# ps-auxw/CLI-P

Measured on AMD Instinct MI355X. Metric: images/sec ViT-B/32 encode, higher is better.
Workload: dtype bf16

## Files before the change

### cli-p_amd/_lib.py

```python
import ctypes as C
import os

HERE = os.path.dirname(os.path.abspath(__file__))
DEV_LIB = os.environ.get("CLIPMI_DEV_LIB", "") not in ("", "0")
LIB_PATH = os.path.join(HERE, "libclipmi_dev.so" if DEV_LIB else "libclipmi.so")

ABI_VERSION = 8
F32, BF16, U8 = 0, 1, 2

SYMBOLS = [
    "clipmi_encode_image_workspace_bytes", "clipmi_encode_image",
    "clipmi_encode_text_workspace_bytes", "clipmi_encode_text",
    "clipmi_topk_ip_workspace_bytes", "clipmi_topk_ip",
    "clipmi_topk_ip_coarse_workspace_bytes", "clipmi_topk_ip_coarse", "clipmi_dbg_topk_coarse_scan_ms",
    "clipmi_rows_stats", "clipmi_rows_absmax", "clipmi_rows_order_workspace_bytes", "clipmi_rows_order_by_absmax", "clipmi_rows_to_bf16", "clipmi_i8_copy_bytes", "clipmi_i8_meta_bytes", "clipmi_quantize_rows_i8", "clipmi_topk_ip_coarse_i8", "clipmi_dbg_topk_coarse_i8_scan_ms",
    "clipmi_topk_ip_wide_workspace_bytes", "clipmi_topk_ip_wide_i8", "clipmi_dbg_topk_wide_i8_scan_ms",
    "clipmi_dbg_quantize_rows_fp8", "clipmi_dbg_gemm_fp8",
    "clipmi_merge_topk_workspace_bytes", "clipmi_merge_topk", "clipmi_merge_topk_packed",
    "clipmi_l2_normalize_rows", "clipmi_resize_crop_rgb8", "clipmi_jpeg_workspace_bytes", "clipmi_jpeg_decode_rgb8", "clipmi_jpeg_progressive_workspace_bytes", "clipmi_jpeg_decode_progressive_rgb8", "clipmi_last_error", "clipmi_abi_version",
    "clipmi_dbg_gemm_bf16", "clipmi_dbg_layernorm", "clipmi_dbg_attention", "clipmi_dbg_topk_scan_ms",
    "clipmi_dbg_encode_image_probe_ms", "clipmi_dbg_encode_image_probe3_ms",
    "clipmi_dbg_split_stats", "clipmi_dbg_gemm_ln", "clipmi_dbg_gemm_resid_ln", "clipmi_dbg_gemm_resid_ln_leaf", "clipmi_dbg_gemm_ln_leaf", "clipmi_dbg_quantize_rows_fp8mx", "clipmi_dbg_gemm_fp8_bsa",
]


class Tower(C.Structure):
    _fields_ = [(n, C.c_int32) for n in (
        "abi_version", "kind", "width", "layers", "heads", "mlp", "embed", "tokens",
        "patch", "res", "patch_k", "vocab")] + [(n, C.c_uint64) for n in (
        "blob_bytes",
        "off_patch_w", "off_cls", "off_pos", "off_ln_pre_w", "off_ln_pre_b",
        "off_tok_emb",
        "off_layers", "layer_stride",
        "lo_ln1_w", "lo_ln1_b", "lo_qkv_w", "lo_qkv_b", "lo_out_w", "lo_out_b",
        "lo_ln2_w", "lo_ln2_b", "lo_fc_w", "lo_fc_b", "lo_proj_w", "lo_proj_b",
        "off_ln_post_w", "off_ln_post_b", "off_out_proj")] + [
        ("weight_format", C.c_int32), ("ln_fold", C.c_int32)] + [(n, C.c_uint64) for n in (
        "lo_qkv_s", "lo_out_s", "lo_fc_s", "lo_proj_s", "lo_qkv_colsum", "lo_qkv_cb", "lo_fc_colsum", "lo_fc_cb")]


class ClipmiError(RuntimeError):
    pass


_lib = None


def lib():
    global _lib
    if _lib is not None:
        return _lib
    if not os.path.exists(LIB_PATH):
        raise ClipmiError(
            f"{LIB_PATH} is missing: build the HIP library first "
            "(python -c 'import __graft_entry__ as g; g.build()'). There is no CPU fallback.")
    from . import build as _build
    if os.path.isdir(_build.CSRC) and not _build.is_current(_build.DEV if DEV_LIB else _build.PRODUCT):
        raise ClipmiError(
            f"{LIB_PATH} does not match the sources under csrc/ (content stamp mismatch): rebuild "
            "(python cli-p_amd/build.py). A stale HIP library is never loaded silently.")
    L = C.CDLL(LIB_PATH)
    vp, i32, i64, sz = C.c_void_p, C.c_int, C.c_int64, C.c_size_t
    TP = C.POINTER(Tower)
    L.clipmi_last_error.restype = C.c_char_p
    L.clipmi_abi_version.restype = i32
    L.clipmi_encode_image_workspace_bytes.restype = sz
    L.clipmi_encode_image_workspace_bytes.argtypes = [TP, i32]
    L.clipmi_encode_image.restype = i32
    L.clipmi_encode_image.argtypes = [TP, vp, vp, i32, i32, vp, i32, vp, sz, vp]
    L.clipmi_encode_text_workspace_bytes.restype = sz
    L.clipmi_encode_text_workspace_bytes.argtypes = [TP, i32]
    L.clipmi_encode_text.restype = i32
    L.clipmi_encode_text.argtypes = [TP, vp, vp, i32, vp, i32, vp, sz, vp]
    L.clipmi_topk_ip_workspace_bytes.restype = sz
    L.clipmi_topk_ip_workspace_bytes.argtypes = [i64, i32, i32, i32]
    L.clipmi_topk_ip.restype = i32
    L.clipmi_topk_ip.argtypes = [vp, i32, i64, i32, vp, i32, i32, i64, vp, vp, vp, sz, vp]
    L.clipmi_topk_ip_coarse_workspace_bytes.restype = sz
    L.clipmi_topk_ip_coarse_workspace_bytes.argtypes = [i64, i32, i32, i32]
    L.clipmi_topk_ip_coarse.restype = i32
    L.clipmi_topk_ip_coarse.argtypes = [vp, vp, i64, i32, C.c_float, vp, i32, i32, i64, vp, vp, vp, sz, vp]
    L.clipmi_dbg_quantize_rows_fp8.restype = i32
    L.clipmi_dbg_quantize_rows_fp8.argtypes = [vp, vp, vp, i32, i32, vp]
    L.clipmi_dbg_gemm_fp8.restype = i32
    L.clipmi_dbg_gemm_fp8.argtypes = [vp, vp, vp, vp, vp, vp, i32, i32, i32, i32, vp]
    L.clipmi_rows_stats.restype = i32
    L.clipmi_rows_stats.argtypes = [vp, i64, i32, vp, vp, vp]
    L.clipmi_rows_to_bf16.restype = i32
    L.clipmi_rows_to_bf16.argtypes = [vp, i64, i32, vp, vp]
    L.clipmi_i8_copy_bytes.restype = sz
    L.clipmi_i8_copy_bytes.argtypes = [i64, i32]
    L.clipmi_i8_meta_bytes.restype = sz
    L.clipmi_i8_meta_bytes.argtypes = [i64]
    L.clipmi_quantize_rows_i8.restype = i32
    L.clipmi_quantize_rows_i8.argtypes = [vp, i64, i32, vp, vp, sz, vp, sz, vp]
    L.clipmi_rows_absmax.restype = i32
    L.clipmi_rows_absmax.argtypes = [vp, i64, i32, vp, vp]
    L.clipmi_rows_order_workspace_bytes.restype = sz
    L.clipmi_rows_order_workspace_bytes.argtypes = [i64]
    L.clipmi_rows_order_by_absmax.restype = i32
    L.clipmi_rows_order_by_absmax.argtypes = [vp, i64, i32, vp, vp, sz, vp]
    L.clipmi_topk_ip_coarse_i8.restype = i32
    L.clipmi_topk_ip_coarse_i8.argtypes = [vp, vp, vp, C.c_float, i64, i32, C.c_float, vp, i32, i32, i64, vp, vp, vp, sz, vp]
    L.clipmi_dbg_topk_coarse_i8_scan_ms.restype = i32
    L.clipmi_dbg_topk_coarse_i8_scan_ms.argtypes = [vp, vp, vp, C.c_float, i64, i32, C.c_float, vp, i32, i32, vp, vp, vp, sz, vp,
                                                    i32, C.POINTER(C.c_float), C.POINTER(C.c_longlong)]
    L.clipmi_topk_ip_wide_workspace_bytes.restype = sz
    L.clipmi_topk_ip_wide_workspace_bytes.argtypes = [i64, i32, i32, i32]
    L.clipmi_topk_ip_wide_i8.restype = i32
    L.clipmi_topk_ip_wide_i8.argtypes = [vp, vp, vp, C.c_float, i64, i32, C.c_float, vp, i32, i32, i64, vp, vp, vp, sz, vp]
    L.clipmi_dbg_topk_wide_i8_scan_ms.restype = i32
    L.clipmi_dbg_topk_wide_i8_scan_ms.argtypes = [vp, vp, vp, C.c_float, i64, i32, C.c_float, vp, i32, i32, vp, vp, vp, sz, vp,
                                                  i32, C.POINTER(C.c_float), C.POINTER(C.c_longlong), C.POINTER(C.c_int),
                                                  C.POINTER(C.c_int)]
    L.clipmi_dbg_topk_coarse_scan_ms.restype = i32
    L.clipmi_dbg_topk_coarse_scan_ms.argtypes = [vp, vp, i64, i32, C.c_float, vp, i32, i32, vp, vp, vp, sz, vp, i32,
                                                 C.POINTER(C.c_float), C.POINTER(C.c_longlong)]
    L.clipmi_merge_topk_workspace_bytes.restype = sz
    L.clipmi_merge_topk_workspace_bytes.argtypes = [i32, i32, i32]
    L.clipmi_merge_topk.restype = i32
    L.clipmi_merge_topk.argtypes = [vp, vp, i32, i32, i32, vp, vp, vp, sz, vp]
    L.clipmi_merge_topk_packed.restype = i32
    L.clipmi_merge_topk_packed.argtypes = [vp, sz, i32, i32, i32, vp, vp, vp]
    L.clipmi_l2_normalize_rows.restype = i32
    L.clipmi_l2_normalize_rows.argtypes = [vp, i64, i32, vp]
    L.clipmi_resize_crop_rgb8.restype = i32
    L.clipmi_resize_crop_rgb8.argtypes = [vp, vp, i32, i32, vp, i32, vp, vp, vp]
    L.clipmi_jpeg_workspace_bytes.restype = i64
    L.clipmi_jpeg_workspace_bytes.argtypes = [i64, i32]
    L.clipmi_jpeg_decode_rgb8.restype = i32
    L.clipmi_jpeg_decode_rgb8.argtypes = [vp, vp, i32, vp, i32, i64, i64, i64, vp, vp, vp, i64, vp]
    L.clipmi_jpeg_progressive_workspace_bytes.restype = i64
    L.clipmi_jpeg_progressive_workspace_bytes.argtypes = [i32, i64, i32]
    L.clipmi_jpeg_decode_progressive_rgb8.restype = i32
    L.clipmi_jpeg_decode_progressive_rgb8.argtypes = [vp, vp, i32, vp, i32, vp, i32, i64, i64, i64, vp, vp, vp, i64, vp]
    L.clipmi_dbg_gemm_bf16.restype = i32
    L.clipmi_dbg_gemm_bf16.argtypes = [vp, vp, vp, vp, i32, i32, i32, i32, vp]
    L.clipmi_dbg_split_stats.restype = i32
    L.clipmi_dbg_split_stats.argtypes = [vp, i32, vp, vp, i32, i32, vp]
    L.clipmi_dbg_gemm_ln.restype = i32
    L.clipmi_dbg_gemm_ln.argtypes = [vp, vp, vp, vp, vp, vp, i32, i32, i32, i32, vp]
    L.clipmi_dbg_quantize_rows_fp8mx.restype = i32
    L.clipmi_dbg_quantize_rows_fp8mx.argtypes = [vp, vp, vp, i32, i32, vp]
    L.clipmi_dbg_gemm_fp8_bsa.restype = i32
    L.clipmi_dbg_gemm_fp8_bsa.argtypes = [vp, vp, vp, vp, vp, vp, i32, i32, i32, i32, vp]
    L.clipmi_dbg_gemm_resid_ln_leaf.restype = i32
    L.clipmi_dbg_gemm_resid_ln_leaf.argtypes = [vp, vp, vp, vp, vp, i32, i32, i32, vp]
    L.clipmi_dbg_gemm_ln_leaf.restype = i32
    L.clipmi_dbg_gemm_ln_leaf.argtypes = [vp, vp, vp, vp, vp, vp, i32, i32, i32, i32, vp]
    L.clipmi_dbg_gemm_resid_ln.restype = i32
    L.clipmi_dbg_gemm_resid_ln.argtypes = [vp, vp, vp, vp, vp, vp, i32, i32, i32, i32, vp]
    L.clipmi_dbg_layernorm.restype = i32
    L.clipmi_dbg_layernorm.argtypes = [vp, vp, vp, vp, i32, i32, i32, vp]
    L.clipmi_dbg_attention.restype = i32
    L.clipmi_dbg_attention.argtypes = [vp, vp, i32, i32, i32, i32, vp]
    L.clipmi_dbg_topk_scan_ms.restype = i32
    L.clipmi_dbg_topk_scan_ms.argtypes = [vp, i64, i32, vp, i32, i32, vp, vp, vp, sz, vp, i32, C.POINTER(C.c_float)]
    L.clipmi_dbg_encode_image_probe_ms.restype = i32
    L.clipmi_dbg_encode_image_probe_ms.argtypes = [TP, vp, vp, i32, i32, vp, vp, sz, vp, i32, i32,
                                                   C.POINTER(C.c_float), C.POINTER(C.c_int)]
    L.clipmi_dbg_encode_image_probe3_ms.restype = i32
    L.clipmi_dbg_encode_image_probe3_ms.argtypes = [TP, vp, vp, i32, i32, vp, vp, sz, vp, i32, i32,
                                                    C.POINTER(C.c_float), C.POINTER(C.c_int), C.POINTER(C.c_int),
                                                    C.POINTER(C.c_int)]
    if L.clipmi_abi_version() != ABI_VERSION:
        raise ClipmiError(f"libclipmi.so ABI {L.clipmi_abi_version()} != binding {ABI_VERSION}: rebuild")
    _lib = L
    return L


def check(rc, what):
    if rc != 0:
        msg = lib().clipmi_last_error().decode("utf-8", "replace")
        raise ClipmiError(f"{what} failed (code {rc}): {msg}")


def last_error():
    return lib().clipmi_last_error().decode("utf-8", "replace")


def stream_ptr(device=None):
    import torch
    return C.c_void_p(torch.cuda.current_stream(device).cuda_stream)


_SIDE_STREAMS = {}


_COPY_STREAMS = {}


def copy_stream(device):
    import torch
    key = torch.device(device).index
    s = _COPY_STREAMS.get(key)
    if s is None:
        s = _COPY_STREAMS[key] = torch.cuda.Stream(device=device)
    return s


def side_stream(device):
    import torch
    cur = torch.cuda.current_stream(device)
    key = (torch.device(device).index, cur.cuda_stream)
    s = _SIDE_STREAMS.get(key)
    if s is None:
        s = _SIDE_STREAMS[key] = torch.cuda.Stream(device=device)
    return cur, s
```

### cli-p_amd/csrc/encode.hip

```cpp
#include "vit_kernels.hpp"

namespace clipmi {
namespace {

struct Ws {
    unsigned short* patches;
    float* x;
    unsigned short* h;
    unsigned short* big;
    unsigned short* pooled;
    int* rowidx;
    unsigned char* a8;
    float* a_scale;
    unsigned char* a_bs;
    unsigned char* x8;
    unsigned char* x8_bs;
    void* x3;
    float* ln_part;
    float* ln_leaf;
    void* x3c;
    float* partc;
    float* leafc;
    float* xc;
};

size_t carve(const clipmi_tower* t, int B, void* base, size_t cap, Ws* out) {
    Arena ar(base ? base : reinterpret_cast<void*>(256), cap);
    const size_t rows = (size_t)B * t->tokens;
    const int W = t->width;
    Ws w{};
    if (t->kind == 0) w.patches = ar.take<unsigned short>((size_t)B * (t->tokens - 1) * t->patch_k);
    w.x = ar.take<float>(rows * W);
    w.h = ar.take<unsigned short>(rows * W);
    w.big = ar.take<unsigned short>(rows * 4 * W);
    w.pooled = ar.take<unsigned short>((size_t)B * W);
    w.rowidx = ar.take<int>((size_t)B);
    if (t->weight_format == 1) {
        w.a8 = ar.take<unsigned char>(rows * 4 * W);
        w.a_scale = ar.take<float>(rows);
        w.a_bs = ar.take<unsigned char>((rows + 255) / 256 * 256 * (size_t)(4 * W / 32));
    }
    if (t->ln_fold && t->weight_format == 1) {
        w.x8 = ar.take<unsigned char>(rows * W);
        w.x8_bs = ar.take<unsigned char>((rows + 255) / 256 * 256 * (size_t)(W / 32));
        w.ln_part = ar.take<float>(rows * 2 * (W / 256));
    } else if (t->ln_fold) {
        w.x3 = ar.take<unsigned char>(rows * resid_row_bytes(W));
        w.ln_part = ar.take<float>(rows * 2 * (W / 256));
        if (rows <= (size_t)SKINNY_MAX_M) w.ln_leaf = ar.take<float>(rows * 2 * (W / 4));
    }
    if (t->kind == 0 && t->weight_format == 0) {
        if (t->ln_fold) {
            w.x3c = ar.take<unsigned char>((size_t)B * resid_row_bytes(W));
            w.partc = ar.take<float>((size_t)B * 2 * (W / 256));
            if (B <= SKINNY_MAX_M) w.leafc = ar.take<float>((size_t)B * 2 * (W / 4));
        } else {
            w.xc = ar.take<float>((size_t)B * W);
        }
    }
    if (out) *out = w;
    return ar.off + 256;
}

int check_tower(const clipmi_tower* t, int kind, const char* who) {
    if (!t) return set_err(CLIPMI_EINVAL, "%s: NULL tower", who);
    if (t->abi_version != CLIPMI_ABI_VERSION)
        return set_err(CLIPMI_EINVAL, "%s: tower ABI %d != %d", who, t->abi_version, CLIPMI_ABI_VERSION);
    if (t->kind != kind) return set_err(CLIPMI_EINVAL, "%s: tower kind %d", who, t->kind);
    if (t->width % 128 != 0 || t->heads * 64 != t->width || t->mlp != 4 * t->width || t->embed % 128 != 0 ||
        t->width > 1024 || t->layers < 1)
        return set_err(CLIPMI_EUNSUPPORTED,
                       "%s: width=%d heads=%d mlp=%d embed=%d (need width %% 128 == 0 <= 1024, head dim 64, embed %% 128 == 0)",
                       who, t->width, t->heads, t->mlp, t->embed);
    if (t->weight_format != 0 && t->weight_format != 1)
        return set_err(CLIPMI_EINVAL, "%s: weight_format %d", who, t->weight_format);
    if (t->weight_format == 1 && t->width % 256 != 0)
        return set_err(CLIPMI_EUNSUPPORTED, "%s: fp8 weights need width %% 256 == 0 (width %d)", who, t->width);
    if (t->ln_fold != 0 && (t->ln_fold != 1 || t->width % 256 != 0))
        return set_err(CLIPMI_EINVAL, "%s: ln_fold %d needs width %% 256 == 0 (width %d)", who, t->ln_fold, t->width);
#ifndef CLIPMI_DEV
    if (t->ln_fold != 0 && t->weight_format != 0)
        return set_err(CLIPMI_EUNSUPPORTED, "%s: folded LayerNorms on FP8 weights exist in the development library only", who);
#endif
    if (t->tokens > 80 && kind == 1)
        return set_err(CLIPMI_EUNSUPPORTED, "%s: %d tokens (causal attention covers <= 80)", who, t->tokens);
    return 0;
}

template <typename T>
const T* at(const void* blob, uint64_t off) {
    return reinterpret_cast<const T*>(static_cast<const char*>(blob) + off);
}

bool encode_tail() {
    static const int mode = (int)dev_knob("CLIPMI_ENCODE_TAIL", 1);
    return mode != 0;
}

int launch_gather_rows(const void* src, void* dst, int B, int L, size_t row_bytes, hipStream_t st) {
    if (row_bytes % 16 != 0) return set_err(CLIPMI_EINVAL, "gather_rows: %zu bytes per row", row_bytes);
    const int row16 = (int)(row_bytes / 16);
    hipLaunchKernelGGL(gather_rows_kernel, dim3((unsigned)(((long long)B * row16 + 255) / 256)), dim3(256), 0, st,
                       static_cast<const uint4*>(src), static_cast<uint4*>(dst), B, L, row16);
    CLIPMI_CHECK_LAUNCH("gather_rows_kernel");
    return 0;
}

int run_layers(const clipmi_tower* t, const void* blob, const Ws& w, int B, int causal, hipStream_t st, GemmProbe* probe,
               bool* pruned = nullptr) {
    const int W = t->width, L = t->tokens, M = B * L;
    const bool fp8 = t->weight_format == 1;
    const bool tail = pruned && !causal && !fp8 && (t->ln_fold ? w.x3c != nullptr : w.xc != nullptr) && encode_tail();
    if (pruned) *pruned = tail;
    auto linear = [&](const unsigned short* A, int K, uint64_t w_off, uint64_t b_off, void* out, int N, int epi) -> int {
        GemmArgs g{};
        g.bias = at<float>(blob, b_off); g.out = out; g.M = M; g.N = N; g.K = K;
        g.A = A; g.W = at<unsigned short>(blob, w_off);
        return launch_gemm_algo(g, epi, 0, st, probe);
    };
#ifdef CLIPMI_DEV
    if (t->ln_fold && fp8) {
        auto lnfold8 = [&](uint64_t w_off, uint64_t s_off, uint64_t cb_off, uint64_t cs_off, void* out, unsigned char* out_bs, int N,
                           int epi) -> int {
            GemmArgs g{};
            g.A = reinterpret_cast<const unsigned short*>(w.x8); g.a_bscale = w.x8_bs;
            g.W = at<unsigned short>(blob, w_off); g.w_scale = at<float>(blob, s_off);
            g.bias = at<float>(blob, cb_off); g.colsum = at<float>(blob, cs_off); g.ln_part_in = w.ln_part;
            g.out = out; g.out_bscale = out_bs; g.M = M; g.N = N; g.K = W;
            return launch_gemm_fp8(g, epi, st);
        };
        auto resid8 = [&](const unsigned char* A8, int K, uint64_t w_off, uint64_t s_off, uint64_t b_off) -> int {
            GemmArgs g{};
            g.A = reinterpret_cast<const unsigned short*>(A8); g.a_bscale = w.a_bs;
            g.W = at<unsigned short>(blob, w_off); g.w_scale = at<float>(blob, s_off); g.bias = at<float>(blob, b_off);
            g.out = w.x; g.x8 = w.x8; g.x8_bs = w.x8_bs; g.ln_part = w.ln_part; g.M = M; g.N = W; g.K = K;
            return launch_gemm_fp8(g, EPI_BIAS_RESID_LN8, st);
        };
        unsigned char* const big8 = reinterpret_cast<unsigned char*>(w.big);
        static const bool fuse_off = dev_knob("CLIPMI_FP8_FUSE", 1) == 0;
        for (int l = 0; l < t->layers; ++l) {
            const uint64_t lb = t->off_layers + (uint64_t)l * t->layer_stride;
            if (int rc = lnfold8(lb + t->lo_qkv_w, lb + t->lo_qkv_s, lb + t->lo_qkv_cb, lb + t->lo_qkv_colsum, w.big, nullptr, 3 * W, EPI_LN_BIAS_BF16)) return rc;
            bool fused = false;
            if (int rc = launch_attention(w.big, w.h, B, L, t->heads, causal, 1, st, fuse_off ? nullptr : w.a8, w.a_bs, &fused)) return rc;
            if (!fused)
                if (int rc = launch_quantize_rows_fp8mx(w.h, w.a8, w.a_bs, M, W, st)) return rc;
            if (int rc = resid8(w.a8, W, lb + t->lo_out_w, lb + t->lo_out_s, lb + t->lo_out_b)) return rc;
            if (!fuse_off) {
                if (int rc = lnfold8(lb + t->lo_fc_w, lb + t->lo_fc_s, lb + t->lo_fc_cb, lb + t->lo_fc_colsum, big8, w.a_bs, 4 * W, EPI_LN_BIAS_QGELU_BF16)) return rc;
                if (int rc = resid8(big8, 4 * W, lb + t->lo_proj_w, lb + t->lo_proj_s, lb + t->lo_proj_b)) return rc;
            } else {
                if (int rc = lnfold8(lb + t->lo_fc_w, lb + t->lo_fc_s, lb + t->lo_fc_cb, lb + t->lo_fc_colsum, w.big, nullptr, 4 * W, EPI_LN_BIAS_QGELU_BF16)) return rc;
                if (int rc = launch_quantize_rows_fp8mx(w.big, w.a8, w.a_bs, M, 4 * W, st)) return rc;
                if (int rc = resid8(w.a8, 4 * W, lb + t->lo_proj_w, lb + t->lo_proj_s, lb + t->lo_proj_b)) return rc;
            }
        }
        return 0;
    }
#endif
    if (t->ln_fold) {
        auto lb_of = [&](int l) { return t->off_layers + (uint64_t)l * t->layer_stride; };
        const bool leaf_mode = w.ln_leaf != nullptr && gemm_resid_writes_leaves(M, W, W) && gemm_resid_writes_leaves(M, W, 4 * W);
        bool leaves = false;
        auto ln_linear = [&](uint64_t w_off, uint64_t cb_off, uint64_t cs_off, int N, int epi) -> int {
            GemmArgs g{};
            g.A = static_cast<const unsigned short*>(w.x3); g.lda_bytes = (unsigned)resid_row_bytes(W);
            g.W = at<unsigned short>(blob, w_off); g.bias = at<float>(blob, cb_off);
            g.colsum = at<float>(blob, cs_off); g.ln_part_in = w.ln_part;
            if (leaves) g.ln_leaf_in = w.ln_leaf;
            g.out = w.big; g.M = M; g.N = N; g.K = W;
            return launch_gemm_algo(g, epi, 0, st, probe);
        };
        auto resid_linear = [&](const unsigned short* A, int K, uint64_t w_off, uint64_t b_off) -> int {
            GemmArgs g{};
            g.A = A; g.W = at<unsigned short>(blob, w_off); g.bias = at<float>(blob, b_off);
            g.M = M; g.N = W; g.K = K;
            g.x3 = w.x3; g.ln_part = w.ln_part; g.tmp_f32 = w.x;
            if (leaf_mode) { g.ln_leaf = w.ln_leaf; leaves = true; }
            return launch_gemm_algo(g, EPI_BIAS_RESID_LN_F32, 0, st, probe);
        };
        for (int l = 0; l < t->layers; ++l) {
            const uint64_t lb = lb_of(l);
            if (int rc = ln_linear(lb + t->lo_qkv_w, lb + t->lo_qkv_cb, lb + t->lo_qkv_colsum, 3 * W, EPI_LN_BIAS_BF16)) return rc;
            if (tail && l == t->layers - 1) {
                const bool tleaf = w.leafc != nullptr && gemm_resid_writes_leaves(B, W, W) && gemm_resid_writes_leaves(B, W, 4 * W);
                if (int rc = launch_attention(w.big, w.h, B, L, t->heads, causal, 1, st)) return rc;
                if (int rc = launch_gather_rows(w.x3, w.x3c, B, L, resid_row_bytes(W), st)) return rc;
                auto tail_resid = [&](const unsigned short* A, unsigned lda_bytes, int K, uint64_t w_off, uint64_t b_off) -> int {
                    GemmArgs g{};
                    g.A = A; g.lda_bytes = lda_bytes; g.W = at<unsigned short>(blob, w_off); g.bias = at<float>(blob, b_off);
                    g.M = B; g.N = W; g.K = K;
                    g.x3 = w.x3c; g.ln_part = w.partc; g.tmp_f32 = w.x;
                    if (tleaf) g.ln_leaf = w.leafc;
                    return launch_gemm_algo(g, EPI_BIAS_RESID_LN_F32, 0, st, nullptr);
                };
                if (int rc = tail_resid(w.h, (unsigned)((size_t)L * W * 2), W, lb + t->lo_out_w, lb + t->lo_out_b)) return rc;
                GemmArgs g{};
                g.A = static_cast<const unsigned short*>(w.x3c); g.lda_bytes = (unsigned)resid_row_bytes(W);
                g.W = at<unsigned short>(blob, lb + t->lo_fc_w); g.bias = at<float>(blob, lb + t->lo_fc_cb);
                g.colsum = at<float>(blob, lb + t->lo_fc_colsum); g.ln_part_in = w.partc;
                if (tleaf) g.ln_leaf_in = w.leafc;
                g.out = w.big; g.M = B; g.N = 4 * W; g.K = W;
                if (int rc = launch_gemm_algo(g, EPI_LN_BIAS_QGELU_BF16, 0, st, nullptr)) return rc;
                return tail_resid(w.big, 0u, 4 * W, lb + t->lo_proj_w, lb + t->lo_proj_b);
            }
            hipEvent_t* aev = nullptr;
            if (probe && probe->mode == 2 && probe->n < GemmProbe::MAX) {
                const int pi = probe->begin(GemmProbe::EPI_ATTENTION, 2, st, 0);
                aev = &probe->ev[2 * pi];
            }
            if (int rc = launch_attention(w.big, w.h, B, L, t->heads, causal, 1, st, nullptr, nullptr, nullptr, aev)) return rc;
            if (int rc = resid_linear(w.h, W, lb + t->lo_out_w, lb + t->lo_out_b)) return rc;
            if (int rc = ln_linear(lb + t->lo_fc_w, lb + t->lo_fc_cb, lb + t->lo_fc_colsum, 4 * W, EPI_LN_BIAS_QGELU_BF16)) return rc;
            if (int rc = resid_linear(w.big, 4 * W, lb + t->lo_proj_w, lb + t->lo_proj_b)) return rc;
        }
        return 0;
    }
    if (fp8) {
        auto gemm8 = [&](const unsigned char* A8, const float* a_scale, const unsigned char* a_bs, int K, uint64_t w_off,
                         uint64_t s_off, uint64_t b_off, void* out, unsigned char* out_bs, int N, int epi) -> int {
            GemmArgs g{};
            g.bias = at<float>(blob, b_off); g.out = out; g.M = M; g.N = N; g.K = K;
            g.A = reinterpret_cast<const unsigned short*>(A8);
            g.W = at<unsigned short>(blob, w_off);
            g.a_scale = a_scale; g.a_bscale = a_bs; g.out_bscale = out_bs;
            g.w_scale = at<float>(blob, s_off);
            return launch_gemm_fp8(g, epi, st);
        };
        static const bool fuse_off = dev_knob("CLIPMI_FP8_FUSE", 1) == 0;
        const bool fc_mx = !fuse_off && gemm_fp8_emits_mx(M, 4 * W, W);
        unsigned char* const big8 = reinterpret_cast<unsigned char*>(w.big);
        for (int l = 0; l < t->layers; ++l) {
            const uint64_t lb = t->off_layers + (uint64_t)l * t->layer_stride;
            LnArgs ln{w.x, at<float>(blob, lb + t->lo_ln1_w), at<float>(blob, lb + t->lo_ln1_b), w.h, nullptr, 1, M, W, 1};
            ln.out8 = w.a8; ln.scale8 = w.a_scale;
            if (int rc = launch_layernorm(ln, st)) return rc;
            if (int rc = gemm8(w.a8, w.a_scale, nullptr, W, lb + t->lo_qkv_w, lb + t->lo_qkv_s, lb + t->lo_qkv_b, w.big, nullptr, 3 * W, EPI_BIAS_BF16)) return rc;
            bool fused = false;
            if (int rc = launch_attention(w.big, w.h, B, L, t->heads, causal, 1, st, fuse_off ? nullptr : w.a8, w.a_bs, &fused)) return rc;
            if (!fused)
                if (int rc = launch_quantize_rows_fp8mx(w.h, w.a8, w.a_bs, M, W, st)) return rc;
            if (int rc = gemm8(w.a8, nullptr, w.a_bs, W, lb + t->lo_out_w, lb + t->lo_out_s, lb + t->lo_out_b, w.x, nullptr, W, EPI_BIAS_RESID_F32)) return rc;
            ln.w = at<float>(blob, lb + t->lo_ln2_w); ln.b = at<float>(blob, lb + t->lo_ln2_b);
            if (int rc = launch_layernorm(ln, st)) return rc;
            const unsigned char* h8 = w.a8;
            if (fc_mx) {
                if (int rc = gemm8(w.a8, w.a_scale, nullptr, W, lb + t->lo_fc_w, lb + t->lo_fc_s, lb + t->lo_fc_b, big8, w.a_bs, 4 * W, EPI_BIAS_QGELU_BF16)) return rc;
                h8 = big8;
            } else {
                if (int rc = gemm8(w.a8, w.a_scale, nullptr, W, lb + t->lo_fc_w, lb + t->lo_fc_s, lb + t->lo_fc_b, w.big, nullptr, 4 * W, EPI_BIAS_QGELU_BF16)) return rc;
                if (int rc = launch_quantize_rows_fp8mx(w.big, w.a8, w.a_bs, M, 4 * W, st)) return rc;
            }
            if (int rc = gemm8(h8, nullptr, w.a_bs, 4 * W, lb + t->lo_proj_w, lb + t->lo_proj_s, lb + t->lo_proj_b, w.x, nullptr, W, EPI_BIAS_RESID_F32)) return rc;
        }
        return 0;
    }
    for (int l = 0; l < t->layers; ++l) {
        const uint64_t lb = t->off_layers + (uint64_t)l * t->layer_stride;
        LnArgs ln{w.x, at<float>(blob, lb + t->lo_ln1_w), at<float>(blob, lb + t->lo_ln1_b), w.h, nullptr, 1, M, W, 1};
        if (int rc = launch_layernorm(ln, st)) return rc;
        if (int rc = linear(w.h, W, lb + t->lo_qkv_w, lb + t->lo_qkv_b, w.big, 3 * W, EPI_BIAS_BF16)) return rc;
        if (int rc = launch_attention(w.big, w.h, B, L, t->heads, causal, 1, st)) return rc;
        if (tail && l == t->layers - 1) {
            if (int rc = launch_gather_rows(w.x, w.xc, B, L, (size_t)W * 4, st)) return rc;
            auto tail_linear = [&](const unsigned short* A, unsigned lda_bytes, int K, uint64_t w_off, uint64_t b_off, void* out, int N,
                                   int epi) -> int {
                GemmArgs g{};
                g.A = A; g.lda_bytes = lda_bytes; g.W = at<unsigned short>(blob, w_off); g.bias = at<float>(blob, b_off);
                g.out = out; g.M = B; g.N = N; g.K = K;
                return launch_gemm_algo(g, epi, 0, st, nullptr);
            };
            if (int rc = tail_linear(w.h, (unsigned)((size_t)L * W * 2), W, lb + t->lo_out_w, lb + t->lo_out_b, w.xc, W, EPI_BIAS_RESID_F32)) return rc;
            LnArgs ln2{w.xc, at<float>(blob, lb + t->lo_ln2_w), at<float>(blob, lb + t->lo_ln2_b), w.h, nullptr, 1, B, W, 1};
            if (int rc = launch_layernorm(ln2, st)) return rc;
            if (int rc = tail_linear(w.h, 0u, W, lb + t->lo_fc_w, lb + t->lo_fc_b, w.big, 4 * W, EPI_BIAS_QGELU_BF16)) return rc;
            return tail_linear(w.big, 0u, 4 * W, lb + t->lo_proj_w, lb + t->lo_proj_b, w.xc, W, EPI_BIAS_RESID_F32);
        }
        if (int rc = linear(w.h, W, lb + t->lo_out_w, lb + t->lo_out_b, w.x, W, EPI_BIAS_RESID_F32)) return rc;
        ln.w = at<float>(blob, lb + t->lo_ln2_w); ln.b = at<float>(blob, lb + t->lo_ln2_b);
        if (int rc = launch_layernorm(ln, st)) return rc;
        if (int rc = linear(w.h, W, lb + t->lo_fc_w, lb + t->lo_fc_b, w.big, 4 * W, EPI_BIAS_QGELU_BF16)) return rc;
        if (int rc = linear(w.big, 4 * W, lb + t->lo_proj_w, lb + t->lo_proj_b, w.x, W, EPI_BIAS_RESID_F32)) return rc;
    }
    return 0;
}

int run_head(const clipmi_tower* t, const void* blob, const Ws& w, int B, const int* rowidx, long long row_step,
             float* out, int normalize, hipStream_t st) {
    const bool split = t->ln_fold && t->weight_format == 0;
    LnArgs ln{split ? nullptr : w.x, at<float>(blob, t->off_ln_post_w), at<float>(blob, t->off_ln_post_b), w.pooled, rowidx,
              row_step, B, t->width, 1};
    ln.x3 = w.x3;
    if (int rc = launch_layernorm(ln, st)) return rc;
    GemmArgs g{};
    g.A = w.pooled; g.W = at<unsigned short>(blob, t->off_out_proj); g.bias = nullptr; g.out = out;
    g.M = B; g.N = t->embed; g.K = t->width;
    if (int rc = launch_gemm_algo(g, EPI_F32, 0, st)) return rc;
    if (normalize) return clipmi_l2_normalize_rows(out, B, t->embed, st);
    return 0;
}

}
}

using namespace clipmi;

extern "C" size_t clipmi_encode_image_workspace_bytes(const clipmi_tower* t, int B) {
    if (check_tower(t, 0, "encode_image")) return 0;
    if (B < 1) { set_err(CLIPMI_EINVAL, "encode_image: B=%d", B); return 0; }
    return carve(t, B, nullptr, ~(size_t)0, nullptr);
}

static int encode_image_impl(const clipmi_tower* t, const void* blob_dev, const void* pixels_dev, int pix_dtype,
                             int B, float* out_dev, int normalize, void* ws_dev, size_t ws_bytes, void* stream, GemmProbe* probe) {
    if (int rc = check_tower(t, 0, "encode_image")) return rc;
    if (!blob_dev || !pixels_dev || !out_dev || !ws_dev) return set_err(CLIPMI_EINVAL, "encode_image: NULL pointer");
    if (B < 1) return set_err(CLIPMI_EINVAL, "encode_image: B=%d", B);
    if (pix_dtype != CLIPMI_F32 && pix_dtype != CLIPMI_BF16 && pix_dtype != CLIPMI_U8)
        return set_err(CLIPMI_EINVAL, "encode_image: pix_dtype %d", pix_dtype);
    const int grid = t->res / t->patch, np = grid * grid;
    if (np + 1 != t->tokens || t->patch_k % 64 != 0 || t->patch_k < 3 * t->patch * t->patch)
        return set_err(CLIPMI_EINVAL, "encode_image: inconsistent tower (res %d patch %d tokens %d patch_k %d)", t->res,
                       t->patch, t->tokens, t->patch_k);
    const size_t need = clipmi_encode_image_workspace_bytes(t, B);
    if (ws_bytes < need) return set_err(CLIPMI_EWORKSPACE, "encode_image: workspace %zu < %zu", ws_bytes, need);
    Ws w;
    carve(t, B, ws_dev, ws_bytes, &w);
    hipStream_t st = as_stream(stream);
    const int W = t->width, L = t->tokens;

    PatchArgs pa{pixels_dev, w.patches, pix_dtype, B, t->res, t->patch, grid, np, t->patch_k};
    if (int rc = launch_patchify(pa, st)) return rc;
    GemmArgs g{};
    g.A = w.patches; g.W = at<unsigned short>(blob_dev, t->off_patch_w); g.bias = nullptr; g.out = w.x;
    g.M = B * np; g.N = W; g.K = t->patch_k; g.pos = at<float>(blob_dev, t->off_pos); g.np = np; g.L = L;
    if (int rc = launch_gemm_algo(g, EPI_PATCH_F32, 0, st)) return rc;
    hipLaunchKernelGGL(cls_rows_kernel, dim3((unsigned)(((long long)B * W + 255) / 256)), dim3(256), 0, st, w.x,
                       at<float>(blob_dev, t->off_cls), at<float>(blob_dev, t->off_pos), B, L, W);
    CLIPMI_CHECK_LAUNCH("cls_rows_kernel");
    LnArgs ln{w.x, at<float>(blob_dev, t->off_ln_pre_w), at<float>(blob_dev, t->off_ln_pre_b), w.x, nullptr, 1, B * L, W, 0};
    const bool fold8 = t->ln_fold && t->weight_format == 1;
    if (t->ln_fold && !fold8) { ln.out_x3 = w.x3; ln.out_part = w.ln_part; }
    if (int rc = launch_layernorm(ln, st)) return rc;
#ifdef CLIPMI_DEV
    if (fold8)
        if (int rc = launch_rows_mx_stats(w.x, w.x8, w.x8_bs, w.ln_part, B * L, W, st)) return rc;
#endif
    bool pruned = false;
    if (int rc = run_layers(t, blob_dev, w, B, 0, st, probe, &pruned)) return rc;
    if (pruned) {
        Ws wc = w;
        wc.x = w.xc; wc.x3 = w.x3c;
        return run_head(t, blob_dev, wc, B, nullptr, 1, out_dev, normalize, st);
    }
    return run_head(t, blob_dev, w, B, nullptr, L, out_dev, normalize, st);
}

extern "C" int clipmi_encode_image(const clipmi_tower* t, const void* blob_dev, const void* pixels_dev, int pix_dtype,
                                   int B, float* out_dev, int normalize, void* ws_dev, size_t ws_bytes, void* stream) {
    return encode_image_impl(t, blob_dev, pixels_dev, pix_dtype, B, out_dev, normalize, ws_dev, ws_bytes, stream, nullptr);
}

extern "C" size_t clipmi_encode_text_workspace_bytes(const clipmi_tower* t, int Q) {
    if (check_tower(t, 1, "encode_text")) return 0;
    if (Q < 1) { set_err(CLIPMI_EINVAL, "encode_text: Q=%d", Q); return 0; }
    return carve(t, Q, nullptr, ~(size_t)0, nullptr);
}

extern "C" int clipmi_encode_text(const clipmi_tower* t, const void* blob_dev, const int32_t* ids_dev, int Q,
                                  float* out_dev, int normalize, void* ws_dev, size_t ws_bytes, void* stream) {
    if (int rc = check_tower(t, 1, "encode_text")) return rc;
    if (!blob_dev || !ids_dev || !out_dev || !ws_dev) return set_err(CLIPMI_EINVAL, "encode_text: NULL pointer");
    if (Q < 1) return set_err(CLIPMI_EINVAL, "encode_text: Q=%d", Q);
    const size_t need = clipmi_encode_text_workspace_bytes(t, Q);
    if (ws_bytes < need) return set_err(CLIPMI_EWORKSPACE, "encode_text: workspace %zu < %zu", ws_bytes, need);
    Ws w;
    carve(t, Q, ws_dev, ws_bytes, &w);
    hipStream_t st = as_stream(stream);
    const int W = t->width, L = t->tokens;
    const long long n4 = (long long)Q * L * (W / 4);
    const bool fold8_ = t->ln_fold && t->weight_format == 1;
    if (t->ln_fold && !fold8_ && W % 256 == 0 && W <= 1024) {
        hipLaunchKernelGGL(text_embed_split_kernel, dim3((unsigned)((Q * L + 3) / 4 + 1)), dim3(256), 0, st, ids_dev,
                           at<float>(blob_dev, t->off_tok_emb), at<float>(blob_dev, t->off_pos), w.x3, w.ln_part, w.rowidx, Q, L, W,
                           t->vocab);
        CLIPMI_CHECK_LAUNCH("text_embed_split_kernel");
        if (int rc = run_layers(t, blob_dev, w, Q, 1, st, nullptr)) return rc;
        return run_head(t, blob_dev, w, Q, w.rowidx, 1, out_dev, normalize, st);
    }
    hipLaunchKernelGGL(text_embed_kernel, dim3((unsigned)((n4 + 255) / 256)), dim3(256), 0, st, w.x, ids_dev,
                       at<float>(blob_dev, t->off_tok_emb), at<float>(blob_dev, t->off_pos), Q, L, W, t->vocab);
    CLIPMI_CHECK_LAUNCH("text_embed_kernel");
    hipLaunchKernelGGL(eot_rows_kernel, dim3((Q + 63) / 64), dim3(64), 0, st, ids_dev, w.rowidx, Q, L);
    CLIPMI_CHECK_LAUNCH("eot_rows_kernel");
#ifdef CLIPMI_DEV
    if (t->ln_fold && t->weight_format == 1) {
        if (int rc = launch_rows_mx_stats(w.x, w.x8, w.x8_bs, w.ln_part, Q * L, W, st)) return rc;
    } else
#endif
    if (t->ln_fold) {
        if (int rc = launch_split_stats(w.x, false, w.x3, w.ln_part, Q * L, W, st)) return rc;
    }
    if (int rc = run_layers(t, blob_dev, w, Q, 1, st, nullptr)) return rc;
    return run_head(t, blob_dev, w, Q, w.rowidx, 1, out_dev, normalize, st);
}

static int encode_probe(const clipmi_tower* t, const void* blob_dev, const void* pixels_dev, int pix_dtype, int B, float* out_dev,
                        void* ws_dev, size_t ws_bytes, void* stream, int probe_epi, int reps, int nmodes, float* ms, int* launches,
                        int* kernel_kind, int* epi_ran) {
    if (!ms || reps < 1) return set_err(CLIPMI_EINVAL, "dbg_encode_image_probe_ms: bad arguments");
    const int k_filter = probe_epi >> 8;
    probe_epi &= 0xff;
    GemmProbe p;
    for (int i = 0; i < 2 * GemmProbe::MAX; ++i)
        if (hipEventCreate(&p.ev[i]) != hipSuccess) return set_err(CLIPMI_EHIP, "hipEventCreate");
    for (int i = 0; i < GemmProbe::MAX; ++i)
        if (hipEventCreate(&p.pre[i]) != hipSuccess) return set_err(CLIPMI_EHIP, "hipEventCreate");
    int rc = 0;
    for (int mode = 0; mode < nmodes && rc == 0; ++mode) {
        double total = 0.0;
        int count = 0;
        for (int r = 0; r < reps && rc == 0; ++r) {
            p.epi = probe_epi; p.n = 0; p.mode = mode;
            rc = encode_image_impl(t, blob_dev, pixels_dev, pix_dtype, B, out_dev, 1, ws_dev, ws_bytes, stream, &p);
            if (rc) break;
            if (hipStreamSynchronize(as_stream(stream)) != hipSuccess) { rc = set_err(CLIPMI_EHIP, "hipStreamSynchronize"); break; }
            for (int i = 0; i < p.n; ++i) {
                if (GemmProbe::base_of(p.epi_of[i]) != probe_epi || (k_filter && p.k_of[i] != k_filter)) continue;
                float v = 0.f;
                if (mode == 0) (void)hipEventElapsedTime(&v, p.ev[2 * i], p.ev[2 * i + 1]);
                else if (mode == 1) (void)hipEventElapsedTime(&v, p.pre[i], p.ev[2 * i + 1]);
                else {
                    if (i == 0 || p.kernel_of[i - 1] != 2 ||
                        (p.epi_of[i - 1] != EPI_BIAS_RESID_LN_F32 && p.epi_of[i - 1] != EPI_LN_BIAS_QGELU_BF16 &&
                         p.epi_of[i - 1] != GemmProbe::EPI_ATTENTION)) continue;
                    (void)hipEventElapsedTime(&v, p.ev[2 * (i - 1) + 1], p.ev[2 * i + 1]);
                }
                total += v;
                ++count;
                if (kernel_kind) *kernel_kind = p.kernel_of[i];
                if (epi_ran) *epi_ran = p.epi_of[i];
            }
        }
        if (rc == 0 && count == 0 && mode == 0) rc = set_err(CLIPMI_EINVAL, "dbg_encode_image_probe_ms: no launch matched epi %d", probe_epi);
        if (rc == 0) { ms[mode] = count ? (float)(total / count) : 0.f; if (launches && mode == 0) *launches = count; }
    }
    for (int i = 0; i < 2 * GemmProbe::MAX; ++i) (void)hipEventDestroy(p.ev[i]);
    for (int i = 0; i < GemmProbe::MAX; ++i) (void)hipEventDestroy(p.pre[i]);
    return rc;
}

extern "C" int clipmi_dbg_encode_image_probe_ms(const clipmi_tower* t, const void* blob_dev, const void* pixels_dev,
                                                int pix_dtype, int B, float* out_dev, void* ws_dev, size_t ws_bytes,
                                                void* stream, int probe_epi, int reps, float* kernel_ms, int* launches) {
    return encode_probe(t, blob_dev, pixels_dev, pix_dtype, B, out_dev, ws_dev, ws_bytes, stream, probe_epi, reps, 1, kernel_ms,
                        launches, nullptr, nullptr);
}

extern "C" int clipmi_dbg_encode_image_probe3_ms(const clipmi_tower* t, const void* blob_dev, const void* pixels_dev,
                                                 int pix_dtype, int B, float* out_dev, void* ws_dev, size_t ws_bytes,
                                                 void* stream, int probe_epi, int reps, float* ms3, int* launches,
                                                 int* kernel_kind, int* epi_ran) {
    return encode_probe(t, blob_dev, pixels_dev, pix_dtype, B, out_dev, ws_dev, ws_bytes, stream, probe_epi, reps, 3, ms3,
                        launches, kernel_kind, epi_ran);
}
```

### cli-p_amd/csrc/gemm.hip

```cpp
#include "gemm256p.hpp"
#include "gemm_skinny.hpp"
#ifdef CLIPMI_DEV
#endif
#include "gemm256f8.hpp"
#include <hip/hip_ext.h>
#include <cstdlib>

namespace clipmi {

static bool lds_opted(int* slots) {
    int dev = 0;
    (void)hipGetDevice(&dev);
    if (dev < 0 || dev >= 64) return false;
    if (slots[dev]) return true;
    slots[dev] = 1;
    return false;
}

template <int EPI>
static int launch_epi(const GemmArgs& g, hipStream_t st, GemmProbe* probe) {
    const int grid = (g.N / GEMM_BN) * ((g.M + GEMM_BM - 1) / GEMM_BM);
    if (probe && probe->wants(EPI)) {
        GemmProbe& p = *probe;
        const int i = p.begin(EPI, 0, st, g.K);
        hipExtLaunchKernelGGL(gemm_bf16_nt_kernel<EPI>, dim3(grid), dim3(256), GEMM_LDS_BYTES, st, p.ev[2 * i],
                              p.ev[2 * i + 1], 0, g);
    } else {
        hipLaunchKernelGGL(gemm_bf16_nt_kernel<EPI>, dim3(grid), dim3(256), GEMM_LDS_BYTES, st, g);
    }
    CLIPMI_CHECK_LAUNCH("gemm_bf16_nt_kernel");
    return 0;
}

template <int EPI>
static int launch_epi256(const GemmArgs& g, hipStream_t st, GemmProbe* probe) {
    const int grid = (g.N / 256) * ((g.M + 255) / 256);
    static thread_local int opted[64];
    if (!lds_opted(opted)) {
        if (hipFuncSetAttribute((const void*)gemm256_bf16_nt_kernel<EPI>, hipFuncAttributeMaxDynamicSharedMemorySize,
                                G256_LDS) != hipSuccess)
            return set_err(CLIPMI_EHIP, "hipFuncSetAttribute(gemm256, %d B LDS)", G256_LDS);
    }
    if (probe && probe->wants(EPI)) {
        GemmProbe& p = *probe;
        const int i = p.begin(EPI, 1, st, g.K);
        hipExtLaunchKernelGGL(gemm256_bf16_nt_kernel<EPI>, dim3(grid), dim3(512), G256_LDS, st, p.ev[2 * i],
                              p.ev[2 * i + 1], 0, g);
    } else {
        hipLaunchKernelGGL(gemm256_bf16_nt_kernel<EPI>, dim3(grid), dim3(512), G256_LDS, st, g);
    }
    CLIPMI_CHECK_LAUNCH("gemm256_bf16_nt_kernel");
    return 0;
}

#ifdef CLIPMI_DEV
template <int EPI, int WD = 1>
static int launch_epi256wd(const GemmArgs& g, hipStream_t st) {
    const int grid = (g.N / 256) * ((g.M + 255) / 256);
    static thread_local int opted[64];
    if (!lds_opted(opted)) {
        if (hipFuncSetAttribute((const void*)gemm256_bf16_nt_kernel<EPI, WD>, hipFuncAttributeMaxDynamicSharedMemorySize,
                                G256_LDS) != hipSuccess)
            return set_err(CLIPMI_EHIP, "hipFuncSetAttribute(gemm256 WD, %d B LDS)", G256_LDS);
    }
    hipLaunchKernelGGL((gemm256_bf16_nt_kernel<EPI, WD>), dim3(grid), dim3(512), G256_LDS, st, g);
    CLIPMI_CHECK_LAUNCH("gemm256_bf16_nt_kernel<WD>");
    return 0;
}
#endif

static int persist_mode() {
    static const int mode = (int)dev_knob("CLIPMI_GEMM_PERSIST", 1);
    return mode;
}

constexpr int g256p_lds(int epi, bool fp8, int N, int K, int dbg) {
    const int nseg = K >> 8;
    return G256_LDS + N * 4 * (fp8 ? 2 : 1) + (fp8 ? 1024 : epi_is_ln(epi) ? 1024 + 256 * nseg * 8 + (nseg < 4 ? 8 : 0) : 0) +
           ((dbg & 12) ? 8192 + 2048 : 0);
}

template <int EPI, bool FP8 = false>
static int launch_epi256p(const GemmArgs& g, hipStream_t st, GemmProbe* probe) {
    const int tiles = (g.N / 256) * ((g.M + 255) / 256);
    static const int grid_max = (int)dev_knob("CLIPMI_GEMM_GRID", NUM_CU);
    const int grid = tiles < grid_max ? tiles : grid_max;
    const int lds = g256p_lds(EPI, FP8, g.N, g.K, g.dbg);
    if (lds > LDS_BYTES) return set_err(CLIPMI_EUNSUPPORTED, "gemm256p: %d B of LDS for N=%d", lds, g.N);
    static thread_local int opted[64];
    if (!lds_opted(opted)) {
        if (hipFuncSetAttribute((const void*)gemm256p_bf16_nt_kernel<EPI, FP8>, hipFuncAttributeMaxDynamicSharedMemorySize,
                                LDS_BYTES) != hipSuccess)
            return set_err(CLIPMI_EHIP, "hipFuncSetAttribute(gemm256p, %d B LDS)", LDS_BYTES);
    }
    if (probe && probe->wants(EPI)) {
        GemmProbe& p = *probe;
        const int i = p.begin(EPI, 2, st, g.K);
        hipExtLaunchKernelGGL((gemm256p_bf16_nt_kernel<EPI, FP8>), dim3(grid), dim3(512), lds, st, p.ev[2 * i],
                              p.ev[2 * i + 1], 0, g);
    } else {
        hipLaunchKernelGGL((gemm256p_bf16_nt_kernel<EPI, FP8>), dim3(grid), dim3(512), lds, st, g);
    }
    CLIPMI_CHECK_LAUNCH("gemm256p_bf16_nt_kernel");
    return 0;
}


static int split_pct() {
    static const int pct = (int)dev_knob("CLIPMI_GEMM_SPLIT", 40);
    return pct;
}

static bool skinny_ok(const GemmArgs& g) {
    static const bool off = dev_knob("CLIPMI_GEMM_SKINNY", 1) == 0;
    return !off && g.M >= 1 && g.M <= SKINNY_MAX_M && g.N % 16 == 0 && g.K % 32 == 0 && g.K >= 32;
}

template <int EPI>
static int launch_skinny_t(const GemmArgs& g, hipStream_t st) {
    const int nstrips = g.N / 16, mtiles = (g.M + 15) / 16;
    const int waves = nstrips * mtiles <= 4 * NUM_CU ? 1 : 4;
    const dim3 grid((nstrips + waves - 1) / waves, mtiles);
    if (g.K > 512) hipLaunchKernelGGL((gemm_skinny_kernel<EPI, 32>), grid, dim3(waves * 64), 0, st, g);
    else hipLaunchKernelGGL((gemm_skinny_kernel<EPI, 16>), grid, dim3(waves * 64), 0, st, g);
    CLIPMI_CHECK_LAUNCH("gemm_skinny_kernel");
    return 0;
}

bool gemm_resid_writes_leaves(int M, int N, int K) {
    GemmArgs g{};
    g.M = M; g.N = N; g.K = K;
    return skinny_ok(g) && N % 256 == 0 && N <= 1024;
}

static int launch_skinny(const GemmArgs& g, int epi, hipStream_t st) {
    if (!g.A || !g.W || (!g.out && epi != EPI_BIAS_RESID_LN_F32)) return set_err(CLIPMI_EINVAL, "gemm: NULL pointer");
    switch (epi) {
        case EPI_BIAS_BF16: return launch_skinny_t<EPI_BIAS_BF16>(g, st);
        case EPI_BIAS_QGELU_BF16: return launch_skinny_t<EPI_BIAS_QGELU_BF16>(g, st);
        case EPI_BIAS_RESID_F32: return launch_skinny_t<EPI_BIAS_RESID_F32>(g, st);
        case EPI_F32: return launch_skinny_t<EPI_F32>(g, st);
        case EPI_PATCH_F32: return launch_skinny_t<EPI_PATCH_F32>(g, st);
        case EPI_LN_BIAS_BF16: return launch_skinny_t<EPI_LN_BIAS_BF16>(g, st);
        case EPI_LN_BIAS_QGELU_BF16: return launch_skinny_t<EPI_LN_BIAS_QGELU_BF16>(g, st);
        case EPI_BIAS_RESID_LN_F32: return launch_skinny_t<EPI_BIAS_RESID_LN_F32>(g, st);
    }
    return set_err(CLIPMI_EINVAL, "gemm_skinny: epilogue %d", epi);
}

int launch_gemm_algo(const GemmArgs& g, int epi, int algo, hipStream_t st, GemmProbe* probe) {
    if (epi_is_ln(epi) && ((!g.ln_part_in && !g.ln_leaf_in) || !g.colsum || !g.bias || g.K % 256 != 0 || g.K > 1024))
        return set_err(CLIPMI_EINVAL, "gemm: LN-folded epilogue %d needs ln_part_in, colsum, bias and K %% 256 == 0, K <= 1024", epi);
    if (epi == EPI_BIAS_RESID_LN_F32 &&
        (!g.x3 || !g.ln_part || !g.tmp_f32 || g.N % 256 != 0 || g.N > 1024 || ((size_t)g.x3 & 15) != 0))
        return set_err(CLIPMI_EINVAL, "gemm: EPI_BIAS_RESID_LN_F32 needs x3 (16-byte aligned), ln_part, tmp_f32 and N %% 256 == 0, N <= 1024");
    if (g.lda_bytes && (g.lda_bytes % 16 != 0 || g.lda_bytes < 2u * (unsigned)g.K))
        return set_err(CLIPMI_EINVAL, "gemm: lda_bytes %u (need a multiple of 16, >= 2 K)", g.lda_bytes);
#ifndef CLIPMI_DEV
    if (algo == 4 || algo == 5) return set_err(CLIPMI_EUNSUPPORTED, "algo %d exists in the development build only (libclipmi_dev.so)", algo);
#else
    if (algo == 5) {
        if (g.N % 256 != 0 || g.K % 64 != 0 || g.K < 128 || g.M < 1 || !g.A || !g.W || !g.out)
            return set_err(CLIPMI_EINVAL, "gemm256 WD: N %% 256 == 0, K %% 64 == 0, K >= 128");
        if (epi == EPI_BIAS_BF16) return launch_epi256wd<EPI_BIAS_BF16>(g, st);
        if (epi == EPI_BIAS_QGELU_BF16) return launch_epi256wd<EPI_BIAS_QGELU_BF16>(g, st);
        if (epi == EPI_F32) return launch_epi256wd<EPI_F32>(g, st);
        return set_err(CLIPMI_EINVAL, "gemm256 WD: epilogue %d", epi);
    }
    if (algo == 4) return set_err(CLIPMI_EUNSUPPORTED, "algo 4 (gemm2w, DESIGN 4.4g) was removed in round 5: measured slower in round 3, its sources are in the history");
#endif
    const bool ok256 = g.N % 256 == 0 && g.K % 64 == 0 && g.K >= 128;
    if (algo == 2 && !ok256) return set_err(CLIPMI_EINVAL, "gemm256: N=%d K=%d (need N %% 256 == 0, K %% 64 == 0, K >= 128)", g.N, g.K);
    const bool store_only = epi == EPI_BIAS_BF16 || epi == EPI_BIAS_QGELU_BF16 || epi == EPI_BIAS_RESID_F32 || epi_is_ln(epi) ||
                            epi == EPI_BIAS_RESID_LN_F32;
    const bool ok256p = ok256 && g.K % 128 == 0 && g.N <= G256P_MAX_N && store_only && g.K <= (1 << 20) &&
                        g256p_lds(epi, false, g.N, g.K, g.dbg) <= LDS_BYTES && (!epi_is_ln(epi) || (g.K % 256 == 0 && g.K <= 1024));
    if (algo == 3 && !ok256p)
        return set_err(CLIPMI_EINVAL, "gemm256p: M=%d N=%d K=%d epi=%d (need N %% 256 == 0, K %% 128 == 0, a store-only epilogue "
                       "and bias/colsum rows that fit LDS)", g.M, g.N, g.K, epi);
    bool use256 = algo == 2 || algo == 3;
    bool use256p = algo == 3;
    if (algo == 0 && ok256 && g.M >= 1024) {
        const long long tiles = (long long)(g.N / 256) * ((g.M + 255) / 256);
        const long long rounds = (tiles + NUM_CU - 1) / NUM_CU;
        const long long pct = g.K >= 2048 ? 72 : 78;
        use256 = tiles * 100 >= rounds * NUM_CU * pct;
        use256p = use256 && ok256p && persist_mode() != 0 &&
                  (tiles > NUM_CU || (epi == EPI_BIAS_RESID_LN_F32 && persist_mode() != 2));
        if (ok256p && persist_mode() != 0 && tiles > NUM_CU && epi != EPI_PATCH_F32 && (tiles % NUM_CU) != 0 &&
            (tiles % NUM_CU) * 100 < (long long)NUM_CU * split_pct()) {
            const int ntn = g.N / 256;
            const long long main_tiles = (tiles / NUM_CU) * NUM_CU;
            const int rows_main = (int)(main_tiles / ntn) * 256;
            if (rows_main >= 256 && rows_main < g.M) {
                GemmArgs a = g, b = g;
                a.M = rows_main;
                b.M = g.M - rows_main;
                b.A = g.A + (size_t)rows_main * gemm_lda(g);
                const size_t oe = (size_t)rows_main * g.N;
                if (epi == EPI_BIAS_RESID_LN_F32) {
                    b.x3 = static_cast<char*>(g.x3) + (size_t)rows_main * resid_row_bytes(g.N); b.tmp_f32 = g.tmp_f32 + oe;
                    b.ln_part = g.ln_part + (size_t)rows_main * (g.N / 256) * 2;
                } else if (epi_is_bf16_out(epi)) {
                    b.out = static_cast<unsigned short*>(g.out) + oe;
                } else {
                    b.out = static_cast<float*>(g.out) + oe;
                }
                if (b.ln_part_in) b.ln_part_in = g.ln_part_in + (size_t)rows_main * (g.K / 256) * 2;
                if (int rc = launch_gemm_algo(a, epi, 3, st, probe)) return rc;
                return launch_gemm_algo(b, epi, 0, st, probe);
            }
        }
    }
    if (g.M < 1 || !g.A || !g.W || (!g.out && epi != EPI_BIAS_RESID_LN_F32)) return set_err(CLIPMI_EINVAL, "gemm: bad arguments");
    const bool skinny = algo == 0 && skinny_ok(g);
    if (skinny && epi != EPI_BIAS_RESID_LN_F32) return launch_skinny(g, epi, st);
    if (epi == EPI_BIAS_RESID_LN_F32 && skinny && g.ln_leaf) return launch_skinny(g, epi, st);
    if (g.ln_leaf_in && !(skinny && epi_is_ln(epi)))
        return set_err(CLIPMI_EINVAL, "gemm: ln_leaf_in is read by the skinny LN-folded consumers only (M <= %d)", SKINNY_MAX_M);
    if (epi == EPI_BIAS_RESID_LN_F32 && !use256p) {
        GemmArgs t = g;
        t.out = g.tmp_f32;
        GemmProbe* pr = (probe && probe->wants(EPI_BIAS_RESID_LN_F32)) ? probe : nullptr;
        const int saved_epi = pr ? pr->epi : -1;
        if (pr) pr->epi = EPI_F32;
        const int rc = skinny ? launch_skinny(t, EPI_F32, st) : use256 ? launch_epi256<EPI_F32>(t, st, pr) : launch_gemm(t, EPI_F32, st, pr);
        if (pr) pr->epi = saved_epi;
        if (rc) return rc;
        return launch_split_stats(g.tmp_f32, true, g.x3, g.ln_part, g.M, g.N, st);
    }
    if (!use256) return launch_gemm(g, epi, st, probe);
    if (use256p) {
        switch (epi) {
            case EPI_BIAS_BF16: return launch_epi256p<EPI_BIAS_BF16>(g, st, probe);
            case EPI_BIAS_QGELU_BF16: return launch_epi256p<EPI_BIAS_QGELU_BF16>(g, st, probe);
            case EPI_BIAS_RESID_F32: return launch_epi256p<EPI_BIAS_RESID_F32>(g, st, probe);
            case EPI_LN_BIAS_BF16: return launch_epi256p<EPI_LN_BIAS_BF16>(g, st, probe);
            case EPI_LN_BIAS_QGELU_BF16: return launch_epi256p<EPI_LN_BIAS_QGELU_BF16>(g, st, probe);
            case EPI_BIAS_RESID_LN_F32: return launch_epi256p<EPI_BIAS_RESID_LN_F32>(g, st, probe);
        }
        return set_err(CLIPMI_EINVAL, "gemm256p: epilogue %d", epi);
    }
    switch (epi) {
        case EPI_BIAS_BF16: return launch_epi256<EPI_BIAS_BF16>(g, st, probe);
        case EPI_BIAS_QGELU_BF16: return launch_epi256<EPI_BIAS_QGELU_BF16>(g, st, probe);
        case EPI_BIAS_RESID_F32: return launch_epi256<EPI_BIAS_RESID_F32>(g, st, probe);
        case EPI_F32: return launch_epi256<EPI_F32>(g, st, probe);
        case EPI_PATCH_F32: return launch_epi256<EPI_PATCH_F32>(g, st, probe);
        case EPI_LN_BIAS_BF16: return launch_epi256<EPI_LN_BIAS_BF16>(g, st, probe);
        case EPI_LN_BIAS_QGELU_BF16: return launch_epi256<EPI_LN_BIAS_QGELU_BF16>(g, st, probe);
    }
    return set_err(CLIPMI_EINVAL, "gemm: unknown epilogue %d", epi);
}

template <int EPI, bool MX>
static int launch_epi256f8(const GemmArgs& g, hipStream_t st) {
    const int grid = (g.N / 256) * ((g.M + 255) / 256);
    static thread_local int opted[64];
    if (!lds_opted(opted)) {
        if (hipFuncSetAttribute((const void*)gemm256f8_nt_kernel<EPI, MX>, hipFuncAttributeMaxDynamicSharedMemorySize,
                                G256_LDS) != hipSuccess)
            return set_err(CLIPMI_EHIP, "hipFuncSetAttribute(gemm256f8, %d B LDS)", G256_LDS);
    }
    hipLaunchKernelGGL((gemm256f8_nt_kernel<EPI, MX>), dim3(grid), dim3(512), G256_LDS, st, g);
    CLIPMI_CHECK_LAUNCH("gemm256f8_nt_kernel");
    return 0;
}

constexpr int G256F8_BSA_MAX_K = 4096;
template <int EPI>
static int launch_epi256f8_bsa(const GemmArgs& g, hipStream_t st) {
    const int grid = (g.N / 256) * ((g.M + 255) / 256);
    const int lds = G256_LDS + 256 * (g.K / 32);
    static thread_local int opted[64];
    if (!lds_opted(opted)) {
        if (hipFuncSetAttribute((const void*)gemm256f8_nt_kernel<EPI, true, true>, hipFuncAttributeMaxDynamicSharedMemorySize,
                                G256_LDS + 256 * (G256F8_BSA_MAX_K / 32)) != hipSuccess)
            return set_err(CLIPMI_EHIP, "hipFuncSetAttribute(gemm256f8 block-scaled)");
    }
    hipLaunchKernelGGL((gemm256f8_nt_kernel<EPI, true, true>), dim3(grid), dim3(512), lds, st, g);
    CLIPMI_CHECK_LAUNCH("gemm256f8_nt_kernel(block-scaled A)");
    return 0;
}

bool gemm_fp8_emits_mx(int M, int N, int K) {
    const long long tiles = (long long)(N / 256) * ((M + 255) / 256);
    return M >= 1 && N % 256 == 0 && K % 256 == 0 && K >= 256 && tiles > NUM_CU && N <= 3840 && persist_mode() != 0;
}

int launch_gemm_fp8(const GemmArgs& g, int epi, hipStream_t st, int mx) {
    if (g.M < 1 || g.N % 256 != 0 || g.K % 128 != 0 || g.K < 256)
        return set_err(CLIPMI_EINVAL, "gemm_fp8: M=%d N=%d K=%d (need N %% 256 == 0, K %% 128 == 0, K >= 256)", g.M, g.N, g.K);
    if (!g.A || !g.W || !g.out || (!g.a_scale && !g.a_bscale) || !g.w_scale) return set_err(CLIPMI_EINVAL, "gemm_fp8: NULL pointer");
    if (g.a_bscale) {
        if (g.K > G256F8_BSA_MAX_K) return set_err(CLIPMI_EINVAL, "gemm_fp8: block-scaled A needs K <= %d", G256F8_BSA_MAX_K);
        if (epi == EPI_BIAS_RESID_F32) return launch_epi256f8_bsa<EPI_BIAS_RESID_F32>(g, st);
        if (epi == EPI_F32) return launch_epi256f8_bsa<EPI_F32>(g, st);
#ifdef CLIPMI_DEV
        if (epi == EPI_BIAS_RESID_LN8) {
            if (!g.x8 || !g.x8_bs || !g.ln_part || g.N > 1024)
                return set_err(CLIPMI_EINVAL, "gemm_fp8: EPI_BIAS_RESID_LN8 needs x8, x8_bs, ln_part and N <= 1024");
            return launch_epi256f8_bsa<EPI_BIAS_RESID_LN8>(g, st);
        }
        if (epi_is_ln(epi)) {
            if (!g.ln_part_in || !g.colsum || !g.bias || g.K % 256 != 0 || g.K > 1024)
                return set_err(CLIPMI_EINVAL, "gemm_fp8: LN-folded epilogue %d needs ln_part_in, colsum, bias, K %% 256 == 0, K <= 1024", epi);
            if (g.out_bscale && epi != EPI_LN_BIAS_QGELU_BF16)
                return set_err(CLIPMI_EINVAL, "gemm_fp8: e4m3 + block-scale output exists for the QuickGELU forms only");
            return epi == EPI_LN_BIAS_BF16 ? launch_epi256f8_bsa<EPI_LN_BIAS_BF16>(g, st) : launch_epi256f8_bsa<EPI_LN_BIAS_QGELU_BF16>(g, st);
        }
#endif
        return set_err(CLIPMI_EINVAL, "gemm_fp8: block-scaled A with epilogue %d", epi);
    }
    const long long tiles = (long long)(g.N / 256) * ((g.M + 255) / 256);
    if (g.out_bscale && !(mx == 1 && epi == EPI_BIAS_QGELU_BF16 && gemm_fp8_emits_mx(g.M, g.N, g.K)))
        return set_err(CLIPMI_EINVAL, "gemm_fp8: e4m3 + block-scale output exists for the persistent QuickGELU form only");
    if (mx == 1 && tiles > NUM_CU && g.K % 256 == 0 && g.N <= 3840 && persist_mode() != 0) {
        if (epi == EPI_BIAS_BF16) return launch_epi256p<EPI_BIAS_BF16, true>(g, st, nullptr);
        if (epi == EPI_BIAS_QGELU_BF16) return launch_epi256p<EPI_BIAS_QGELU_BF16, true>(g, st, nullptr);
    }
    switch (epi) {
        case EPI_BIAS_BF16: return mx ? launch_epi256f8<EPI_BIAS_BF16, true>(g, st) : launch_epi256f8<EPI_BIAS_BF16, false>(g, st);
        case EPI_BIAS_QGELU_BF16:
            return mx ? launch_epi256f8<EPI_BIAS_QGELU_BF16, true>(g, st) : launch_epi256f8<EPI_BIAS_QGELU_BF16, false>(g, st);
        case EPI_BIAS_RESID_F32:
            return mx ? launch_epi256f8<EPI_BIAS_RESID_F32, true>(g, st) : launch_epi256f8<EPI_BIAS_RESID_F32, false>(g, st);
        case EPI_F32: return mx ? launch_epi256f8<EPI_F32, true>(g, st) : launch_epi256f8<EPI_F32, false>(g, st);
    }
    return set_err(CLIPMI_EINVAL, "gemm_fp8: epilogue %d", epi);
}

int launch_gemm(const GemmArgs& g, int epi, hipStream_t st, GemmProbe* probe) {
    if (g.M < 1 || g.N < 1 || g.K < 1 || g.N % GEMM_BN != 0 || g.K % GEMM_BK != 0)
        return set_err(CLIPMI_EINVAL, "gemm: M=%d N=%d K=%d (need N %% 128 == 0, K %% 64 == 0)", g.M, g.N, g.K);
    if (!g.A || !g.W || !g.out) return set_err(CLIPMI_EINVAL, "gemm: NULL pointer");
    switch (epi) {
        case EPI_BIAS_BF16: return launch_epi<EPI_BIAS_BF16>(g, st, probe);
        case EPI_BIAS_QGELU_BF16: return launch_epi<EPI_BIAS_QGELU_BF16>(g, st, probe);
        case EPI_BIAS_RESID_F32: return launch_epi<EPI_BIAS_RESID_F32>(g, st, probe);
        case EPI_F32: return launch_epi<EPI_F32>(g, st, probe);
        case EPI_PATCH_F32: return launch_epi<EPI_PATCH_F32>(g, st, probe);
        case EPI_LN_BIAS_BF16: return launch_epi<EPI_LN_BIAS_BF16>(g, st, probe);
        case EPI_LN_BIAS_QGELU_BF16: return launch_epi<EPI_LN_BIAS_QGELU_BF16>(g, st, probe);
    }
    return set_err(CLIPMI_EINVAL, "gemm: unknown epilogue %d", epi);
}

}

using namespace clipmi;

extern "C" int clipmi_dbg_gemm_bf16(const void* a_dev, const void* w_dev, const float* bias_dev, void* out_dev, int M,
                                    int N, int K, int epi, void* stream) {
    const int algo = (epi >> 8) & 7;
    epi &= 0xff;
    if (epi < 0 || epi > 3) return set_err(CLIPMI_EINVAL, "dbg_gemm: epi %d", epi);
    GemmArgs g{};
    g.A = static_cast<const unsigned short*>(a_dev);
    g.W = static_cast<const unsigned short*>(w_dev);
    g.bias = bias_dev;
    g.out = out_dev;
    g.M = M; g.N = N; g.K = K;
    static const int dbg_env = (int)dev_knob("CLIPMI_GEMM_DBG", 0);
    g.dbg = dbg_env;
    if (g.dbg & 12) { g.pos = bias_dev; g.bias = nullptr; }
    return launch_gemm_algo(g, epi, algo, as_stream(stream));
}

extern "C" int clipmi_dbg_gemm_ln(const void* x3_dev, const void* wg_dev, const float* cb_dev, const float* colsum_dev,
                                  const float* part_dev, void* out_dev, int M, int N, int K, int epi, void* stream) {
    const int algo = (epi >> 8) & 3;
    epi &= 0xff;
    if (!epi_is_ln(epi)) return set_err(CLIPMI_EINVAL, "dbg_gemm_ln: epi %d", epi);
    GemmArgs g{};
    g.A = static_cast<const unsigned short*>(x3_dev);
    g.lda_bytes = (unsigned)resid_row_bytes(K);
    g.W = static_cast<const unsigned short*>(wg_dev);
    g.bias = cb_dev; g.colsum = colsum_dev; g.ln_part_in = part_dev;
    g.out = out_dev;
    g.M = M; g.N = N; g.K = K;
    return launch_gemm_algo(g, epi, algo, as_stream(stream));
}

extern "C" int clipmi_dbg_gemm_resid_ln_leaf(const void* a_dev, const void* w_dev, const float* bias_dev, void* x3_dev, float* leaf_dev,
                                             int M, int N, int K, void* stream) {
    if (!leaf_dev || !gemm_resid_writes_leaves(M, N, K))
        return set_err(CLIPMI_EINVAL, "dbg_gemm_resid_ln_leaf: M <= %d, N %% 256 == 0, N <= 1024, K %% 32 == 0", SKINNY_MAX_M);
    GemmArgs g{};
    g.A = static_cast<const unsigned short*>(a_dev);
    g.W = static_cast<const unsigned short*>(w_dev);
    g.bias = bias_dev;
    g.x3 = x3_dev; g.ln_leaf = leaf_dev;
    g.ln_part = leaf_dev; g.tmp_f32 = leaf_dev;
    g.M = M; g.N = N; g.K = K;
    return launch_gemm_algo(g, EPI_BIAS_RESID_LN_F32, 0, as_stream(stream));
}

extern "C" int clipmi_dbg_gemm_ln_leaf(const void* x3_dev, const void* wg_dev, const float* cb_dev, const float* colsum_dev,
                                       const float* leaf_dev, void* out_dev, int M, int N, int K, int epi, void* stream) {
    if (!epi_is_ln(epi)) return set_err(CLIPMI_EINVAL, "dbg_gemm_ln_leaf: epi %d", epi);
    GemmArgs g{};
    g.A = static_cast<const unsigned short*>(x3_dev);
    g.lda_bytes = (unsigned)resid_row_bytes(K);
    g.W = static_cast<const unsigned short*>(wg_dev);
    g.bias = cb_dev; g.colsum = colsum_dev; g.ln_leaf_in = leaf_dev;
    g.out = out_dev;
    g.M = M; g.N = N; g.K = K;
    return launch_gemm_algo(g, epi, 0, as_stream(stream));
}

extern "C" int clipmi_dbg_gemm_resid_ln(const void* a_dev, const void* w_dev, const float* bias_dev, void* x3_dev,
                                        float* part_dev, float* tmp_dev, int M, int N, int K, int algo, void* stream) {
    GemmArgs g{};
    g.A = static_cast<const unsigned short*>(a_dev);
    g.W = static_cast<const unsigned short*>(w_dev);
    g.bias = bias_dev;
    g.x3 = x3_dev;
    g.ln_part = part_dev; g.tmp_f32 = tmp_dev;
    g.M = M; g.N = N; g.K = K;
    static const int dbg_env = (int)dev_knob("CLIPMI_GEMM_DBG", 0);
    g.dbg = dbg_env;
    return launch_gemm_algo(g, EPI_BIAS_RESID_LN_F32, algo & 7, as_stream(stream));
}

extern "C" int clipmi_dbg_gemm_fp8_bsa(const void* a8_dev, const void* w8_dev, const void* a_bscale_dev, const float* w_scale_dev,
                                       const float* bias_dev, void* out_dev, int M, int N, int K, int epi, void* stream) {
    GemmArgs g{};
    g.A = static_cast<const unsigned short*>(a8_dev);
    g.W = static_cast<const unsigned short*>(w8_dev);
    g.a_bscale = static_cast<const unsigned char*>(a_bscale_dev); g.w_scale = w_scale_dev;
    g.bias = bias_dev;
    g.out = out_dev;
    g.M = M; g.N = N; g.K = K;
    return launch_gemm_fp8(g, epi, as_stream(stream), 1);
}

extern "C" int clipmi_dbg_gemm_fp8(const void* a8_dev, const void* w8_dev, const float* a_scale_dev, const float* w_scale_dev,
                                   const float* bias_dev, void* out_dev, int M, int N, int K, int epi, void* stream) {
    const int mx = (epi >> 8) & 1 ? 0 : ((epi >> 9) & 1 ? 2 : 1);
    epi &= 0xff;
    if (epi < 0 || epi > 3) return set_err(CLIPMI_EINVAL, "dbg_gemm_fp8: epi %d", epi);
    GemmArgs g{};
    g.A = static_cast<const unsigned short*>(a8_dev);
    g.W = static_cast<const unsigned short*>(w8_dev);
    g.a_scale = a_scale_dev; g.w_scale = w_scale_dev;
    g.bias = bias_dev;
    g.out = out_dev;
    g.M = M; g.N = N; g.K = K;
    return launch_gemm_fp8(g, epi, as_stream(stream), mx);
}
```

### cli-p_amd/csrc/gemm.hpp

```cpp
#pragma once
#include "common.hpp"

namespace clipmi {

typedef __bf16 bf16x8 __attribute__((ext_vector_type(8)));
typedef __bf16 bf16x2 __attribute__((ext_vector_type(2)));
typedef float f32x4 __attribute__((ext_vector_type(4)));
typedef float f32x2 __attribute__((ext_vector_type(2)));

__device__ __forceinline__ unsigned pack_bf16x2(float a, float b) {
    f32x2 v = {a, b};
    bf16x2 r = __builtin_convertvector(v, bf16x2);
    return __builtin_bit_cast(unsigned, r);
}

__device__ __forceinline__ float bf16_to_f32(unsigned short h) { return __uint_as_float((unsigned)h << 16); }

constexpr float QGELU_C = -2.4554669595930157f;
__device__ __forceinline__ float quick_gelu(float x) {
    return x * __builtin_amdgcn_rcpf(1.0f + __builtin_amdgcn_exp2f(x * QGELU_C));
}
__device__ __forceinline__ f32x4 quick_gelu4(f32x4 x) {
    const f32x4 t = x * QGELU_C;
    f32x4 e;
    e.x = __builtin_amdgcn_exp2f(t.x); e.y = __builtin_amdgcn_exp2f(t.y);
    e.z = __builtin_amdgcn_exp2f(t.z); e.w = __builtin_amdgcn_exp2f(t.w);
    const f32x4 d = e + 1.0f;
    f32x4 r;
    r.x = __builtin_amdgcn_rcpf(d.x); r.y = __builtin_amdgcn_rcpf(d.y);
    r.z = __builtin_amdgcn_rcpf(d.z); r.w = __builtin_amdgcn_rcpf(d.w);
    return x * r;
}

enum Epilogue {
    EPI_BIAS_BF16 = 0,
    EPI_BIAS_QGELU_BF16 = 1,
    EPI_BIAS_RESID_F32 = 2,
    EPI_F32 = 3,
    EPI_PATCH_F32 = 4,
    EPI_LN_BIAS_BF16 = 5,
    EPI_LN_BIAS_QGELU_BF16 = 6,
    EPI_BIAS_RESID_LN_F32 = 7,
    EPI_BIAS_RESID_LN8 = 8
};

constexpr float LN_EPS = 1e-5f;

__device__ __forceinline__ float ln_lane_sum(f32x4 v) { return (v.x + v.y) + (v.z + v.w); }
__device__ __forceinline__ float ln_lane_sumsq(f32x4 v) {
    float q = v.x * v.x;
    q = __builtin_fmaf(v.y, v.y, q);
    q = __builtin_fmaf(v.z, v.z, q);
    return __builtin_fmaf(v.w, v.w, q);
}
template <int CTRL>
__device__ __forceinline__ float lane_dpp(float v) {
    return __int_as_float(__builtin_amdgcn_update_dpp(0, __float_as_int(v), CTRL, 0xf, 0xf, false));
}
__device__ __forceinline__ float lane_xor8(float v) { return lane_dpp<0x128>(v); }
__device__ __forceinline__ float lane_xor4(float v, bool bit2) {
    const float up = lane_dpp<0x104>(v), dn = lane_dpp<0x114>(v);
    return bit2 ? dn : up;
}
__device__ __forceinline__ float lane_xor2(float v) { return lane_dpp<0x4E>(v); }
__device__ __forceinline__ float lane_xor1(float v) { return lane_dpp<0xB1>(v); }
__device__ __forceinline__ float lane_fold32(float a, float b) {
    const auto r = __builtin_amdgcn_permlane32_swap(__float_as_uint(a), __float_as_uint(b), false, false);
    return __uint_as_float(r[0]) + __uint_as_float(r[1]);
}
__device__ __forceinline__ float lane_fold16(float a, float b) {
    const auto r = __builtin_amdgcn_permlane16_swap(__float_as_uint(a), __float_as_uint(b), false, false);
    return __uint_as_float(r[0]) + __uint_as_float(r[1]);
}
__device__ __forceinline__ float ln_wave_sum(float v) {
    const bool bit2 = (__builtin_amdgcn_mbcnt_lo(~0u, 0u) & 4u) != 0;
    v = lane_fold32(v, v);
    v = lane_fold16(v, v);
    v += lane_xor8(v);
    v += lane_xor4(v, bit2);
    v += lane_xor2(v);
    v += lane_xor1(v);
    return v;
}
__device__ __forceinline__ f32x2 ln_row_stats(const float* part, int nseg, int W) {
    float s = part[0], q = part[1];
    if (nseg > 1) { s += part[2]; q += part[3]; }
    if (nseg > 2) { s += part[4]; q += part[5]; }
    if (nseg > 3) { s += part[6]; q += part[7]; }
    const float inv = 1.0f / (float)W;
    const float mean = s * inv;
    float var = __builtin_fmaf(-mean, mean, q * inv);
    var = var > 0.f ? var : 0.f;
    return f32x2{mean, __builtin_amdgcn_rsqf(var + LN_EPS)};
}
__device__ __forceinline__ f32x4 ln_apply(f32x4 acc, float mean, float rstd, f32x4 colsum, f32x4 cb) {
    f32x4 r;
    r.x = __builtin_fmaf(__builtin_fmaf(-mean, colsum.x, acc.x), rstd, cb.x);
    r.y = __builtin_fmaf(__builtin_fmaf(-mean, colsum.y, acc.y), rstd, cb.y);
    r.z = __builtin_fmaf(__builtin_fmaf(-mean, colsum.z, acc.z), rstd, cb.z);
    r.w = __builtin_fmaf(__builtin_fmaf(-mean, colsum.w, acc.w), rstd, cb.w);
    return r;
}
__device__ __forceinline__ f32x4 split_join(uint2 hi, unsigned lo) {
    return f32x4{__uint_as_float(__builtin_amdgcn_perm(hi.x, lo, 0x0504000cu) - 0x8000u),
                 __uint_as_float(__builtin_amdgcn_perm(hi.x, lo, 0x0706010cu) - 0x8000u),
                 __uint_as_float(__builtin_amdgcn_perm(hi.y, lo, 0x0504020cu) - 0x8000u),
                 __uint_as_float(__builtin_amdgcn_perm(hi.y, lo, 0x0706030cu) - 0x8000u)};
}
__device__ __forceinline__ void split_make(f32x4 o, uint2& hi, unsigned& lo) {
    hi = make_uint2(pack_bf16x2(o.x, o.y), pack_bf16x2(o.z, o.w));
    auto rem = [](float v, unsigned hb) -> unsigned {
        const unsigned t = (__float_as_uint(v) + 0x8080u) - hb;
        return t < 0xffffu ? t : 0xffffu;
    };
    const unsigned t0 = rem(o.x, hi.x << 16), t1 = rem(o.y, hi.x & 0xffff0000u), t2 = rem(o.z, hi.y << 16),
                   t3 = rem(o.w, hi.y & 0xffff0000u);
    lo = __builtin_amdgcn_perm(t1, t0, 0x0c0c0501u) | __builtin_amdgcn_perm(t3, t2, 0x05010c0cu);
}
__host__ __device__ constexpr size_t resid_row_bytes(int W) { return (size_t)W * 3; }
__device__ __forceinline__ const unsigned short* resid_hi(const void* x3, size_t row, int W) {
    return reinterpret_cast<const unsigned short*>(static_cast<const char*>(x3) + row * resid_row_bytes(W));
}
__device__ __forceinline__ unsigned short* resid_hi(void* x3, size_t row, int W) {
    return reinterpret_cast<unsigned short*>(static_cast<char*>(x3) + row * resid_row_bytes(W));
}
__device__ __forceinline__ const unsigned char* resid_lo(const void* x3, size_t row, int W) {
    return reinterpret_cast<const unsigned char*>(static_cast<const char*>(x3) + row * resid_row_bytes(W) + (size_t)W * 2);
}
__device__ __forceinline__ unsigned char* resid_lo(void* x3, size_t row, int W) {
    return reinterpret_cast<unsigned char*>(static_cast<char*>(x3) + row * resid_row_bytes(W) + (size_t)W * 2);
}
__device__ __forceinline__ unsigned fp8mx_scale_byte(float amax) {
    const int e = (int)((__float_as_uint(amax) >> 23) & 0xffu);
    if (amax == 0.f) return 127u;
    return (unsigned)(e > 7 ? e - 7 : 0);
}
__device__ __forceinline__ float fp8mx_inv(unsigned sb) { return __uint_as_float((254u - sb) << 23); }
__device__ __forceinline__ uint2 fp8_pack8(const float* f) {
    int lo = 0, hi = 0;
    lo = __builtin_amdgcn_cvt_pk_fp8_f32(f[0], f[1], lo, false);
    lo = __builtin_amdgcn_cvt_pk_fp8_f32(f[2], f[3], lo, true);
    hi = __builtin_amdgcn_cvt_pk_fp8_f32(f[4], f[5], hi, false);
    hi = __builtin_amdgcn_cvt_pk_fp8_f32(f[6], f[7], hi, true);
    return make_uint2((unsigned)lo, (unsigned)hi);
}

__device__ __forceinline__ void ln8_row_segment(f32x4 v, unsigned& packed4, unsigned& scale_byte, float& sum, float& sumsq) {
    sum = ln_wave_sum(ln_lane_sum(v));
    sumsq = ln_wave_sum(ln_lane_sumsq(v));
    float mx = fmaxf(fmaxf(fabsf(v.x), fabsf(v.y)), fmaxf(fabsf(v.z), fabsf(v.w)));
    mx = fmaxf(mx, __shfl_xor(mx, 1));
    mx = fmaxf(mx, __shfl_xor(mx, 2));
    mx = fmaxf(mx, __shfl_xor(mx, 4));
    scale_byte = fp8mx_scale_byte(mx);
    const float inv = fp8mx_inv(scale_byte);
    int pk = 0;
    pk = __builtin_amdgcn_cvt_pk_fp8_f32(v.x * inv, v.y * inv, pk, false);
    pk = __builtin_amdgcn_cvt_pk_fp8_f32(v.z * inv, v.w * inv, pk, true);
    packed4 = (unsigned)pk;
}

__device__ __forceinline__ uint2 mx_pack_bf16x8(uint4 x, unsigned& sb_out) {
    const unsigned w_[4] = {x.x, x.y, x.z, x.w};
    typedef unsigned short u16x2 __attribute__((ext_vector_type(2)));
    u16x2 pm = __builtin_elementwise_max(
        __builtin_elementwise_max(__builtin_bit_cast(u16x2, w_[0] & 0x7fff7fffu), __builtin_bit_cast(u16x2, w_[1] & 0x7fff7fffu)),
        __builtin_elementwise_max(__builtin_bit_cast(u16x2, w_[2] & 0x7fff7fffu), __builtin_bit_cast(u16x2, w_[3] & 0x7fff7fffu)));
    unsigned mm = __builtin_bit_cast(unsigned, pm);
    mm = (mm & 0xffffu) > (mm >> 16) ? (mm & 0xffffu) : (mm >> 16);
    const unsigned m1_ = (unsigned)__builtin_amdgcn_update_dpp(0, (int)mm, 0xB1, 0xf, 0xf, false);
    mm = mm > m1_ ? mm : m1_;
    const unsigned m2_ = (unsigned)__builtin_amdgcn_update_dpp(0, (int)mm, 0x4E, 0xf, 0xf, false);
    mm = mm > m2_ ? mm : m2_;
    const unsigned e_ = mm >> 7;
    const unsigned sb_ = mm == 0u ? 127u : (e_ > 7u ? e_ - 7u : 0u);
    const float inv_ = fp8mx_inv(sb_);
    float f[8];
#pragma unroll
    for (int j = 0; j < 4; ++j) {
        const f32x2 p_ = f32x2{__uint_as_float(w_[j] << 16), __uint_as_float(w_[j] & 0xffff0000u)} * inv_;
        f[2 * j] = p_.x;
        f[2 * j + 1] = p_.y;
    }
    sb_out = sb_;
    return fp8_pack8(f);
}

constexpr bool epi_is_ln(int e) { return e == EPI_LN_BIAS_BF16 || e == EPI_LN_BIAS_QGELU_BF16; }
constexpr bool epi_is_qgelu(int e) { return e == EPI_BIAS_QGELU_BF16 || e == EPI_LN_BIAS_QGELU_BF16; }
constexpr bool epi_is_bf16_out(int e) { return e == EPI_BIAS_BF16 || e == EPI_BIAS_QGELU_BF16 || epi_is_ln(e); }

struct GemmArgs {
    const unsigned short* A;
    const unsigned short* W;
    const float* bias;
    void* out;
    int M, N, K;
    const float* pos;
    int np, L;
    unsigned char* x8;
    unsigned char* x8_bs;
    int dbg;
    const float* a_scale;
    const float* w_scale;
    const unsigned char* a_bscale;
    unsigned char* out_bscale;
    const float* ln_part_in;
    const float* colsum;
    void* x3;
    float* ln_part;
    float* tmp_f32;
    unsigned lda_bytes;
    float* ln_leaf;
    const float* ln_leaf_in;
};
constexpr int SKINNY_MAX_M = 128;
__host__ __device__ inline size_t gemm_lda(const GemmArgs& g) { return g.lda_bytes ? (size_t)g.lda_bytes / 2 : (size_t)g.K; }

__device__ __forceinline__ void gemm_tile_coords(int bid, int nwg, int mtiles, int ntn, int GM, int GN, int& bm, int& bn) {
    const int xcd = bid & 7, qq = nwg >> 3, rr = nwg & 7;
    const int tile = (xcd < rr ? xcd * (qq + 1) : rr * (qq + 1) + (xcd - rr) * qq) + (bid >> 3);
    const int per_super = GM * ntn;
    const int sr = tile / per_super;
    const int r = tile - sr * per_super;
    const int left = mtiles - sr * GM;
    const int gm = left < GM ? left : GM;
    const int full = ntn / GN;
    int ng = r / (gm * GN);
    ng = ng < full ? ng : full;
    const int r2 = r - ng * gm * GN;
    const int gn = (ntn - ng * GN) < GN ? (ntn - ng * GN) : GN;
    const int mi = r2 / gn;
    bm = sr * GM + mi;
    bn = ng * GN + (r2 - mi * gn);
}

constexpr int GEMM_BM = 128, GEMM_BN = 128, GEMM_BK = 64;
constexpr int GEMM_TILE_BYTES = GEMM_BM * GEMM_BK * 2;
constexpr int GEMM_LDS_BYTES = 4 * GEMM_TILE_BYTES;

template <int EPI>
__global__ void __launch_bounds__(256) gemm_bf16_nt_kernel(GemmArgs g) {
    extern __shared__ __attribute__((aligned(16))) char smem[];
    const int tid = threadIdx.x;
    const int lane = tid & 63;
    const int wave = __builtin_amdgcn_readfirstlane(tid >> 6);
    const int wm = wave >> 1, wn = wave & 1;
    const int fr = lane & 15, fg = lane >> 4;

    const int ntn = g.N / GEMM_BN;
    int bm, bn;
    gemm_tile_coords(blockIdx.x, gridDim.x, (g.M + GEMM_BM - 1) / GEMM_BM, ntn, 8, 8, bm, bn);
    const int m0 = bm * GEMM_BM, n0 = bn * GEMM_BN;
    const int K = g.K;

    const int srow = lane >> 3;
    const int spos = lane & 7;
    const unsigned short* a_src[4];
    const unsigned short* w_src[4];
#pragma unroll
    for (int i = 0; i < 4; ++i) {
        const int row = wave * 32 + i * 8 + srow;
        const int chunk = spos ^ (row & 7);
        int am = m0 + row;
        am = am < g.M ? am : g.M - 1;
        a_src[i] = g.A + (size_t)am * gemm_lda(g) + chunk * 8;
        w_src[i] = g.W + (size_t)(n0 + row) * K + chunk * 8;
    }
    auto stage = [&](int kt, int buf) {
        char* abase = smem + buf * (2 * GEMM_TILE_BYTES) + wave * 32 * 128;
        char* bbase = abase + GEMM_TILE_BYTES;
#pragma unroll
        for (int i = 0; i < 4; ++i) {
            __builtin_amdgcn_global_load_lds((const __attribute__((address_space(1))) void*)(a_src[i] + kt * GEMM_BK),
                                             (__attribute__((address_space(3))) void*)(abase + i * 1024), 16, 0, 0);
            __builtin_amdgcn_global_load_lds((const __attribute__((address_space(1))) void*)(w_src[i] + kt * GEMM_BK),
                                             (__attribute__((address_space(3))) void*)(bbase + i * 1024), 16, 0, 0);
        }
    };

    f32x4 acc[4][4];
#pragma unroll
    for (int i = 0; i < 4; ++i)
#pragma unroll
        for (int j = 0; j < 4; ++j) acc[i][j] = f32x4{0.f, 0.f, 0.f, 0.f};

    const int sw = fr & 7;
    const int a_off = (wm * 64 + fr) * 128;
    const int b_off = GEMM_TILE_BYTES + (wn * 64 + fr) * 128;
    const int c0 = ((0 + fg) ^ sw) * 16, c1 = ((4 + fg) ^ sw) * 16;

    const int nk = K / GEMM_BK;
    stage(0, 0);
    for (int kt = 0; kt < nk; ++kt) {
        asm volatile("s_waitcnt vmcnt(0)" ::: "memory");
        __syncthreads();
        if (kt + 1 < nk) stage(kt + 1, (kt + 1) & 1);
        const char* base = smem + (kt & 1) * (2 * GEMM_TILE_BYTES);
        bf16x8 af[4][2], wf[4][2];
#pragma unroll
        for (int t = 0; t < 4; ++t) {
            af[t][0] = *reinterpret_cast<const bf16x8*>(base + a_off + t * 2048 + c0);
            af[t][1] = *reinterpret_cast<const bf16x8*>(base + a_off + t * 2048 + c1);
            wf[t][0] = *reinterpret_cast<const bf16x8*>(base + b_off + t * 2048 + c0);
            wf[t][1] = *reinterpret_cast<const bf16x8*>(base + b_off + t * 2048 + c1);
        }
#pragma unroll
        for (int ks = 0; ks < 2; ++ks)
#pragma unroll
            for (int mt = 0; mt < 4; ++mt)
#pragma unroll
                for (int nt = 0; nt < 4; ++nt)
                    acc[mt][nt] = __builtin_amdgcn_mfma_f32_16x16x32_bf16(wf[nt][ks], af[mt][ks], acc[mt][nt], 0, 0, 0);
    }

    f32x4 bz[4], cs[4];
#pragma unroll
    for (int nt = 0; nt < 4; ++nt) {
        const int n = n0 + wn * 64 + nt * 16 + 4 * fg;
        bz[nt] = g.bias ? *reinterpret_cast<const f32x4*>(g.bias + n) : f32x4{0.f, 0.f, 0.f, 0.f};
        if (epi_is_ln(EPI)) cs[nt] = *reinterpret_cast<const f32x4*>(g.colsum + n);
    }
    constexpr bool RMW = (EPI == EPI_BIAS_RESID_F32) || (EPI == EPI_PATCH_F32);
    auto row_of = [&](int mt, size_t& orow, const float*& addrow, bool& valid) {
        const int m = m0 + wm * 64 + mt * 16 + fr;
        valid = m < g.M;
        const int mc = valid ? m : g.M - 1;
        orow = (size_t)mc;
        addrow = nullptr;
        if (EPI == EPI_PATCH_F32) {
            const int b_ = mc / g.np, p_ = mc - b_ * g.np;
            orow = (size_t)b_ * g.L + 1 + p_;
            addrow = g.pos + (size_t)(1 + p_) * g.N;
        } else if (EPI == EPI_BIAS_RESID_F32) {
            addrow = static_cast<const float*>(g.out) + orow * g.N;
        }
    };
    f32x4 cur[4], nxt[4];
    if (RMW) {
        size_t orow; const float* addrow; bool valid;
        row_of(0, orow, addrow, valid);
#pragma unroll
        for (int nt = 0; nt < 4; ++nt) cur[nt] = *reinterpret_cast<const f32x4*>(addrow + n0 + wn * 64 + nt * 16 + 4 * fg);
    }
#pragma unroll
    for (int mt = 0; mt < 4; ++mt) {
        size_t orow; const float* addrow; bool valid;
        row_of(mt, orow, addrow, valid);
        if (RMW && mt + 1 < 4) {
            size_t orow2; const float* addrow2; bool valid2;
            row_of(mt + 1, orow2, addrow2, valid2);
#pragma unroll
            for (int nt = 0; nt < 4; ++nt) nxt[nt] = *reinterpret_cast<const f32x4*>(addrow2 + n0 + wn * 64 + nt * 16 + 4 * fg);
        }
#pragma unroll
        for (int nt = 0; nt < 4; ++nt) {
            const int n = n0 + wn * 64 + nt * 16 + 4 * fg;
            f32x4 v;
            if (epi_is_ln(EPI)) {
                const int nseg = g.K >> 8;
                const f32x2 st = ln_row_stats(g.ln_part_in + orow * 2 * nseg, nseg, g.K);
                v = ln_apply(acc[mt][nt], st.x, st.y, cs[nt], bz[nt]);
            } else {
                v = acc[mt][nt] + bz[nt];
            }
            if (epi_is_bf16_out(EPI)) {
                if (epi_is_qgelu(EPI)) {
                    v = quick_gelu4(v);
                }
                if (valid)
                    *reinterpret_cast<uint2*>(static_cast<unsigned short*>(g.out) + orow * g.N + n) =
                        make_uint2(pack_bf16x2(v.x, v.y), pack_bf16x2(v.z, v.w));
            } else {
                if (RMW) v += cur[nt];
                if (valid) *reinterpret_cast<f32x4*>(static_cast<float*>(g.out) + orow * g.N + n) = v;
            }
        }
        if (RMW) {
#pragma unroll
            for (int nt = 0; nt < 4; ++nt) cur[nt] = nxt[nt];
        }
    }
}

struct GemmProbe {
    static constexpr int MAX = 96;
    static constexpr int EPI_ATTENTION = 100;
    int epi = -1, n = 0;
    int mode = 0;
    hipEvent_t ev[2 * MAX];
    hipEvent_t pre[MAX];
    int epi_of[MAX];
    int kernel_of[MAX];
    int k_of[MAX];
    static int base_of(int e) {
        return e == EPI_LN_BIAS_BF16 ? EPI_BIAS_BF16 : e == EPI_LN_BIAS_QGELU_BF16 ? EPI_BIAS_QGELU_BF16 :
               e == EPI_BIAS_RESID_LN_F32 ? EPI_BIAS_RESID_F32 : e;
    }
    bool wants(int e) const { return n < MAX && (mode == 2 || base_of(e) == epi); }
    int begin(int e, int kernel, hipStream_t st, int K = 0) {
        epi_of[n] = e;
        kernel_of[n] = kernel;
        k_of[n] = K;
        if (mode == 1) (void)hipEventRecord(pre[n], st);
        return n++;
    }
};

int launch_gemm(const GemmArgs& g, int epi, hipStream_t st, GemmProbe* probe = nullptr);
int launch_gemm_algo(const GemmArgs& g, int epi, int algo, hipStream_t st, GemmProbe* probe = nullptr);
int launch_gemm_fp8(const GemmArgs& g, int epi, hipStream_t st, int mx = 1);
bool gemm_resid_writes_leaves(int M, int N, int K);
bool gemm_fp8_emits_mx(int M, int N, int K);
int launch_split_stats(const float* x_or_add, bool add, void* x3, float* part, int M, int W, hipStream_t st);

}
```

### cli-p_amd/csrc/gemm_skinny.hpp

```cpp
#pragma once
#include "gemm.hpp"

namespace clipmi {

template <int EPI, int DEPTH>
__global__ void __launch_bounds__(256) gemm_skinny_kernel(GemmArgs g) {
    constexpr int SKINNY_DEPTH = DEPTH;
    const int lane = threadIdx.x & 63;
    const int wave = __builtin_amdgcn_readfirstlane(threadIdx.x >> 6);
    const int fr = lane & 15, fg = lane >> 4;
    const int nstrips = g.N >> 4;
    const int strip = blockIdx.x * (blockDim.x >> 6) + wave;
    if (strip >= nstrips) return;
    const int n0 = strip << 4, m0 = blockIdx.y << 4;
    const int K = g.K;
    int am = m0 + fr;
    const bool valid = am < g.M;
    am = valid ? am : g.M - 1;
    const bf16x8* wp = reinterpret_cast<const bf16x8*>(g.W + (size_t)(n0 + fr) * K + 8 * fg);
    const bf16x8* ap = reinterpret_cast<const bf16x8*>(g.A + (size_t)am * gemm_lda(g) + 8 * fg);
    const int nk = K >> 5;

    const int n = n0 + 4 * fg;
    const f32x4 bz = g.bias ? *reinterpret_cast<const f32x4*>(g.bias + n) : f32x4{0.f, 0.f, 0.f, 0.f};
    f32x4 cs = {0.f, 0.f, 0.f, 0.f};
    float part[8] = {0.f, 0.f, 0.f, 0.f, 0.f, 0.f, 0.f, 0.f};
    f32x4 add = {0.f, 0.f, 0.f, 0.f};
    size_t orow = (size_t)am;
    if (epi_is_ln(EPI)) {
        cs = *reinterpret_cast<const f32x4*>(g.colsum + n);
        const int nseg = K >> 8;
        if (!g.ln_leaf_in) {
            const float* pp = g.ln_part_in + orow * 2 * nseg;
#pragma unroll
            for (int i = 0; i < 4; ++i)
                if (i < nseg) { part[2 * i] = pp[2 * i]; part[2 * i + 1] = pp[2 * i + 1]; }
        }
    } else if (EPI == EPI_PATCH_F32) {
        const int b_ = am / g.np, p_ = am - b_ * g.np;
        orow = (size_t)b_ * g.L + 1 + p_;
        add = *reinterpret_cast<const f32x4*>(g.pos + (size_t)(1 + p_) * g.N + n);
    } else if (EPI == EPI_BIAS_RESID_F32) {
        add = *reinterpret_cast<const f32x4*>(static_cast<const float*>(g.out) + orow * g.N + n);
    }
    uint2 xh = make_uint2(0u, 0u);
    unsigned xl = 0u;
    if (EPI == EPI_BIAS_RESID_LN_F32) {
        xh = *reinterpret_cast<const uint2*>(resid_hi(g.x3, orow, g.N) + n);
        xl = *reinterpret_cast<const unsigned*>(resid_lo(g.x3, orow, g.N) + n);
    }
    if (epi_is_ln(EPI) && g.ln_leaf_in) {
        const int nseg = K >> 8;
        const f32x2* lf = reinterpret_cast<const f32x2*>(g.ln_leaf_in) + orow * (size_t)(K >> 2) + fg;
#pragma unroll
        for (int j = 0; j < 4; ++j) {
            if (j < nseg) {
                f32x2 v[16];
#pragma unroll
                for (int t = 0; t < 16; ++t) v[t] = lf[64 * j + 4 * t];
                float sm[2];
#pragma unroll
                for (int c = 0; c < 2; ++c) {
                    float a[8], b[4];
#pragma unroll
                    for (int t = 0; t < 8; ++t) a[t] = v[t][c] + v[t + 8][c];
#pragma unroll
                    for (int t = 0; t < 4; ++t) b[t] = a[t] + a[t + 4];
                    const float c0 = b[0] + b[2], c1 = b[1] + b[3];
                    float d = c0 + c1;
                    d = lane_fold32(d, d);
                    sm[c] = lane_fold16(d, d);
                }
                part[2 * j] = sm[0];
                part[2 * j + 1] = sm[1];
            }
        }
    }

    f32x4 acc = {0.f, 0.f, 0.f, 0.f};
    bf16x8 wf[SKINNY_DEPTH], af[SKINNY_DEPTH];
#pragma unroll
    for (int d = 0; d < SKINNY_DEPTH; ++d) {
        const int s = d < nk ? d : nk - 1;
        wf[d] = wp[4 * s];
        af[d] = ap[4 * s];
    }
    for (int s0 = 0; s0 < nk; s0 += SKINNY_DEPTH) {
#pragma unroll
        for (int d = 0; d < SKINNY_DEPTH; ++d) {
            if (s0 + d < nk) acc = __builtin_amdgcn_mfma_f32_16x16x32_bf16(wf[d], af[d], acc, 0, 0, 0);
            int s = s0 + d + SKINNY_DEPTH;
            s = s < nk ? s : nk - 1;
            wf[d] = wp[4 * s];
            af[d] = ap[4 * s];
        }
    }

    f32x4 v;
    if (epi_is_ln(EPI)) {
        const f32x2 st = ln_row_stats(part, K >> 8, K);
        v = ln_apply(acc, st.x, st.y, cs, bz);
    } else {
        v = acc + bz;
    }
    if (epi_is_bf16_out(EPI)) {
        if (epi_is_qgelu(EPI)) v = quick_gelu4(v);
        if (valid)
            *reinterpret_cast<uint2*>(static_cast<unsigned short*>(g.out) + orow * g.N + n) =
                make_uint2(pack_bf16x2(v.x, v.y), pack_bf16x2(v.z, v.w));
        return;
    }
    if (EPI == EPI_BIAS_RESID_LN_F32) {
        const f32x4 o = v + split_join(xh, xl);
        uint2 nh;
        unsigned nl;
        split_make(o, nh, nl);
        if (valid) {
            *reinterpret_cast<uint2*>(resid_hi(g.x3, orow, g.N) + n) = nh;
            *reinterpret_cast<unsigned*>(resid_lo(g.x3, orow, g.N) + n) = nl;
            *reinterpret_cast<f32x2*>(g.ln_leaf + (orow * (size_t)(g.N >> 2) + (size_t)(n >> 2)) * 2) = f32x2{ln_lane_sum(o), ln_lane_sumsq(o)};
        }
        return;
    }
    if (EPI == EPI_PATCH_F32 || EPI == EPI_BIAS_RESID_F32) v += add;
    if (valid) *reinterpret_cast<f32x4*>(static_cast<float*>(g.out) + orow * g.N + n) = v;
}

}
```

### cli-p_amd/csrc/vit_kernels.hip

```cpp
#include "vit_kernels.hpp"
#include <hip/hip_ext.h>
#include <cstdlib>

namespace clipmi {

int launch_layernorm(const LnArgs& a, hipStream_t st) {
    if (a.M < 1) return 0;
    if (a.W % 4 != 0 || a.W > 1024) return set_err(CLIPMI_EINVAL, "layernorm: W=%d (need W %% 4 == 0, W <= 1024)", a.W);
    if (a.out_x3 && (a.W % 256 != 0 || !a.out_part)) return set_err(CLIPMI_EINVAL, "layernorm: split output needs W %% 256 == 0");
    hipLaunchKernelGGL(layernorm_kernel, dim3((a.M + 3) / 4), dim3(256), 0, st, a);
    CLIPMI_CHECK_LAUNCH("layernorm_kernel");
    return 0;
}

int launch_split_stats(const float* x_or_add, bool add, void* x3, float* part, int M, int W, hipStream_t st) {
    if (M < 1) return 0;
    if (!x_or_add || !x3 || !part || W % 256 != 0 || W < 256 || W > 1024)
        return set_err(CLIPMI_EINVAL, "split_stats: W=%d (need W %% 256 == 0, 256 <= W <= 1024)", W);
    if (add) hipLaunchKernelGGL(split_stats_kernel<true>, dim3((M + 3) / 4), dim3(256), 0, st, x_or_add, x3, part, M, W);
    else hipLaunchKernelGGL(split_stats_kernel<false>, dim3((M + 3) / 4), dim3(256), 0, st, x_or_add, x3, part, M, W);
    CLIPMI_CHECK_LAUNCH("split_stats_kernel");
    return 0;
}

template <int NT, bool CAUSAL, bool TR>
static int launch_attn_t(const unsigned short* qkv, unsigned short* out, int B, int L, int heads, hipStream_t st) {
    constexpr int KS = (NT + 1) / 2;
    const size_t lds = 4 * KS * 32 * 128;
    const long long items = (long long)B * heads;
    hipLaunchKernelGGL((attention_kernel<NT, CAUSAL, TR>), dim3((unsigned)((items + 3) / 4)), dim3(256), lds, st, qkv, out,
                       B, L, heads);
    CLIPMI_CHECK_LAUNCH("attention_kernel");
    return 0;
}

int launch_attention(const unsigned short* qkv, unsigned short* out, int B, int L, int heads, int causal, int tr,
                     hipStream_t st, unsigned char* out8, unsigned char* out_bs, bool* fused, hipEvent_t* probe_ev) {
    if (fused) *fused = false;
    if (B < 1) return 0;
    if (L < 1) return set_err(CLIPMI_EINVAL, "attention: L=%d", L);
    if (L > 80) {
        if (causal) return set_err(CLIPMI_EUNSUPPORTED, "attention: causal mask with L=%d > 80", L);
        const int qblocks = (L + 31) / 32;
        const int g4 = (qblocks + 3) / 4;
        const long long groups = (long long)B * heads * g4;
        hipLaunchKernelGGL((attention_flash_kernel<4, 2>), dim3((unsigned)groups), dim3(256), 2 * 16384, st, qkv, out, B, L, heads, g4);
        CLIPMI_CHECK_LAUNCH("attention_flash_kernel");
        return 0;
    }
    const int nt = (L + 15) / 16;
    static const int use52 = (int)dev_knob("CLIPMI_ATTN52", 2);
    if (L >= 49 && L <= 52 && !causal && tr == 1 && use52 == 2) {
        const long long items = (long long)B * heads;
        const long long resident = (long long)NUM_CU * 5;
        if (out8 && out_bs && fused) {
            hipLaunchKernelGGL(attention52x4_kernel<true>, dim3((unsigned)(items < resident ? items : resident)), dim3(256),
                               64 * 128 + 52 * 128, st, qkv, out, B, L, heads, out8, out_bs);
            *fused = true;
        } else if (probe_ev) {
            hipExtLaunchKernelGGL(attention52x4_kernel<false>, dim3((unsigned)(items < resident ? items : resident)), dim3(256),
                                  64 * 128 + 52 * 128, st, probe_ev[0], probe_ev[1], 0, qkv, out, B, L, heads, (unsigned char*)nullptr,
                                  (unsigned char*)nullptr);
        } else {
            hipLaunchKernelGGL(attention52x4_kernel<false>, dim3((unsigned)(items < resident ? items : resident)), dim3(256),
                               64 * 128 + 52 * 128, st, qkv, out, B, L, heads, (unsigned char*)nullptr, (unsigned char*)nullptr);
        }
        CLIPMI_CHECK_LAUNCH("attention52x4_kernel");
        return 0;
    }
    if (L >= 49 && L <= 52 && !causal && tr && use52) {
        const long long items = (long long)B * heads;
        const size_t lds = 4 * 52 * 128;
        hipLaunchKernelGGL(attention52_kernel, dim3((unsigned)((items + 3) / 4)), dim3(256), lds, st, qkv, out, B, L, heads);
        CLIPMI_CHECK_LAUNCH("attention52_kernel");
        return 0;
    }
#define ATT(NT_)                                                                                         \
    if (nt <= NT_) {                                                                                     \
        if (causal) return tr ? launch_attn_t<NT_, true, true>(qkv, out, B, L, heads, st)                \
                              : launch_attn_t<NT_, true, false>(qkv, out, B, L, heads, st);              \
        return tr ? launch_attn_t<NT_, false, true>(qkv, out, B, L, heads, st)                           \
                  : launch_attn_t<NT_, false, false>(qkv, out, B, L, heads, st);                         \
    }
    ATT(1) ATT(2) ATT(4) ATT(5)
#undef ATT
    return set_err(CLIPMI_EUNSUPPORTED, "attention: L=%d", L);
}

int launch_quantize_rows_fp8(const unsigned short* in, unsigned char* out, float* scale, int M, int K, hipStream_t st) {
    if (M < 1) return 0;
    if (K < 8 || K % 8 != 0 || !in || !out || !scale) return set_err(CLIPMI_EINVAL, "quantize_rows_fp8: K=%d", K);
    hipLaunchKernelGGL(quantize_rows_fp8_kernel, dim3((unsigned)((M + 3) / 4)), dim3(256), 0, st, in, out, scale, M, K);
    CLIPMI_CHECK_LAUNCH("quantize_rows_fp8_kernel");
    return 0;
}

int launch_quantize_rows_fp8mx(const unsigned short* in, unsigned char* out, unsigned char* bscale, int M, int K, hipStream_t st) {
    if (M < 1) return 0;
    if (K < 32 || K % 32 != 0 || !in || !out || !bscale) return set_err(CLIPMI_EINVAL, "quantize_rows_fp8mx: K=%d", K);
    hipLaunchKernelGGL(quantize_rows_fp8mx_kernel, dim3((unsigned)((M + 3) / 4)), dim3(256), 0, st, in, out, bscale, M, K);
    CLIPMI_CHECK_LAUNCH("quantize_rows_fp8mx_kernel");
    return 0;
}

#ifdef CLIPMI_DEV
int launch_rows_mx_stats(const float* x, unsigned char* x8, unsigned char* bs, float* part, int M, int W, hipStream_t st) {
    if (M < 1) return 0;
    if (W < 256 || W % 256 != 0 || !x || !x8 || !bs || !part) return set_err(CLIPMI_EINVAL, "rows_mx_stats: W=%d", W);
    hipLaunchKernelGGL(rows_mx_stats_kernel, dim3((unsigned)((M + 3) / 4)), dim3(256), 0, st, x, x8, bs, part, M, W);
    CLIPMI_CHECK_LAUNCH("rows_mx_stats_kernel");
    return 0;
}
#endif

int launch_patchify(const PatchArgs& a, hipStream_t st) {
    if (a.dtype == CLIPMI_U8 && a.P % 16 == 0 && a.R % 16 == 0 && a.patch_k == 3 * a.P * a.P && a.P * a.R <= 48 * 1024) {
        hipLaunchKernelGGL(patchify_strip_u8_kernel, dim3((unsigned)((long long)a.B * 3 * a.grid)), dim3(256), (size_t)a.P * a.R + 512, st, a);
        CLIPMI_CHECK_LAUNCH("patchify_strip_u8_kernel");
        return 0;
    }
    const long long total = (long long)a.B * a.np * (a.patch_k / 8);
    hipLaunchKernelGGL(patchify_kernel, dim3((unsigned)((total + 255) / 256)), dim3(256), 0, st, a);
    CLIPMI_CHECK_LAUNCH("patchify_kernel");
    return 0;
}

}

using namespace clipmi;

extern "C" int clipmi_dbg_layernorm(const float* x_dev, const float* w_dev, const float* b_dev, void* out_dev, int M,
                                    int W, int out_bf16, void* stream) {
    if (!x_dev || !w_dev || !b_dev || !out_dev) return set_err(CLIPMI_EINVAL, "dbg_layernorm: NULL pointer");
    LnArgs a{x_dev, w_dev, b_dev, out_dev, nullptr, 1, M, W, out_bf16};
    return launch_layernorm(a, as_stream(stream));
}

extern "C" int clipmi_dbg_attention(const void* qkv_dev, void* out_dev, int B, int L, int heads, int causal,
                                    void* stream) {
    if (!qkv_dev || !out_dev) return set_err(CLIPMI_EINVAL, "dbg_attention: NULL pointer");
    return launch_attention(static_cast<const unsigned short*>(qkv_dev), static_cast<unsigned short*>(out_dev), B, L,
                            heads, causal & 1, (causal & 2) ? 0 : ((causal & 4) ? 2 : 1), as_stream(stream));
}

extern "C" int clipmi_dbg_quantize_rows_fp8(const void* in_bf16_dev, void* out_fp8_dev, float* scale_dev, int M, int K,
                                            void* stream) {
    return launch_quantize_rows_fp8(static_cast<const unsigned short*>(in_bf16_dev), static_cast<unsigned char*>(out_fp8_dev),
                                    scale_dev, M, K, as_stream(stream));
}

extern "C" int clipmi_dbg_quantize_rows_fp8mx(const void* in_bf16_dev, void* out_fp8_dev, void* bscale_dev, int M, int K, void* stream) {
    return launch_quantize_rows_fp8mx(static_cast<const unsigned short*>(in_bf16_dev), static_cast<unsigned char*>(out_fp8_dev),
                                      static_cast<unsigned char*>(bscale_dev), M, K, as_stream(stream));
}

extern "C" int clipmi_dbg_split_stats(const float* x_dev, int add, void* x3_dev, float* part_dev, int M, int W, void* stream) {
    return launch_split_stats(x_dev, add != 0, x3_dev, part_dev, M, W, as_stream(stream));
}
```

### cli-p_amd/csrc/vit_kernels.hpp

```cpp
#pragma once
#include "gemm.hpp"

namespace clipmi {

struct PatchArgs {
    const void* pix;
    unsigned short* out;
    int dtype, B, R, P, grid, np, patch_k;
};

static __global__ void __launch_bounds__(256) patchify_kernel(PatchArgs a) {
    const long long total = (long long)a.B * a.np * (a.patch_k / 8);
    const long long i = (long long)blockIdx.x * 256 + threadIdx.x;
    if (i >= total) return;
    const int kc = a.patch_k / 8;
    const int k8 = (int)(i % kc);
    const long long bp = i / kc;
    const int p = (int)(bp % a.np);
    const int b = (int)(bp / a.np);
    const int PP = a.P * a.P;
    const float mean[3] = {0.48145466f, 0.4578275f, 0.40821073f};
    const float stdv[3] = {0.26862954f, 0.26130258f, 0.27577711f};
    float v[8];
    if ((a.P & 7) == 0 && (a.R & 7) == 0) {
        const int k = k8 * 8;
        if (k < 3 * PP) {
            const int c = k / PP, rem = k - c * PP;
            const int py = rem / a.P, px = rem - py * a.P;
            const int y = (p / a.grid) * a.P + py, xx = (p % a.grid) * a.P + px;
            const size_t src = (((size_t)b * 3 + c) * a.R + y) * a.R + xx;
            if (a.dtype == CLIPMI_F32) {
                const f32x4 lo = *reinterpret_cast<const f32x4*>(static_cast<const float*>(a.pix) + src);
                const f32x4 hi = *reinterpret_cast<const f32x4*>(static_cast<const float*>(a.pix) + src + 4);
                v[0] = lo.x; v[1] = lo.y; v[2] = lo.z; v[3] = lo.w; v[4] = hi.x; v[5] = hi.y; v[6] = hi.z; v[7] = hi.w;
            } else if (a.dtype == CLIPMI_BF16) {
                const uint4 raw = *reinterpret_cast<const uint4*>(static_cast<const unsigned short*>(a.pix) + src);
                const unsigned w[4] = {raw.x, raw.y, raw.z, raw.w};
#pragma unroll
                for (int j = 0; j < 4; ++j) {
                    v[2 * j] = __uint_as_float(w[j] << 16);
                    v[2 * j + 1] = __uint_as_float(w[j] & 0xffff0000u);
                }
            } else {
                const uint2 raw = *reinterpret_cast<const uint2*>(static_cast<const unsigned char*>(a.pix) + src);
                const float m = mean[c], s = stdv[c];
#pragma unroll
                for (int j = 0; j < 8; ++j) {
                    const unsigned byte = ((j < 4 ? raw.x : raw.y) >> (8 * (j & 3))) & 0xffu;
                    v[j] = ((float)byte / 255.0f - m) / s;
                }
            }
        } else {
#pragma unroll
            for (int j = 0; j < 8; ++j) v[j] = 0.f;
        }
    } else {
#pragma unroll
    for (int j = 0; j < 8; ++j) {
        const int k = k8 * 8 + j;
        float x = 0.f;
        if (k < 3 * PP) {
            const int c = k / PP, rem = k - c * PP;
            const int py = rem / a.P, px = rem - py * a.P;
            const int y = (p / a.grid) * a.P + py, xx = (p % a.grid) * a.P + px;
            const size_t src = (((size_t)b * 3 + c) * a.R + y) * a.R + xx;
            if (a.dtype == CLIPMI_F32) x = static_cast<const float*>(a.pix)[src];
            else if (a.dtype == CLIPMI_BF16) x = bf16_to_f32(static_cast<const unsigned short*>(a.pix)[src]);
            else x = ((float)static_cast<const unsigned char*>(a.pix)[src] / 255.0f - mean[c]) / stdv[c];
        }
        v[j] = x;
    }
    }
    uint4 o = make_uint4(pack_bf16x2(v[0], v[1]), pack_bf16x2(v[2], v[3]), pack_bf16x2(v[4], v[5]), pack_bf16x2(v[6], v[7]));
    *reinterpret_cast<uint4*>(a.out + ((size_t)bp * a.patch_k + k8 * 8)) = o;
}

static __global__ void __launch_bounds__(256) patchify_strip_u8_kernel(PatchArgs a) {
    extern __shared__ __attribute__((aligned(16))) char smem[];
    const int gy = blockIdx.x % a.grid;
    const int c = (blockIdx.x / a.grid) % 3;
    const int b = blockIdx.x / (3 * a.grid);
    const float mean[3] = {0.48145466f, 0.4578275f, 0.40821073f};
    const float stdv[3] = {0.26862954f, 0.26130258f, 0.27577711f};
    const float m = mean[c], sd = stdv[c];
    const unsigned char* src = static_cast<const unsigned char*>(a.pix) + (((size_t)b * 3 + c) * a.R + (size_t)gy * a.P) * a.R;
    unsigned short* lut = reinterpret_cast<unsigned short*>(smem + a.P * a.R);
    lut[threadIdx.x] = (unsigned short)(pack_bf16x2(((float)threadIdx.x / 255.0f - m) / sd, 0.f) & 0xffffu);
    const int nchunk = (a.P * a.R) >> 4;
    for (int j = threadIdx.x; j < nchunk; j += 256)
        *reinterpret_cast<uint4*>(smem + j * 16) = *reinterpret_cast<const uint4*>(src + (size_t)j * 16);
    __syncthreads();
    const int per_patch = (a.P * a.P) >> 3, per_row = a.P >> 3;
    for (int o = threadIdx.x; o < a.grid * per_patch; o += 256) {
        const int gx = o / per_patch, rem = o - gx * per_patch;
        const int y = rem / per_row, px = (rem - y * per_row) << 3;
        const uint2 raw = *reinterpret_cast<const uint2*>(smem + y * a.R + gx * a.P + px);
        unsigned w4[4];
#pragma unroll
        for (int k = 0; k < 4; ++k) {
            const unsigned word = k < 2 ? raw.x : raw.y;
            const unsigned b0 = (word >> (16 * (k & 1))) & 0xffu, b1 = (word >> (16 * (k & 1) + 8)) & 0xffu;
            w4[k] = (unsigned)lut[b0] | ((unsigned)lut[b1] << 16);
        }
        unsigned short* dst = a.out + ((size_t)b * a.np + gy * a.grid + gx) * a.patch_k + c * a.P * a.P + y * a.P + px;
        *reinterpret_cast<uint4*>(dst) = make_uint4(w4[0], w4[1], w4[2], w4[3]);
    }
}

static __global__ void __launch_bounds__(256) cls_rows_kernel(float* x, const float* cls, const float* pos, int B, int L, int W) {
    const long long i = (long long)blockIdx.x * 256 + threadIdx.x;
    if (i >= (long long)B * W) return;
    const int b = (int)(i / W), c = (int)(i - (long long)b * W);
    x[(size_t)b * L * W + c] = cls[c] + pos[c];
}

static __global__ void __launch_bounds__(256) gather_rows_kernel(const uint4* __restrict__ src, uint4* __restrict__ dst, int B,
                                                                 int row_step, int row16) {
    const long long i = (long long)blockIdx.x * 256 + threadIdx.x;
    if (i >= (long long)B * row16) return;
    const int b = (int)(i / row16), c = (int)(i - (long long)b * row16);
    dst[(size_t)b * row16 + c] = src[(size_t)b * row_step * row16 + c];
}

static __global__ void __launch_bounds__(256) text_embed_kernel(float* x, const int* ids, const float* tok, const float* pos,
                                                         int Q, int L, int W, int vocab) {
    const long long i = (long long)blockIdx.x * 256 + threadIdx.x;
    const int wc = W / 4;
    if (i >= (long long)Q * L * wc) return;
    const int c4 = (int)(i % wc);
    const long long row = i / wc;
    const int t = (int)(row % L);
    int id = ids[row];
    id = id < 0 ? 0 : (id >= vocab ? vocab - 1 : id);
    const f32x4 e = *reinterpret_cast<const f32x4*>(tok + (size_t)id * W + c4 * 4);
    const f32x4 p = *reinterpret_cast<const f32x4*>(pos + (size_t)t * W + c4 * 4);
    *reinterpret_cast<f32x4*>(x + (size_t)row * W + c4 * 4) = e + p;
}

static __global__ void eot_rows_kernel(const int* ids, int* rowidx, int Q, int L) {
    const int q = blockIdx.x * blockDim.x + threadIdx.x;
    if (q >= Q) return;
    int best = ids[(size_t)q * L], bi = 0;
    for (int t = 1; t < L; ++t) {
        const int v = ids[(size_t)q * L + t];
        if (v > best) { best = v; bi = t; }
    }
    rowidx[q] = q * L + bi;
}

struct LnArgs {
    const float* x;
    const float* w;
    const float* b;
    void* out;
    const int* rowidx;
    long long row_step;
    int M, W, out_bf16;
    unsigned char* out8;
    float* scale8;
    const void* x3;
    void* out_x3;
    float* out_part;
};

static __global__ void __launch_bounds__(256) layernorm_kernel(LnArgs a) {
    const int lane = threadIdx.x & 63;
    const int r = blockIdx.x * 4 + (threadIdx.x >> 6);
    if (r >= a.M) return;
    const long long src_row = a.rowidx ? (long long)a.rowidx[r] : (long long)r * a.row_step;
    const float* p = a.x + src_row * a.W;
    f32x4 v[4];
    float s = 0.f;
#pragma unroll
    for (int i = 0; i < 4; ++i) {
        const int c = i * 256 + lane * 4;
        v[i] = f32x4{0.f, 0.f, 0.f, 0.f};
        if (c < a.W) {
            if (a.x) v[i] = *reinterpret_cast<const f32x4*>(p + c);
            else v[i] = split_join(*reinterpret_cast<const uint2*>(resid_hi(a.x3, (size_t)src_row, a.W) + c),
                                   *reinterpret_cast<const unsigned*>(resid_lo(a.x3, (size_t)src_row, a.W) + c));
        }
        s += v[i].x + v[i].y + v[i].z + v[i].w;
    }
#pragma unroll
    for (int o = 32; o >= 1; o >>= 1) s += __shfl_xor(s, o);
    const float mean = s / (float)a.W;
    float q = 0.f;
#pragma unroll
    for (int i = 0; i < 4; ++i) {
        const int c = i * 256 + lane * 4;
        if (c < a.W) {
            const f32x4 d = v[i] - mean;
            q += d.x * d.x + d.y * d.y + d.z * d.z + d.w * d.w;
        }
    }
#pragma unroll
    for (int o = 32; o >= 1; o >>= 1) q += __shfl_xor(q, o);
    const float rstd = rsqrtf(q / (float)a.W + 1e-5f);
    if (a.out8) {
        float mx = 0.f;
#pragma unroll
        for (int i = 0; i < 4; ++i) {
            const int c = i * 256 + lane * 4;
            if (c < a.W) {
                const f32x4 g = *reinterpret_cast<const f32x4*>(a.w + c);
                const f32x4 bb = *reinterpret_cast<const f32x4*>(a.b + c);
                const f32x4 y = (v[i] - mean) * rstd * g + bb;
                const unsigned lo = pack_bf16x2(y.x, y.y), hi = pack_bf16x2(y.z, y.w);
                v[i] = f32x4{__uint_as_float(lo << 16), __uint_as_float(lo & 0xffff0000u), __uint_as_float(hi << 16),
                             __uint_as_float(hi & 0xffff0000u)};
                mx = fmaxf(fmaxf(mx, fabsf(v[i].x)), fmaxf(fabsf(v[i].y), fmaxf(fabsf(v[i].z), fabsf(v[i].w))));
            }
        }
#pragma unroll
        for (int o = 32; o >= 1; o >>= 1) mx = fmaxf(mx, __shfl_xor(mx, o));
        const float sc = mx > 0.f ? mx / 448.0f : 1.0f;
        const float inv = 1.0f / sc;
#pragma unroll
        for (int i = 0; i < 4; ++i) {
            const int c = i * 256 + lane * 4;
            if (c < a.W) {
                int pk = 0;
                pk = __builtin_amdgcn_cvt_pk_fp8_f32(v[i].x * inv, v[i].y * inv, pk, false);
                pk = __builtin_amdgcn_cvt_pk_fp8_f32(v[i].z * inv, v[i].w * inv, pk, true);
                *reinterpret_cast<unsigned*>(a.out8 + (size_t)r * a.W + c) = (unsigned)pk;
            }
        }
        if (lane == 0) a.scale8[r] = sc;
        return;
    }
    if (a.out_x3) {
        const int nseg = a.W >> 8;
#pragma unroll
        for (int i = 0; i < 4; ++i) {
            if (i < nseg) {
                const int c = i * 256 + lane * 4;
                const f32x4 g = *reinterpret_cast<const f32x4*>(a.w + c);
                const f32x4 bb = *reinterpret_cast<const f32x4*>(a.b + c);
                const f32x4 y = (v[i] - mean) * rstd * g + bb;
                uint2 nh;
                unsigned nl;
                split_make(y, nh, nl);
                *reinterpret_cast<uint2*>(resid_hi(a.out_x3, (size_t)r, a.W) + c) = nh;
                *reinterpret_cast<unsigned*>(resid_lo(a.out_x3, (size_t)r, a.W) + c) = nl;
                const float sa = ln_wave_sum(ln_lane_sum(y));
                const float sq = ln_wave_sum(ln_lane_sumsq(y));
                if (lane == 0) *reinterpret_cast<f32x2*>(a.out_part + ((size_t)r * nseg + i) * 2) = f32x2{sa, sq};
            }
        }
        return;
    }
#pragma unroll
    for (int i = 0; i < 4; ++i) {
        const int c = i * 256 + lane * 4;
        if (c < a.W) {
            const f32x4 g = *reinterpret_cast<const f32x4*>(a.w + c);
            const f32x4 bb = *reinterpret_cast<const f32x4*>(a.b + c);
            const f32x4 y = (v[i] - mean) * rstd * g + bb;
            if (a.out_bf16)
                *reinterpret_cast<uint2*>(static_cast<unsigned short*>(a.out) + (size_t)r * a.W + c) =
                    make_uint2(pack_bf16x2(y.x, y.y), pack_bf16x2(y.z, y.w));
            else
                *reinterpret_cast<f32x4*>(static_cast<float*>(a.out) + (size_t)r * a.W + c) = y;
        }
    }
}

template <bool ADD>
static __global__ void __launch_bounds__(256) split_stats_kernel(const float* __restrict__ x, void* x3, float* __restrict__ part,
                                                                 int M, int W) {
    const int lane = threadIdx.x & 63;
    const int r = blockIdx.x * 4 + (threadIdx.x >> 6);
    if (r >= M) return;
    const int nseg = W >> 8;
    const float* p = x + (size_t)r * W;
    unsigned short* const hrow = resid_hi(x3, (size_t)r, W);
    unsigned char* const lrow = resid_lo(x3, (size_t)r, W);
#pragma unroll
    for (int j = 0; j < 4; ++j) {
        if (j < nseg) {
            const int c = j * 256 + lane * 4;
            f32x4 v = *reinterpret_cast<const f32x4*>(p + c);
            if (ADD) v = v + split_join(*reinterpret_cast<const uint2*>(hrow + c), *reinterpret_cast<const unsigned*>(lrow + c));
            uint2 nh;
            unsigned nl;
            split_make(v, nh, nl);
            *reinterpret_cast<uint2*>(hrow + c) = nh;
            *reinterpret_cast<unsigned*>(lrow + c) = nl;
            const float sa = ln_wave_sum(ln_lane_sum(v));
            const float sq = ln_wave_sum(ln_lane_sumsq(v));
            if (lane == 0) *reinterpret_cast<f32x2*>(part + ((size_t)r * nseg + j) * 2) = f32x2{sa, sq};
        }
    }
}

static __global__ void __launch_bounds__(256) text_embed_split_kernel(const int* __restrict__ ids, const float* __restrict__ tok,
                                                                      const float* __restrict__ pos, void* x3, float* __restrict__ part,
                                                                      int* __restrict__ rowidx, int Q, int L, int W, int vocab) {
    const int M = Q * L, nrb = (M + 3) / 4;
    if ((int)blockIdx.x >= nrb) {
        for (int q = threadIdx.x; q < Q; q += 256) {
            int best = ids[(size_t)q * L], bi = 0;
            for (int t = 1; t < L; ++t) {
                const int v = ids[(size_t)q * L + t];
                if (v > best) { best = v; bi = t; }
            }
            rowidx[q] = q * L + bi;
        }
        return;
    }
    const int lane = threadIdx.x & 63;
    const int r = blockIdx.x * 4 + (threadIdx.x >> 6);
    if (r >= M) return;
    const int nseg = W >> 8, t = r % L;
    int id = ids[r];
    id = id < 0 ? 0 : (id >= vocab ? vocab - 1 : id);
    unsigned short* const hrow = resid_hi(x3, (size_t)r, W);
    unsigned char* const lrow = resid_lo(x3, (size_t)r, W);
#pragma unroll
    for (int j = 0; j < 4; ++j) {
        if (j < nseg) {
            const int c = j * 256 + lane * 4;
            const f32x4 v = *reinterpret_cast<const f32x4*>(tok + (size_t)id * W + c) + *reinterpret_cast<const f32x4*>(pos + (size_t)t * W + c);
            uint2 nh;
            unsigned nl;
            split_make(v, nh, nl);
            *reinterpret_cast<uint2*>(hrow + c) = nh;
            *reinterpret_cast<unsigned*>(lrow + c) = nl;
            const float sa = ln_wave_sum(ln_lane_sum(v));
            const float sq = ln_wave_sum(ln_lane_sumsq(v));
            if (lane == 0) *reinterpret_cast<f32x2*>(part + ((size_t)r * nseg + j) * 2) = f32x2{sa, sq};
        }
    }
}

typedef short s16x4 __attribute__((ext_vector_type(4)));

template <int NT, bool CAUSAL, bool TR>
__global__ void __launch_bounds__(256) attention_kernel(const unsigned short* __restrict__ qkv,
                                                        unsigned short* __restrict__ out, int B, int L, int heads) {
    extern __shared__ __attribute__((aligned(16))) char smem[];
    constexpr int KS = (NT + 1) / 2;
    constexpr int ROWS = KS * 32;
    const int lane = threadIdx.x & 63;
    const int wave = __builtin_amdgcn_readfirstlane(threadIdx.x >> 6);
    const int fr = lane & 15, fg = lane >> 4;
    const int W = heads * 64;
    const long long item = (long long)blockIdx.x * 4 + wave;
    if (item >= (long long)B * heads) return;
    const int b = (int)(item / heads), h = (int)(item - (long long)b * heads);
    const unsigned short* base = qkv + (size_t)b * L * 3 * W + h * 64;
    const size_t rs = (size_t)3 * W;
    char* vt = smem + wave * (ROWS * 128);

#pragma unroll
    for (int i = 0; i < ROWS / 8; ++i) {
        int row = i * 8 + (lane >> 3);
        const int srcrow = row < L ? row : L - 1;
        const uint4 d = *reinterpret_cast<const uint4*>(base + (size_t)srcrow * rs + 2 * W + (lane & 7) * 8);
        *reinterpret_cast<uint4*>(vt + row * 128 + (lane & 7) * 16) = d;
    }

    bf16x8 kf[NT][2], qf[NT][2];
#pragma unroll
    for (int t = 0; t < NT; ++t) {
        int row = t * 16 + fr;
        row = row < L ? row : L - 1;
        const unsigned short* pr = base + (size_t)row * rs + fg * 8;
        qf[t][0] = *reinterpret_cast<const bf16x8*>(pr);
        qf[t][1] = *reinterpret_cast<const bf16x8*>(pr + 32);
        kf[t][0] = *reinterpret_cast<const bf16x8*>(pr + W);
        kf[t][1] = *reinterpret_cast<const bf16x8*>(pr + W + 32);
    }
    f32x4 s[NT][NT];
#pragma unroll
    for (int kt = 0; kt < NT; ++kt)
#pragma unroll
        for (int qt = 0; qt < NT; ++qt) {
            f32x4 a = {0.f, 0.f, 0.f, 0.f};
            a = __builtin_amdgcn_mfma_f32_16x16x32_bf16(kf[kt][0], qf[qt][0], a, 0, 0, 0);
            a = __builtin_amdgcn_mfma_f32_16x16x32_bf16(kf[kt][1], qf[qt][1], a, 0, 0, 0);
            s[kt][qt] = a;
        }

#pragma unroll
    for (int qt = 0; qt < NT; ++qt) {
        const int qi = qt * 16 + fr;
        float mx = -INFINITY;
#pragma unroll
        for (int kt = 0; kt < NT; ++kt)
#pragma unroll
            for (int r = 0; r < 4; ++r) {
                const int ki = kt * 16 + 4 * fg + r;
                float x = s[kt][qt][r] * 0.125f;
                if (ki >= L || (CAUSAL && ki > qi)) x = -INFINITY;
                s[kt][qt][r] = x;
                mx = fmaxf(mx, x);
            }
        mx = fmaxf(mx, __shfl_xor(mx, 16));
        mx = fmaxf(mx, __shfl_xor(mx, 32));
        float sum = 0.f;
#pragma unroll
        for (int kt = 0; kt < NT; ++kt)
#pragma unroll
            for (int r = 0; r < 4; ++r) {
                const float e = __expf(s[kt][qt][r] - mx);
                s[kt][qt][r] = e;
                sum += e;
            }
        sum += __shfl_xor(sum, 16);
        sum += __shfl_xor(sum, 32);
        const float inv = 1.0f / sum;
#pragma unroll
        for (int kt = 0; kt < NT; ++kt) s[kt][qt] *= inv;
    }

    asm volatile("s_waitcnt lgkmcnt(0)" ::: "memory");
    __builtin_amdgcn_wave_barrier();
    f32x4 o[4][NT];
#pragma unroll
    for (int dt = 0; dt < 4; ++dt)
#pragma unroll
        for (int qt = 0; qt < NT; ++qt) o[dt][qt] = f32x4{0.f, 0.f, 0.f, 0.f};
#pragma unroll
    for (int ks = 0; ks < KS; ++ks) {
        bf16x8 pf[NT];
#pragma unroll
        for (int qt = 0; qt < NT; ++qt) {
            const f32x4 lo = s[2 * ks][qt];
            f32x4 hi = {0.f, 0.f, 0.f, 0.f};
            if (2 * ks + 1 < NT) hi = s[2 * ks + 1 < NT ? 2 * ks + 1 : 0][qt];
            const uint4 u = make_uint4(pack_bf16x2(lo.x, lo.y), pack_bf16x2(lo.z, lo.w), pack_bf16x2(hi.x, hi.y),
                                       pack_bf16x2(hi.z, hi.w));
            pf[qt] = __builtin_bit_cast(bf16x8, u);
        }
#pragma unroll
        for (int dt = 0; dt < 4; ++dt) {
            bf16x8 vf;
            if (TR) {
                const int k0 = 32 * ks + 4 * fg + (fr >> 2);
                const char* ad = vt + k0 * 128 + (dt * 16 + 4 * (fr & 3)) * 2;
                const s16x4 t0 = __builtin_amdgcn_ds_read_tr16_b64_v4i16((__attribute__((address_space(3))) s16x4*)(ad));
                const s16x4 t1 = __builtin_amdgcn_ds_read_tr16_b64_v4i16((__attribute__((address_space(3))) s16x4*)(ad + 16 * 128));
                typedef short s16x8 __attribute__((ext_vector_type(8)));
                const s16x8 t = {t0.x, t0.y, t0.z, t0.w, t1.x, t1.y, t1.z, t1.w};
                vf = __builtin_bit_cast(bf16x8, t);
            } else {
                unsigned short e[8];
#pragma unroll
                for (int j = 0; j < 8; ++j) {
                    const int key = 16 * (2 * ks + (j >> 2)) + 4 * fg + (j & 3);
                    e[j] = *reinterpret_cast<const unsigned short*>(vt + key * 128 + (dt * 16 + fr) * 2);
                }
                const uint4 u = make_uint4(e[0] | ((unsigned)e[1] << 16), e[2] | ((unsigned)e[3] << 16),
                                           e[4] | ((unsigned)e[5] << 16), e[6] | ((unsigned)e[7] << 16));
                vf = __builtin_bit_cast(bf16x8, u);
            }
#pragma unroll
            for (int qt = 0; qt < NT; ++qt)
                o[dt][qt] = __builtin_amdgcn_mfma_f32_16x16x32_bf16(vf, pf[qt], o[dt][qt], 0, 0, 0);
        }
    }

#pragma unroll
    for (int qt = 0; qt < NT; ++qt) {
        const int qi = qt * 16 + fr;
        if (qi >= L) continue;
        unsigned short* dst = out + ((size_t)b * L + qi) * W + h * 64 + 4 * fg;
#pragma unroll
        for (int dt = 0; dt < 4; ++dt) {
            const f32x4 v = o[dt][qt];
            *reinterpret_cast<uint2*>(dst + dt * 16) = make_uint2(pack_bf16x2(v.x, v.y), pack_bf16x2(v.z, v.w));
        }
    }
}

static __global__ void __launch_bounds__(256) quantize_rows_fp8_kernel(const unsigned short* __restrict__ in,
                                                                       unsigned char* __restrict__ out,
                                                                       float* __restrict__ scale, int M, int K) {
    const int lane = threadIdx.x & 63;
    const long long r = (long long)blockIdx.x * 4 + (threadIdx.x >> 6);
    if (r >= M) return;
    const unsigned short* x = in + (size_t)r * K;
    float mx = 0.f;
    for (int k = lane * 8; k < K; k += 512) {
        const uint4 v = *reinterpret_cast<const uint4*>(x + k);
        const unsigned w[4] = {v.x, v.y, v.z, v.w};
#pragma unroll
        for (int j = 0; j < 4; ++j)
            mx = fmaxf(mx, fmaxf(fabsf(__uint_as_float(w[j] << 16)), fabsf(__uint_as_float(w[j] & 0xffff0000u))));
    }
#pragma unroll
    for (int o = 32; o >= 1; o >>= 1) mx = fmaxf(mx, __shfl_xor(mx, o));
    const float s = mx > 0.f ? mx / 448.0f : 1.0f;
    const float inv = 1.0f / s;
    for (int k = lane * 8; k < K; k += 512) {
        const uint4 v = *reinterpret_cast<const uint4*>(x + k);
        const unsigned w[4] = {v.x, v.y, v.z, v.w};
        float f[8];
#pragma unroll
        for (int j = 0; j < 4; ++j) {
            f[2 * j] = __uint_as_float(w[j] << 16) * inv;
            f[2 * j + 1] = __uint_as_float(w[j] & 0xffff0000u) * inv;
        }
        int lo = 0, hi = 0;
        lo = __builtin_amdgcn_cvt_pk_fp8_f32(f[0], f[1], lo, false);
        lo = __builtin_amdgcn_cvt_pk_fp8_f32(f[2], f[3], lo, true);
        hi = __builtin_amdgcn_cvt_pk_fp8_f32(f[4], f[5], hi, false);
        hi = __builtin_amdgcn_cvt_pk_fp8_f32(f[6], f[7], hi, true);
        *reinterpret_cast<uint2*>(out + (size_t)r * K + k) = make_uint2((unsigned)lo, (unsigned)hi);
    }
    if (lane == 0) scale[r] = s;
}

static __global__ void __launch_bounds__(256) quantize_rows_fp8mx_kernel(const unsigned short* __restrict__ in,
                                                                         unsigned char* __restrict__ out,
                                                                         unsigned char* __restrict__ bscale, int M, int K) {
    const int lane = threadIdx.x & 63;
    const long long r = (long long)blockIdx.x * 4 + (threadIdx.x >> 6);
    if (r >= M) return;
    const unsigned short* x = in + (size_t)r * K;
    for (int k0 = 0; k0 < K; k0 += 512) {
        const int k = k0 + lane * 8;
        const bool on = k < K;
        float f[8] = {0.f, 0.f, 0.f, 0.f, 0.f, 0.f, 0.f, 0.f};
        if (on) {
            const uint4 v = *reinterpret_cast<const uint4*>(x + k);
            const unsigned w[4] = {v.x, v.y, v.z, v.w};
#pragma unroll
            for (int j = 0; j < 4; ++j) {
                f[2 * j] = __uint_as_float(w[j] << 16);
                f[2 * j + 1] = __uint_as_float(w[j] & 0xffff0000u);
            }
        }
        float mx = 0.f;
#pragma unroll
        for (int j = 0; j < 8; ++j) mx = fmaxf(mx, fabsf(f[j]));
        mx = fmaxf(mx, __shfl_xor(mx, 1));
        mx = fmaxf(mx, __shfl_xor(mx, 2));
        const unsigned sb = fp8mx_scale_byte(mx);
        const float inv = fp8mx_inv(sb);
#pragma unroll
        for (int j = 0; j < 8; ++j) f[j] *= inv;
        if (on) {
            *reinterpret_cast<uint2*>(out + (size_t)r * K + k) = fp8_pack8(f);
            if ((lane & 3) == 0) bscale[(size_t)r * (K >> 5) + (k >> 5)] = (unsigned char)sb;
        }
    }
}

static __global__ void __launch_bounds__(256) rows_mx_stats_kernel(const float* __restrict__ x, unsigned char* __restrict__ x8,
                                                                   unsigned char* __restrict__ bs, float* __restrict__ part,
                                                                   int M, int W) {
    const int lane = threadIdx.x & 63;
    const long long r = (long long)blockIdx.x * 4 + (threadIdx.x >> 6);
    if (r >= M) return;
    const int nseg = W >> 8;
    for (int sg = 0; sg < nseg; ++sg) {
        const size_t col = (size_t)sg * 256 + lane * 4;
        const f32x4 v = *reinterpret_cast<const f32x4*>(x + (size_t)r * W + col);
        unsigned p4, sb;
        float sm, sq;
        ln8_row_segment(v, p4, sb, sm, sq);
        *reinterpret_cast<unsigned*>(x8 + (size_t)r * W + col) = p4;
        if ((lane & 7) == 0) bs[(size_t)r * (W >> 5) + (col >> 5)] = (unsigned char)sb;
        if (lane == 0) *reinterpret_cast<f32x2*>(part + ((size_t)r * nseg + sg) * 2) = f32x2{sm, sq};
    }
}

static __global__ void __launch_bounds__(256, 6) attention52_kernel(const unsigned short* __restrict__ qkv,
                                                                    unsigned short* __restrict__ out, int B, int L,
                                                                    int heads) {
    extern __shared__ __attribute__((aligned(16))) char smem[];
    constexpr int NT = 4, ROWS = 52;
    const int lane = threadIdx.x & 63;
    const int wave = __builtin_amdgcn_readfirstlane(threadIdx.x >> 6);
    const int fr = lane & 15, fg = lane >> 4;
    const int W = heads * 64;
    const long long item = (long long)blockIdx.x * 4 + wave;
    if (item >= (long long)B * heads) return;
    const int b = (int)(item / heads), h = (int)(item - (long long)b * heads);
    const unsigned short* base = qkv + (size_t)b * L * 3 * W + h * 64;
    const size_t rs = (size_t)3 * W;
    char* vt = smem + wave * (ROWS * 128);

#pragma unroll
    for (int i = 0; i < 7; ++i) {
        const int row = i * 8 + (lane >> 3);
        const int srcrow = row < L ? row : L - 1;
        const uint4 d = *reinterpret_cast<const uint4*>(base + (size_t)srcrow * rs + 2 * W + (lane & 7) * 8);
        if (row < ROWS) *reinterpret_cast<uint4*>(vt + row * 128 + (lane & 7) * 16) = d;
    }
    bf16x8 kf[NT][2];
#pragma unroll
    for (int t = 0; t < NT; ++t) {
        int row = t * 16 + fr;
        row = row < L ? row : L - 1;
        const unsigned short* pr = base + (size_t)row * rs + W + fg * 8;
        kf[t][0] = *reinterpret_cast<const bf16x8*>(pr);
        kf[t][1] = *reinterpret_cast<const bf16x8*>(pr + 32);
    }
    auto q_ptr = [&](int qt) {
        int row = qt * 16 + fr;
        row = row < L ? row : L - 1;
        return base + (size_t)row * rs + fg * 8;
    };
    bf16x8 qn0 = *reinterpret_cast<const bf16x8*>(q_ptr(0));
    bf16x8 qn1 = *reinterpret_cast<const bf16x8*>(q_ptr(0) + 32);
    const int k00 = 4 * fg + (fr >> 2);
    const int krow[4] = {k00, k00 + 16, k00 + 32, (k00 + 48 < ROWS ? k00 + 48 : ROWS - 1)};
    const char* vcol = vt + (4 * (fr & 3)) * 2;
    asm volatile("s_waitcnt lgkmcnt(0)" ::: "memory");
    __builtin_amdgcn_wave_barrier();

#pragma unroll 1
    for (int qt = 0; qt < NT; ++qt) {
        const bf16x8 q0 = qn0, q1 = qn1;
        if (qt + 1 < NT) {
            qn0 = *reinterpret_cast<const bf16x8*>(q_ptr(qt + 1));
            qn1 = *reinterpret_cast<const bf16x8*>(q_ptr(qt + 1) + 32);
        }
        f32x4 s[NT];
#pragma unroll
        for (int kt = 0; kt < NT; ++kt) {
            f32x4 a = {0.f, 0.f, 0.f, 0.f};
            a = __builtin_amdgcn_mfma_f32_16x16x32_bf16(kf[kt][0], q0, a, 0, 0, 0);
            a = __builtin_amdgcn_mfma_f32_16x16x32_bf16(kf[kt][1], q1, a, 0, 0, 0);
            s[kt] = a;
        }
        float mx = -INFINITY;
#pragma unroll
        for (int kt = 0; kt < NT; ++kt)
#pragma unroll
            for (int r = 0; r < 4; ++r) {
                const int ki = kt * 16 + 4 * fg + r;
                float x = s[kt][r] * 0.125f;
                if (ki >= L) x = -INFINITY;
                s[kt][r] = x;
                mx = fmaxf(mx, x);
            }
        mx = fmaxf(mx, __shfl_xor(mx, 16));
        mx = fmaxf(mx, __shfl_xor(mx, 32));
        float sum = 0.f;
#pragma unroll
        for (int kt = 0; kt < NT; ++kt)
#pragma unroll
            for (int r = 0; r < 4; ++r) {
                const float e = __expf(s[kt][r] - mx);
                s[kt][r] = e;
                sum += e;
            }
        sum += __shfl_xor(sum, 16);
        sum += __shfl_xor(sum, 32);
        const float inv = 1.0f / sum;
#pragma unroll
        for (int kt = 0; kt < NT; ++kt) s[kt] *= inv;

        f32x4 o[4];
#pragma unroll
        for (int dt = 0; dt < 4; ++dt) o[dt] = f32x4{0.f, 0.f, 0.f, 0.f};
#pragma unroll
        for (int ks = 0; ks < 2; ++ks) {
            const f32x4 lo = s[2 * ks], hi = s[2 * ks + 1];
            const uint4 u = make_uint4(pack_bf16x2(lo.x, lo.y), pack_bf16x2(lo.z, lo.w), pack_bf16x2(hi.x, hi.y),
                                       pack_bf16x2(hi.z, hi.w));
            const bf16x8 pf = __builtin_bit_cast(bf16x8, u);
#pragma unroll
            for (int dt = 0; dt < 4; ++dt) {
                const s16x4 t0 = __builtin_amdgcn_ds_read_tr16_b64_v4i16(
                    (__attribute__((address_space(3))) s16x4*)(vcol + krow[2 * ks] * 128 + dt * 32));
                const s16x4 t1 = __builtin_amdgcn_ds_read_tr16_b64_v4i16(
                    (__attribute__((address_space(3))) s16x4*)(vcol + krow[2 * ks + 1] * 128 + dt * 32));
                typedef short s16x8 __attribute__((ext_vector_type(8)));
                const s16x8 t = {t0.x, t0.y, t0.z, t0.w, t1.x, t1.y, t1.z, t1.w};
                o[dt] = __builtin_amdgcn_mfma_f32_16x16x32_bf16(__builtin_bit_cast(bf16x8, t), pf, o[dt], 0, 0, 0);
            }
        }
        const int qi = qt * 16 + fr;
        if (qi < L) {
            unsigned short* dst = out + ((size_t)b * L + qi) * W + h * 64 + 4 * fg;
#pragma unroll
            for (int dt = 0; dt < 4; ++dt)
                *reinterpret_cast<uint2*>(dst + dt * 16) = make_uint2(pack_bf16x2(o[dt].x, o[dt].y), pack_bf16x2(o[dt].z, o[dt].w));
        }
    }
}

template <bool OUT8>
static __global__ void __launch_bounds__(256, 5) attention52x4_kernel(const unsigned short* __restrict__ qkv,
                                                                      unsigned short* __restrict__ out, int B, int L,
                                                                      int heads, unsigned char* __restrict__ out8, unsigned char* __restrict__ out_bs) {
    extern __shared__ __attribute__((aligned(16))) char smem[];
    constexpr int NT = 4, ROWS = 52;
    const int lane = threadIdx.x & 63;
    const int wave = __builtin_amdgcn_readfirstlane(threadIdx.x >> 6);
    const int fr = lane & 15, fg = lane >> 4;
    const int W = heads * 64;
    const size_t rs = (size_t)3 * W;
    char* kt_ = smem;
    char* vt = smem + 64 * 128;
    const int srow = lane >> 3, sch = lane & 7;
    const int items = B * heads;

    bf16x8 q0n, q1n;
    uint4 kdn0, kdn1, vdn0, vdn1;
#define ATT52_FETCH(IT)                                                                                  \
    do {                                                                                                 \
        const int b_ = (IT) / heads, h_ = (IT) - b_ * heads;                                             \
        const unsigned short* base_ = qkv + (size_t)b_ * L * 3 * W + h_ * 64;                            \
        int qrow_ = wave * 16 + fr;                                                                      \
        qrow_ = qrow_ < L ? qrow_ : L - 1;                                                               \
        const unsigned short* qp_ = base_ + (size_t)qrow_ * rs + fg * 8;                                 \
        q0n = *reinterpret_cast<const bf16x8*>(qp_);                                                     \
        q1n = *reinterpret_cast<const bf16x8*>(qp_ + 32);                                                \
        int r0_ = (wave * 2) * 8 + srow, r1_ = (wave * 2 + 1) * 8 + srow;    \
        r0_ = r0_ < L ? r0_ : L - 1;                                         \
        r1_ = r1_ < L ? r1_ : L - 1;                                                                     \
        kdn0 = *reinterpret_cast<const uint4*>(base_ + (size_t)r0_ * rs + W + sch * 8);                  \
        vdn0 = *reinterpret_cast<const uint4*>(base_ + (size_t)r0_ * rs + 2 * W + sch * 8);              \
        kdn1 = *reinterpret_cast<const uint4*>(base_ + (size_t)r1_ * rs + W + sch * 8);                  \
        vdn1 = *reinterpret_cast<const uint4*>(base_ + (size_t)r1_ * rs + 2 * W + sch * 8);              \
    } while (0)
    int item = blockIdx.x;
    if (item >= items) return;
    ATT52_FETCH(item);
    for (;;) {
        const int b = item / heads, h = item - b * heads;
        const bf16x8 q0 = q0n, q1 = q1n;
        {
            const int row0 = (wave * 2) * 8 + srow, row1 = row0 + 8;
            *reinterpret_cast<uint4*>(kt_ + row0 * 128 + ((sch ^ (row0 & 7)) << 4)) = kdn0;
            *reinterpret_cast<uint4*>(kt_ + row1 * 128 + ((sch ^ (row1 & 7)) << 4)) = kdn1;
            if (row0 < ROWS) *reinterpret_cast<uint4*>(vt + row0 * 128 + sch * 16) = vdn0;
            if (row1 < ROWS) *reinterpret_cast<uint4*>(vt + row1 * 128 + sch * 16) = vdn1;
        }
        const int nxt = item + gridDim.x;
        const bool has_next = nxt < items;
        if (has_next) ATT52_FETCH(nxt);
        __syncthreads();

    bf16x8 kf[NT][2];
#pragma unroll
    for (int t = 0; t < NT; ++t) {
        const int row = t * 16 + fr;
        kf[t][0] = *reinterpret_cast<const bf16x8*>(kt_ + row * 128 + (((0 + fg) ^ (row & 7)) << 4));
        kf[t][1] = *reinterpret_cast<const bf16x8*>(kt_ + row * 128 + (((4 + fg) ^ (row & 7)) << 4));
    }
    const int k00 = 4 * fg + (fr >> 2);
    const int krow[4] = {k00, k00 + 16, k00 + 32, (k00 + 48 < ROWS ? k00 + 48 : ROWS - 1)};
    const char* vcol = vt + (4 * (fr & 3)) * 2;

    f32x4 s[NT];
#pragma unroll
    for (int kt = 0; kt < NT; ++kt) {
        f32x4 a = {0.f, 0.f, 0.f, 0.f};
        a = __builtin_amdgcn_mfma_f32_16x16x32_bf16(kf[kt][0], q0, a, 0, 0, 0);
        a = __builtin_amdgcn_mfma_f32_16x16x32_bf16(kf[kt][1], q1, a, 0, 0, 0);
        s[kt] = a;
    }
    float mx = -INFINITY;
#pragma unroll
    for (int kt = 0; kt < NT; ++kt)
#pragma unroll
        for (int r = 0; r < 4; ++r) {
            const int ki = kt * 16 + 4 * fg + r;
            float x = s[kt][r] * 0.125f;
            if (ki >= L) x = -INFINITY;
            s[kt][r] = x;
            mx = fmaxf(mx, x);
        }
    mx = fmaxf(mx, __shfl_xor(mx, 16));
    mx = fmaxf(mx, __shfl_xor(mx, 32));
    float sum = 0.f;
#pragma unroll
    for (int kt = 0; kt < NT; ++kt)
#pragma unroll
        for (int r = 0; r < 4; ++r) {
            const float e = __expf(s[kt][r] - mx);
            s[kt][r] = e;
            sum += e;
        }
    sum += __shfl_xor(sum, 16);
    sum += __shfl_xor(sum, 32);
    const float inv = 1.0f / sum;
#pragma unroll
    for (int kt = 0; kt < NT; ++kt) s[kt] *= inv;

    f32x4 o[4];
#pragma unroll
    for (int dt = 0; dt < 4; ++dt) o[dt] = f32x4{0.f, 0.f, 0.f, 0.f};
#pragma unroll
    for (int ks = 0; ks < 2; ++ks) {
        const f32x4 lo = s[2 * ks], hi = s[2 * ks + 1];
        const uint4 u = make_uint4(pack_bf16x2(lo.x, lo.y), pack_bf16x2(lo.z, lo.w), pack_bf16x2(hi.x, hi.y),
                                   pack_bf16x2(hi.z, hi.w));
        const bf16x8 pf = __builtin_bit_cast(bf16x8, u);
#pragma unroll
        for (int dt = 0; dt < 4; ++dt) {
            const s16x4 t0 = __builtin_amdgcn_ds_read_tr16_b64_v4i16(
                (__attribute__((address_space(3))) s16x4*)(vcol + krow[2 * ks] * 128 + dt * 32));
            const s16x4 t1 = __builtin_amdgcn_ds_read_tr16_b64_v4i16(
                (__attribute__((address_space(3))) s16x4*)(vcol + krow[2 * ks + 1] * 128 + dt * 32));
            typedef short s16x8 __attribute__((ext_vector_type(8)));
            const s16x8 t = {t0.x, t0.y, t0.z, t0.w, t1.x, t1.y, t1.z, t1.w};
            o[dt] = __builtin_amdgcn_mfma_f32_16x16x32_bf16(__builtin_bit_cast(bf16x8, t), pf, o[dt], 0, 0, 0);
        }
    }
    const int qi = wave * 16 + fr;
    uint2 pk[4];
#pragma unroll
    for (int dt = 0; dt < 4; ++dt) pk[dt] = make_uint2(pack_bf16x2(o[dt].x, o[dt].y), pack_bf16x2(o[dt].z, o[dt].w));
    const bool odd = fg & 1;
    uint2 mine[2], theirs[2];
#pragma unroll
    for (int j = 0; j < 2; ++j) {
        const uint2 give = odd ? pk[2 * j] : pk[2 * j + 1];
        mine[j] = odd ? pk[2 * j + 1] : pk[2 * j];
        theirs[j] = make_uint2(__shfl_xor(give.x, 16), __shfl_xor(give.y, 16));
    }
    if (OUT8) {
#pragma unroll
        for (int j = 0; j < 2; ++j) {
            const int dt = 2 * j + (odd ? 1 : 0);
            const uint4 v = odd ? make_uint4(theirs[j].x, theirs[j].y, mine[j].x, mine[j].y)
                                : make_uint4(mine[j].x, mine[j].y, theirs[j].x, theirs[j].y);
            const unsigned w_[4] = {v.x, v.y, v.z, v.w};
            float f[8];
            float mxa = 0.f;
#pragma unroll
            for (int i = 0; i < 4; ++i) {
                f[2 * i] = __uint_as_float(w_[i] << 16);
                f[2 * i + 1] = __uint_as_float(w_[i] & 0xffff0000u);
                mxa = fmaxf(mxa, fmaxf(fabsf(f[2 * i]), fabsf(f[2 * i + 1])));
            }
            mxa = fmaxf(mxa, __shfl_xor(mxa, 16));
            mxa = fmaxf(mxa, __shfl_xor(mxa, 32));
            const unsigned sb_ = fp8mx_scale_byte(mxa);
            const float inv_ = fp8mx_inv(sb_);
#pragma unroll
            for (int i = 0; i < 8; ++i) f[i] *= inv_;
            if (qi < L) {
                const size_t row_ = (size_t)b * L + qi;
                *reinterpret_cast<uint2*>(out8 + row_ * W + h * 64 + 4 * (fg & ~1) + dt * 16) = fp8_pack8(f);
                if (fg == 0) out_bs[row_ * (W >> 5) + h * 2 + j] = (unsigned char)sb_;
            }
        }
    } else if (qi < L) {
        unsigned short* dst = out + ((size_t)b * L + qi) * W + h * 64 + 4 * (fg & ~1);
#pragma unroll
        for (int j = 0; j < 2; ++j) {
            const int dt = 2 * j + (odd ? 1 : 0);
            const uint4 v = odd ? make_uint4(theirs[j].x, theirs[j].y, mine[j].x, mine[j].y)
                                : make_uint4(mine[j].x, mine[j].y, theirs[j].x, theirs[j].y);
            *reinterpret_cast<uint4*>(dst + dt * 16) = v;
        }
    }
        if (!has_next) break;
        item = nxt;
        __syncthreads();
    }
#undef ATT52_FETCH
}

template <int WPB, int QT>
__global__ void __launch_bounds__(WPB * 64, QT == 2 ? 4 : 2) attention_flash_kernel(const unsigned short* __restrict__ qkv,
                                                                    unsigned short* __restrict__ out, int B, int L,
                                                                    int heads, int qgroups) {
    extern __shared__ __attribute__((aligned(16))) char smem[];
    constexpr int NT = 4;
    const int tid = threadIdx.x;
    const int lane = tid & 63;
    const int wave = __builtin_amdgcn_readfirstlane(tid >> 6);
    const int fr = lane & 15, fg = lane >> 4;
    const int W = heads * 64;
    const int qgi = blockIdx.x % qgroups;
    const int bh = blockIdx.x / qgroups;
    const int b = bh / heads, h = bh - b * heads;
    const unsigned short* base = qkv + (size_t)b * L * 3 * W + h * 64;
    const size_t rs = (size_t)3 * W;
    const int q0 = (qgi * WPB + wave) * (16 * QT);
    const bool wave_active = q0 < L;

    bf16x8 qf[QT][2];
#pragma unroll
    for (int t = 0; t < QT; ++t) {
        int row = q0 + t * 16 + fr;
        row = row < L ? row : L - 1;
        const unsigned short* pr = base + (size_t)row * rs + fg * 8;
        qf[t][0] = *reinterpret_cast<const bf16x8*>(pr);
        qf[t][1] = *reinterpret_cast<const bf16x8*>(pr + 32);
    }
    f32x4 o[4][QT];
#pragma unroll
    for (int dt = 0; dt < 4; ++dt)
#pragma unroll
        for (int qt = 0; qt < QT; ++qt) o[dt][qt] = f32x4{0.f, 0.f, 0.f, 0.f};
    float m_run[QT], l_run[QT];
#pragma unroll
    for (int qt = 0; qt < QT; ++qt) { m_run[qt] = -INFINITY; l_run[qt] = 0.f; }

    constexpr int PPW = 16 / WPB;
    static_assert(PPW <= 8, "a wave's pieces are all K or all V");
    const int pc0 = wave * PPW, isv0 = pc0 >> 3;
    const int row0 = (pc0 & 7) * 8 + (lane >> 3);
    const unsigned short* const src0 = base + (size_t)row0 * rs + (1 + isv0) * W + (isv0 ? (lane & 7) : ((lane & 7) ^ (row0 & 7))) * 8;
    auto issue_tiles = [&](int k0, int buf) {
        if (k0 + 64 <= L) {
#pragma unroll
            for (int i = 0; i < PPW; ++i) {
                const size_t uoff = (size_t)((unsigned)(k0 + 8 * i) * (unsigned)rs);
                __builtin_amdgcn_global_load_lds((const __attribute__((address_space(1))) void*)(src0 + uoff),
                                                 (__attribute__((address_space(3))) void*)(smem + buf * 16384 + (pc0 + i) * 1024), 16, 0, 0);
            }
        } else {
            asm volatile("" ::: "memory");
#pragma unroll
            for (int i = 0; i < PPW; ++i) {
                int row = k0 + row0 + 8 * i;
                row = row < L ? row : L - 1;
                const unsigned short* src = src0 + (size_t)((unsigned)(row - row0) * (unsigned)rs);
                __builtin_amdgcn_global_load_lds((const __attribute__((address_space(1))) void*)src,
                                                 (__attribute__((address_space(3))) void*)(smem + buf * 16384 + (pc0 + i) * 1024), 16, 0, 0);
            }
        }
    };
    issue_tiles(0, 0);

    const float c = 0.125f * 1.4426950408889634f;
    const int nb = (L + 63) >> 6;
    auto block = [&](auto mask_tag, int j) {
        constexpr bool MASK = decltype(mask_tag)::value;
        const int k0 = j << 6;
        asm volatile("s_waitcnt vmcnt(0)" ::: "memory");
        __syncthreads();
        if (j + 1 < nb) issue_tiles(k0 + 64, (j + 1) & 1);
        const char* kb = smem + (j & 1) * 16384;
        const char* vt = kb + 8192;
        if (wave_active) {
            f32x4 s[NT][QT];
#pragma unroll
            for (int hf = 0; hf < 2; ++hf)
#pragma unroll
                for (int kt = 0; kt < NT; ++kt) {
                    const int row = kt * 16 + fr;
                    const bf16x8 kf = *reinterpret_cast<const bf16x8*>(kb + row * 128 + (((4 * hf + fg) ^ (row & 7)) << 4));
#pragma unroll
                    for (int qt = 0; qt < QT; ++qt)
                        s[kt][qt] = __builtin_amdgcn_mfma_f32_16x16x32_bf16(kf, qf[qt][hf], hf ? s[kt][qt] : f32x4{0.f, 0.f, 0.f, 0.f},
                                                                            0, 0, 0);
                }
            if constexpr (MASK) {
#pragma unroll
                for (int qt = 0; qt < QT; ++qt)
#pragma unroll
                    for (int kt = 0; kt < NT; ++kt)
#pragma unroll
                        for (int r = 0; r < 4; ++r)
                            if (k0 + kt * 16 + 4 * fg + r >= L) s[kt][qt][r] = -INFINITY;
            }
#pragma unroll
            for (int qt = 0; qt < QT; ++qt) {
                float mx = -INFINITY;
#pragma unroll
                for (int kt = 0; kt < NT; ++kt)
#pragma unroll
                    for (int r = 0; r < 4; ++r) mx = fmaxf(mx, s[kt][qt][r]);
                mx = fmaxf(mx, __shfl_xor(mx, 16));
                mx = fmaxf(mx, __shfl_xor(mx, 32));
                mx *= c;
                const float m_new = fmaxf(m_run[qt], mx);
                const float alpha = __builtin_amdgcn_exp2f(m_run[qt] - m_new);
                float sum = 0.f;
#pragma unroll
                for (int kt = 0; kt < NT; ++kt)
#pragma unroll
                    for (int r = 0; r < 4; ++r) {
                        const float e = __builtin_amdgcn_exp2f(fmaf(s[kt][qt][r], c, -m_new));
                        s[kt][qt][r] = e;
                        sum += e;
                    }
                sum += __shfl_xor(sum, 16);
                sum += __shfl_xor(sum, 32);
                l_run[qt] = l_run[qt] * alpha + sum;
                m_run[qt] = m_new;
                if (__ballot(alpha != 1.0f)) {
#pragma unroll
                    for (int dt = 0; dt < 4; ++dt) o[dt][qt] *= alpha;
                }
            }
#pragma unroll
            for (int ks = 0; ks < 2; ++ks) {
                bf16x8 pf[QT];
#pragma unroll
                for (int qt = 0; qt < QT; ++qt) {
                    const f32x4 lo = s[2 * ks][qt], hi = s[2 * ks + 1][qt];
                    const uint4 u = make_uint4(pack_bf16x2(lo.x, lo.y), pack_bf16x2(lo.z, lo.w), pack_bf16x2(hi.x, hi.y),
                                               pack_bf16x2(hi.z, hi.w));
                    pf[qt] = __builtin_bit_cast(bf16x8, u);
                }
#pragma unroll
                for (int dt = 0; dt < 4; ++dt) {
                    const int kk = 32 * ks + 4 * fg + (fr >> 2);
                    const char* ad = vt + kk * 128 + (dt * 16 + 4 * (fr & 3)) * 2;
                    const s16x4 t0 = __builtin_amdgcn_ds_read_tr16_b64_v4i16((__attribute__((address_space(3))) s16x4*)(ad));
                    const s16x4 t1 = __builtin_amdgcn_ds_read_tr16_b64_v4i16((__attribute__((address_space(3))) s16x4*)(ad + 16 * 128));
                    typedef short s16x8 __attribute__((ext_vector_type(8)));
                    const s16x8 t = {t0.x, t0.y, t0.z, t0.w, t1.x, t1.y, t1.z, t1.w};
                    const bf16x8 vf = __builtin_bit_cast(bf16x8, t);
#pragma unroll
                    for (int qt = 0; qt < QT; ++qt)
                        o[dt][qt] = __builtin_amdgcn_mfma_f32_16x16x32_bf16(vf, pf[qt], o[dt][qt], 0, 0, 0);
                }
            }
        }
    };
    for (int j = 0; j + 1 < nb; ++j) block(std::false_type{}, j);
    if ((nb << 6) > L) block(std::true_type{}, nb - 1);
    else block(std::false_type{}, nb - 1);

    if (!wave_active) return;
#pragma unroll
    for (int qt = 0; qt < QT; ++qt) {
        const int qi = q0 + qt * 16 + fr;
        if (qi >= L) continue;
        const float inv = 1.0f / l_run[qt];
        unsigned short* dst = out + ((size_t)b * L + qi) * W + h * 64 + 4 * fg;
#pragma unroll
        for (int dt = 0; dt < 4; ++dt) {
            const f32x4 v = o[dt][qt] * inv;
            *reinterpret_cast<uint2*>(dst + dt * 16) = make_uint2(pack_bf16x2(v.x, v.y), pack_bf16x2(v.z, v.w));
        }
    }
}

int launch_layernorm(const LnArgs& a, hipStream_t st);
int launch_attention(const unsigned short* qkv, unsigned short* out, int B, int L, int heads, int causal, int tr,
                     hipStream_t st, unsigned char* out8 = nullptr, unsigned char* out_bs = nullptr, bool* fused = nullptr,
                     hipEvent_t* probe_ev = nullptr);
int launch_patchify(const PatchArgs& a, hipStream_t st);
int launch_quantize_rows_fp8(const unsigned short* in, unsigned char* out, float* scale, int M, int K, hipStream_t st);
int launch_quantize_rows_fp8mx(const unsigned short* in, unsigned char* out, unsigned char* bscale, int M, int K, hipStream_t st);
int launch_rows_mx_stats(const float* x, unsigned char* x8, unsigned char* bs, float* part, int M, int W, hipStream_t st);

}
```

### include/clipmi.h

```cpp
#ifndef CLIPMI_H
#define CLIPMI_H

#include <stddef.h>
#include <stdint.h>

#ifdef __cplusplus
extern "C" {
#endif

#define CLIPMI_ABI_VERSION 8

enum {
    CLIPMI_OK = 0,
    CLIPMI_EINVAL = 1,
    CLIPMI_EWORKSPACE = 2,
    CLIPMI_EHIP = 3,
    CLIPMI_EUNSUPPORTED = 4
};

enum {
    CLIPMI_F32 = 0,
    CLIPMI_BF16 = 1,
    CLIPMI_U8 = 2
};

typedef struct clipmi_tower {
    int32_t abi_version;
    int32_t kind;
    int32_t width;
    int32_t layers;
    int32_t heads;
    int32_t mlp;
    int32_t embed;
    int32_t tokens;
    int32_t patch;
    int32_t res;
    int32_t patch_k;
    int32_t vocab;

    uint64_t blob_bytes;

    uint64_t off_patch_w, off_cls, off_pos, off_ln_pre_w, off_ln_pre_b;
    uint64_t off_tok_emb;

    uint64_t off_layers, layer_stride;
    uint64_t lo_ln1_w, lo_ln1_b;
    uint64_t lo_qkv_w, lo_qkv_b;
    uint64_t lo_out_w, lo_out_b;
    uint64_t lo_ln2_w, lo_ln2_b;
    uint64_t lo_fc_w, lo_fc_b;
    uint64_t lo_proj_w, lo_proj_b;

    uint64_t off_ln_post_w, off_ln_post_b, off_out_proj;

    int32_t weight_format, ln_fold;
    uint64_t lo_qkv_s, lo_out_s, lo_fc_s, lo_proj_s;

    uint64_t lo_qkv_colsum, lo_qkv_cb, lo_fc_colsum, lo_fc_cb;
} clipmi_tower;

size_t clipmi_encode_image_workspace_bytes(const clipmi_tower* t, int B);
int clipmi_encode_image(const clipmi_tower* t, const void* blob_dev,
                        const void* pixels_dev, int pix_dtype, int B,
                        float* out_dev, int normalize,
                        void* ws_dev, size_t ws_bytes, void* stream);

size_t clipmi_encode_text_workspace_bytes(const clipmi_tower* t, int Q);
int clipmi_encode_text(const clipmi_tower* t, const void* blob_dev,
                       const int32_t* ids_dev, int Q,
                       float* out_dev, int normalize,
                       void* ws_dev, size_t ws_bytes, void* stream);

size_t clipmi_topk_ip_workspace_bytes(int64_t N, int E, int Q, int K);
int clipmi_topk_ip(const void* db_dev, int db_dtype, int64_t N, int E,
                   const float* q_dev, int Q, int K, int64_t id_base,
                   float* out_score_dev, int64_t* out_id_dev,
                   void* ws_dev, size_t ws_bytes, void* stream);

size_t clipmi_topk_ip_coarse_workspace_bytes(int64_t N, int E, int Q, int K);
int clipmi_topk_ip_coarse(const void* db_dev, const void* db_bf16_dev, int64_t N, int E, float rmax,
                          const float* q_dev, int Q, int K, int64_t id_base,
                          float* out_score_dev, int64_t* out_id_dev,
                          void* ws_dev, size_t ws_bytes, void* stream);

int clipmi_rows_stats(const float* db_dev, int64_t N, int E, const float* meta_dev, float* stats2_dev, void* stream);
int clipmi_rows_to_bf16(const float* db_dev, int64_t N, int E, void* out_bf16_dev, void* stream);
size_t clipmi_i8_copy_bytes(int64_t N, int E);
size_t clipmi_i8_meta_bytes(int64_t N);
int clipmi_quantize_rows_i8(const float* db_dev, int64_t N, int E, const uint32_t* perm_dev, void* out_i8_dev, size_t out_i8_bytes,
                            float* meta_dev, size_t meta_bytes, void* stream);
int clipmi_rows_absmax(const float* db_dev, int64_t N, int E, float* out_dev, void* stream);
size_t clipmi_rows_order_workspace_bytes(int64_t N);
int clipmi_rows_order_by_absmax(const float* db_dev, int64_t N, int E, uint32_t* perm_dev, void* ws_dev, size_t ws_bytes, void* stream);
int clipmi_topk_ip_coarse_i8(const void* db_dev, const void* db_i8_dev, const float* meta_dev, float amax,
                             int64_t N, int E, float rmax, const float* q_dev, int Q, int K, int64_t id_base,
                             float* out_score_dev, int64_t* out_id_dev,
                             void* ws_dev, size_t ws_bytes, void* stream);
size_t clipmi_topk_ip_wide_workspace_bytes(int64_t N, int E, int Q, int K);
int clipmi_topk_ip_wide_i8(const void* db_dev, const void* db_i8_dev, const float* meta_dev, float amax,
                           int64_t N, int E, float rmax, const float* q_dev, int Q, int K, int64_t id_base,
                           float* out_score_dev, int64_t* out_id_dev,
                           void* ws_dev, size_t ws_bytes, void* stream);

size_t clipmi_merge_topk_workspace_bytes(int R, int Q, int K);
int clipmi_merge_topk(const float* scores_dev, const int64_t* ids_dev, int R, int Q, int K,
                      float* out_score_dev, int64_t* out_id_dev,
                      void* ws_dev, size_t ws_bytes, void* stream);

int clipmi_merge_topk_packed(const void* gathered_dev, size_t record_bytes, int R, int Q, int K,
                             float* out_score_dev, int64_t* out_id_dev, void* stream);

int clipmi_l2_normalize_rows(float* x_dev, int64_t n, int E, void* stream);

typedef struct clipmi_resize_job {
    int64_t src_off;
    int32_t w, h;
    int32_t r0, nrows;
    int32_t out_index;
    int32_t need_h, need_v;
    int32_t left, top;
    int32_t hk, vk;
    int64_t hcoef_off, vcoef_off;
    int64_t tmp_off;
} clipmi_resize_job;
int clipmi_resize_crop_rgb8(const void* raw_dev, const void* jobs_dev, int njobs, int max_rows, const int32_t* coef_dev,
                            int n_px, void* out_dev, void* scratch_dev, void* stream);

typedef struct clipmi_jpeg_image {
    int64_t stream_off;
    int64_t coef_off;
    int64_t out_off;
    int64_t intervals_off;
    int32_t stream_bytes;
    int32_t width, height;
    int32_t ncomp;
    int32_t hs, vs;
    int32_t dc_tbl[3], ac_tbl[3];
    int32_t restart_interval;
    int32_t n_intervals;
    int32_t stuffed;
    int32_t reserved;
    uint8_t quant[3][64];
} clipmi_jpeg_image;
int64_t clipmi_jpeg_workspace_bytes(int64_t total_blocks, int ntables);
int clipmi_jpeg_decode_rgb8(void* streams_dev, void* images_dev, int n, const void* tables_dev, int ntables,
                            int64_t total_blocks, int64_t max_blocks, int64_t max_pixels, void* out_dev, int32_t* status_dev,
                            void* ws_dev, int64_t ws_bytes, void* stream);

typedef struct clipmi_jpeg_scan {
    int64_t stream_off;
    int32_t stream_bytes;
    int32_t ncomp;
    int32_t comp[3];
    int32_t tbl[3];
    int32_t ss, se, ah, al;
    int32_t reserved[2];
} clipmi_jpeg_scan;
typedef struct clipmi_jpeg_progressive_image {
    int64_t coef_off;
    int64_t out_off;
    int32_t width, height;
    int32_t ncomp;
    int32_t hs, vs;
    int32_t first_scan;
    int32_t n_scans;
    int32_t reserved[5];
    uint8_t quant[3][64];
} clipmi_jpeg_progressive_image;
int64_t clipmi_jpeg_progressive_workspace_bytes(int n, int64_t total_blocks, int ntables);
int clipmi_jpeg_decode_progressive_rgb8(const void* streams_dev, const void* images_dev, int n, const void* scans_dev, int nscans,
                                        const void* tables_dev, int ntables, int64_t total_blocks, int64_t max_blocks,
                                        int64_t max_pixels, void* out_dev, int32_t* status_dev, void* ws_dev, int64_t ws_bytes,
                                        void* stream);

const char* clipmi_last_error(void);
int clipmi_abi_version(void);

int clipmi_dbg_gemm_bf16(const void* a_dev, const void* w_dev, const float* bias_dev,
                         void* out_dev, int M, int N, int K, int epi, void* stream);
int clipmi_dbg_layernorm(const float* x_dev, const float* w_dev, const float* b_dev,
                         void* out_dev, int M, int W, int out_bf16, void* stream);
int clipmi_dbg_attention(const void* qkv_dev, void* out_dev, int B, int L, int heads,
                         int causal, void* stream);

int clipmi_dbg_topk_scan_ms(const void* db_dev, int64_t N, int E, const float* q_dev, int Q, int K,
                            float* out_score_dev, int64_t* out_id_dev, void* ws_dev, size_t ws_bytes,
                            void* stream, int reps, float* scan_ms);

int clipmi_dbg_topk_coarse_scan_ms(const void* db_dev, const void* db_bf16_dev, int64_t N, int E, float rmax,
                                   const float* q_dev, int Q, int K, float* out_score_dev, int64_t* out_id_dev,
                                   void* ws_dev, size_t ws_bytes, void* stream, int reps, float* scan_ms,
                                   long long* survivors );

int clipmi_dbg_topk_coarse_i8_scan_ms(const void* db_dev, const void* db_i8_dev, const float* meta_dev, float amax,
                                      int64_t N, int E, float rmax, const float* q_dev, int Q, int K,
                                      float* out_score_dev, int64_t* out_id_dev, void* ws_dev, size_t ws_bytes,
                                      void* stream, int reps, float* scan_ms, long long* survivors);

int clipmi_dbg_topk_wide_i8_scan_ms(const void* db_dev, const void* db_i8_dev, const float* meta_dev, float amax,
                                    int64_t N, int E, float rmax, const float* q_dev, int Q, int K,
                                    float* out_score_dev, int64_t* out_id_dev, void* ws_dev, size_t ws_bytes,
                                    void* stream, int reps, float* scan_ms, long long* survivors, int* scan_launches,
                                    int* fallback_armed);

int clipmi_dbg_quantize_rows_fp8(const void* in_bf16_dev, void* out_fp8_dev, float* scale_dev, int M, int K, void* stream);
int clipmi_dbg_gemm_fp8(const void* a8_dev, const void* w8_dev, const float* a_scale_dev, const float* w_scale_dev,
                        const float* bias_dev, void* out_dev, int M, int N, int K, int epi, void* stream);

int clipmi_dbg_split_stats(const float* x_dev, int add, void* x3_dev, float* part_dev, int M, int W, void* stream);
int clipmi_dbg_gemm_ln(const void* x3_dev, const void* wg_dev, const float* cb_dev, const float* colsum_dev,
                       const float* part_dev, void* out_dev, int M, int N, int K, int epi, void* stream);
int clipmi_dbg_quantize_rows_fp8mx(const void* in_bf16_dev, void* out_fp8_dev, void* bscale_dev, int M, int K, void* stream);
int clipmi_dbg_gemm_fp8_bsa(const void* a8_dev, const void* w8_dev, const void* a_bscale_dev, const float* w_scale_dev,
                            const float* bias_dev, void* out_dev, int M, int N, int K, int epi, void* stream);
int clipmi_dbg_gemm_resid_ln_leaf(const void* a_dev, const void* w_dev, const float* bias_dev, void* x3_dev, float* leaf_dev,
                                  int M, int N, int K, void* stream);
int clipmi_dbg_gemm_ln_leaf(const void* x3_dev, const void* wg_dev, const float* cb_dev, const float* colsum_dev,
                            const float* leaf_dev, void* out_dev, int M, int N, int K, int epi, void* stream);
int clipmi_dbg_gemm_resid_ln(const void* a_dev, const void* w_dev, const float* bias_dev, void* x3_dev, float* part_dev,
                             float* tmp_dev, int M, int N, int K, int algo, void* stream);

int clipmi_dbg_encode_image_probe_ms(const clipmi_tower* t, const void* blob_dev, const void* pixels_dev,
                                     int pix_dtype, int B, float* out_dev, void* ws_dev, size_t ws_bytes,
                                     void* stream, int probe_epi, int reps, float* kernel_ms, int* launches);

int clipmi_dbg_encode_image_probe3_ms(const clipmi_tower* t, const void* blob_dev, const void* pixels_dev,
                                      int pix_dtype, int B, float* out_dev, void* ws_dev, size_t ws_bytes,
                                      void* stream, int probe_epi, int reps, float* ms3, int* launches,
                                      int* kernel_kind, int* epi_ran);

#ifdef __cplusplus
}
#endif
#endif
```

Baseline: 108,100.

## Compute only CLS-token queries in last-layer attention and add wide skinny GEMM

In the final encoder layer only the CLS token is pooled, so the QKV projection is split: K/V are computed for all tokens while Q is computed only for the gathered CLS rows. A CLS-query variant of the attention kernel then attends one query per image. A new wide skinny GEMM kernel handles tail GEMMs with up to 1024 rows, and the gather kernel also copies LN partial statistics. This cuts the Q projection and attention work in the last layer, at the cost of extra launches, idle waves in the CLS attention kernel, and more code-path complexity.

```diff
diff --git a/cli-p_amd/_lib.py b/cli-p_amd/_lib.py
--- a/cli-p_amd/_lib.py
+++ b/cli-p_amd/_lib.py
@@ -18,7 +18,7 @@
     "clipmi_dbg_quantize_rows_fp8", "clipmi_dbg_gemm_fp8",
     "clipmi_merge_topk_workspace_bytes", "clipmi_merge_topk", "clipmi_merge_topk_packed",
     "clipmi_l2_normalize_rows", "clipmi_resize_crop_rgb8", "clipmi_jpeg_workspace_bytes", "clipmi_jpeg_decode_rgb8", "clipmi_jpeg_progressive_workspace_bytes", "clipmi_jpeg_decode_progressive_rgb8", "clipmi_last_error", "clipmi_abi_version",
-    "clipmi_dbg_gemm_bf16", "clipmi_dbg_layernorm", "clipmi_dbg_attention", "clipmi_dbg_topk_scan_ms",
+    "clipmi_dbg_gemm_bf16", "clipmi_dbg_layernorm", "clipmi_dbg_attention", "clipmi_dbg_attention_cls", "clipmi_dbg_topk_scan_ms",
     "clipmi_dbg_encode_image_probe_ms", "clipmi_dbg_encode_image_probe3_ms",
     "clipmi_dbg_split_stats", "clipmi_dbg_gemm_ln", "clipmi_dbg_gemm_resid_ln", "clipmi_dbg_gemm_resid_ln_leaf", "clipmi_dbg_gemm_ln_leaf", "clipmi_dbg_quantize_rows_fp8mx", "clipmi_dbg_gemm_fp8_bsa",
 ]
@@ -154,6 +154,8 @@
     L.clipmi_dbg_layernorm.argtypes = [vp, vp, vp, vp, i32, i32, i32, vp]
     L.clipmi_dbg_attention.restype = i32
     L.clipmi_dbg_attention.argtypes = [vp, vp, i32, i32, i32, i32, vp]
+    L.clipmi_dbg_attention_cls.restype = i32
+    L.clipmi_dbg_attention_cls.argtypes = [vp, vp, vp, i32, i32, i32, vp]
     L.clipmi_dbg_topk_scan_ms.restype = i32
     L.clipmi_dbg_topk_scan_ms.argtypes = [vp, i64, i32, vp, i32, i32, vp, vp, vp, sz, vp, i32, C.POINTER(C.c_float)]
     L.clipmi_dbg_encode_image_probe_ms.restype = i32
diff --git a/cli-p_amd/csrc/encode.hip b/cli-p_amd/csrc/encode.hip
--- a/cli-p_amd/csrc/encode.hip
+++ b/cli-p_amd/csrc/encode.hip
@@ -53,7 +53,7 @@
         if (t->ln_fold) {
             w.x3c = ar.take<unsigned char>((size_t)B * resid_row_bytes(W));
             w.partc = ar.take<float>((size_t)B * 2 * (W / 256));
-            if (B <= SKINNY_MAX_M) w.leafc = ar.take<float>((size_t)B * 2 * (W / 4));
+            if (B <= TAIL_SKINNY_MAX_M) w.leafc = ar.take<float>((size_t)B * 2 * (W / 4));
         } else {
             w.xc = ar.take<float>((size_t)B * W);
         }
@@ -92,16 +92,30 @@
     return reinterpret_cast<const T*>(static_cast<const char*>(blob) + off);
 }
 
-bool encode_tail() {
+int encode_tail() {
     static const int mode = (int)dev_knob("CLIPMI_ENCODE_TAIL", 1);
-    return mode != 0;
-}
-
-int launch_gather_rows(const void* src, void* dst, int B, int L, size_t row_bytes, hipStream_t st) {
-    if (row_bytes % 16 != 0) return set_err(CLIPMI_EINVAL, "gather_rows: %zu bytes per row", row_bytes);
-    const int row16 = (int)(row_bytes / 16);
-    hipLaunchKernelGGL(gather_rows_kernel, dim3((unsigned)(((long long)B * row16 + 255) / 256)), dim3(256), 0, st,
-                       static_cast<const uint4*>(src), static_cast<uint4*>(dst), B, L, row16);
+    return mode;
+}
+bool tail_cls_query(int M, int W) {
+    static const int mode = (int)dev_knob("CLIPMI_ENCODE_CLSQ", 1);
+    if (mode == 0 || encode_tail() == 3) return false;
+    if (mode == 2) return true;
+    const long long rt = (M + 255) / 256, kv = rt * (2 * W / 256), qkv = rt * (3 * W / 256);
+    return kv > NUM_CU && (kv + NUM_CU - 1) / NUM_CU < (qkv + NUM_CU - 1) / NUM_CU;
+}
+int tail_skinny_rows() {
+    static const long long rows = dev_knob("CLIPMI_TAIL_SKINNY", TAIL_SKINNY_MAX_M);
+    return encode_tail() == 3 || rows < 0 ? 0 : (int)(rows < TAIL_SKINNY_MAX_M ? rows : TAIL_SKINNY_MAX_M);
+}
+
+int launch_gather_rows(const void* src, void* dst, int B, int L, size_t row_bytes, hipStream_t st, const void* ssrc = nullptr,
+                       void* sdst = nullptr, size_t srow_bytes = 0) {
+    if (row_bytes % 16 != 0 || srow_bytes % 8 != 0 || (srow_bytes && (!ssrc || !sdst)))
+        return set_err(CLIPMI_EINVAL, "gather_rows: %zu + %zu bytes per row", row_bytes, srow_bytes);
+    const int row16 = (int)(row_bytes / 16), srow8 = (int)(srow_bytes / 8);
+    hipLaunchKernelGGL(gather_rows_kernel, dim3((unsigned)(((long long)B * (row16 + srow8) + 255) / 256)), dim3(256), 0, st,
+                       static_cast<const uint4*>(src), static_cast<uint4*>(dst), B, L, row16, static_cast<const uint2*>(ssrc),
+                       static_cast<uint2*>(sdst), srow8);
     CLIPMI_CHECK_LAUNCH("gather_rows_kernel");
     return 0;
 }
@@ -110,7 +124,7 @@
                bool* pruned = nullptr) {
     const int W = t->width, L = t->tokens, M = B * L;
     const bool fp8 = t->weight_format == 1;
-    const bool tail = pruned && !causal && !fp8 && (t->ln_fold ? w.x3c != nullptr : w.xc != nullptr) && encode_tail();
+    const bool tail = pruned && !causal && !fp8 && (t->ln_fold ? w.x3c != nullptr : w.xc != nullptr) && encode_tail() != 0;
     if (pruned) *pruned = tail;
     auto linear = [&](const unsigned short* A, int K, uint64_t w_off, uint64_t b_off, void* out, int N, int epi) -> int {
         GemmArgs g{};
@@ -162,14 +176,14 @@
         auto lb_of = [&](int l) { return t->off_layers + (uint64_t)l * t->layer_stride; };
         const bool leaf_mode = w.ln_leaf != nullptr && gemm_resid_writes_leaves(M, W, W) && gemm_resid_writes_leaves(M, W, 4 * W);
         bool leaves = false;
-        auto ln_linear = [&](uint64_t w_off, uint64_t cb_off, uint64_t cs_off, int N, int epi) -> int {
+        auto ln_linear = [&](uint64_t w_off, uint64_t cb_off, uint64_t cs_off, int N, int epi, GemmProbe* pr) -> int {
             GemmArgs g{};
             g.A = static_cast<const unsigned short*>(w.x3); g.lda_bytes = (unsigned)resid_row_bytes(W);
             g.W = at<unsigned short>(blob, w_off); g.bias = at<float>(blob, cb_off);
             g.colsum = at<float>(blob, cs_off); g.ln_part_in = w.ln_part;
             if (leaves) g.ln_leaf_in = w.ln_leaf;
             g.out = w.big; g.M = M; g.N = N; g.K = W;
-            return launch_gemm_algo(g, epi, 0, st, probe);
+            return launch_gemm_algo(g, epi, 0, st, pr);
         };
         auto resid_linear = [&](const unsigned short* A, int K, uint64_t w_off, uint64_t b_off) -> int {
             GemmArgs g{};
@@ -181,20 +195,41 @@
         };
         for (int l = 0; l < t->layers; ++l) {
             const uint64_t lb = lb_of(l);
-            if (int rc = ln_linear(lb + t->lo_qkv_w, lb + t->lo_qkv_cb, lb + t->lo_qkv_colsum, 3 * W, EPI_LN_BIAS_BF16)) return rc;
             if (tail && l == t->layers - 1) {
+                const int srows = tail_skinny_rows();
                 const bool tleaf = w.leafc != nullptr && gemm_resid_writes_leaves(B, W, W) && gemm_resid_writes_leaves(B, W, 4 * W);
-                if (int rc = launch_attention(w.big, w.h, B, L, t->heads, causal, 1, st)) return rc;
-                if (int rc = launch_gather_rows(w.x3, w.x3c, B, L, resid_row_bytes(W), st)) return rc;
-                auto tail_resid = [&](const unsigned short* A, unsigned lda_bytes, int K, uint64_t w_off, uint64_t b_off) -> int {
+                const bool wide = !tleaf && w.leafc != nullptr && gemm_resid_writes_leaves(B, W, 4 * W, srows);
+                const bool clsq = tail_cls_query(M, W) && attention_cls_ok(L);
+                unsigned out_lda = 0u;
+                if (clsq) {
+                    if (int rc = leaves ? launch_gather_rows(w.x3, w.x3c, B, L, resid_row_bytes(W), st, w.ln_leaf, w.leafc, (size_t)2 * W)
+                                        : launch_gather_rows(w.x3, w.x3c, B, L, resid_row_bytes(W), st, w.ln_part, w.partc, (size_t)8 * (W / 256)))
+                        return rc;
+                    if (int rc = ln_linear(lb + t->lo_qkv_w + (uint64_t)W * W * 2, lb + t->lo_qkv_cb + (uint64_t)W * 4,
+                                           lb + t->lo_qkv_colsum + (uint64_t)W * 4, 2 * W, EPI_LN_BIAS_BF16, nullptr)) return rc;
+                    GemmArgs q{};
+                    q.A = static_cast<const unsigned short*>(w.x3c); q.lda_bytes = (unsigned)resid_row_bytes(W);
+                    q.W = at<unsigned short>(blob, lb + t->lo_qkv_w); q.bias = at<float>(blob, lb + t->lo_qkv_cb);
+                    q.colsum = at<float>(blob, lb + t->lo_qkv_colsum); q.ln_part_in = w.partc;
+                    if (leaves) q.ln_leaf_in = w.leafc;
+                    q.out = w.pooled; q.M = B; q.N = W; q.K = W; q.skinny_rows = srows;
+                    if (int rc = launch_gemm_algo(q, EPI_LN_BIAS_BF16, 0, st, nullptr)) return rc;
+                    if (int rc = launch_attention_cls(w.pooled, w.big, w.h, B, L, t->heads, st)) return rc;
+                } else {
+                    if (int rc = ln_linear(lb + t->lo_qkv_w, lb + t->lo_qkv_cb, lb + t->lo_qkv_colsum, 3 * W, EPI_LN_BIAS_BF16, probe)) return rc;
+                    if (int rc = launch_attention(w.big, w.h, B, L, t->heads, causal, 1, st)) return rc;
+                    if (int rc = launch_gather_rows(w.x3, w.x3c, B, L, resid_row_bytes(W), st)) return rc;
+                    out_lda = (unsigned)((size_t)L * W * 2);
+                }
+                auto tail_resid = [&](const unsigned short* A, unsigned lda_bytes, int K, uint64_t w_off, uint64_t b_off, bool wide_) -> int {
                     GemmArgs g{};
                     g.A = A; g.lda_bytes = lda_bytes; g.W = at<unsigned short>(blob, w_off); g.bias = at<float>(blob, b_off);
-                    g.M = B; g.N = W; g.K = K;
+                    g.M = B; g.N = W; g.K = K; g.skinny_rows = wide_ ? srows : 0;
                     g.x3 = w.x3c; g.ln_part = w.partc; g.tmp_f32 = w.x;
-                    if (tleaf) g.ln_leaf = w.leafc;
+                    if (tleaf || wide_) g.ln_leaf = w.leafc;
                     return launch_gemm_algo(g, EPI_BIAS_RESID_LN_F32, 0, st, nullptr);
                 };
-                if (int rc = tail_resid(w.h, (unsigned)((size_t)L * W * 2), W, lb + t->lo_out_w, lb + t->lo_out_b)) return rc;
+                if (int rc = tail_resid(w.h, out_lda, W, lb + t->lo_out_w, lb + t->lo_out_b, false)) return rc;
                 GemmArgs g{};
                 g.A = static_cast<const unsigned short*>(w.x3c); g.lda_bytes = (unsigned)resid_row_bytes(W);
                 g.W = at<unsigned short>(blob, lb + t->lo_fc_w); g.bias = at<float>(blob, lb + t->lo_fc_cb);
@@ -202,8 +237,9 @@
                 if (tleaf) g.ln_leaf_in = w.leafc;
                 g.out = w.big; g.M = B; g.N = 4 * W; g.K = W;
                 if (int rc = launch_gemm_algo(g, EPI_LN_BIAS_QGELU_BF16, 0, st, nullptr)) return rc;
-                return tail_resid(w.big, 0u, 4 * W, lb + t->lo_proj_w, lb + t->lo_proj_b);
+                return tail_resid(w.big, 0u, 4 * W, lb + t->lo_proj_w, lb + t->lo_proj_b, wide);
             }
+            if (int rc = ln_linear(lb + t->lo_qkv_w, lb + t->lo_qkv_cb, lb + t->lo_qkv_colsum, 3 * W, EPI_LN_BIAS_BF16, probe)) return rc;
             hipEvent_t* aev = nullptr;
             if (probe && probe->mode == 2 && probe->n < GemmProbe::MAX) {
                 const int pi = probe->begin(GemmProbe::EPI_ATTENTION, 2, st, 0);
@@ -211,7 +247,7 @@
             }
             if (int rc = launch_attention(w.big, w.h, B, L, t->heads, causal, 1, st, nullptr, nullptr, nullptr, aev)) return rc;
             if (int rc = resid_linear(w.h, W, lb + t->lo_out_w, lb + t->lo_out_b)) return rc;
-            if (int rc = ln_linear(lb + t->lo_fc_w, lb + t->lo_fc_cb, lb + t->lo_fc_colsum, 4 * W, EPI_LN_BIAS_QGELU_BF16)) return rc;
+            if (int rc = ln_linear(lb + t->lo_fc_w, lb + t->lo_fc_cb, lb + t->lo_fc_colsum, 4 * W, EPI_LN_BIAS_QGELU_BF16, probe)) return rc;
             if (int rc = resid_linear(w.big, 4 * W, lb + t->lo_proj_w, lb + t->lo_proj_b)) return rc;
         }
         return 0;
diff --git a/cli-p_amd/csrc/gemm.hip b/cli-p_amd/csrc/gemm.hip
--- a/cli-p_amd/csrc/gemm.hip
+++ b/cli-p_amd/csrc/gemm.hip
@@ -111,9 +111,12 @@
     return pct;
 }
 
+static int skinny_limit(const GemmArgs& g) { return g.skinny_rows > SKINNY_MAX_M ? g.skinny_rows : SKINNY_MAX_M; }
+static bool skinny_wide(const GemmArgs& g) { return g.M > SKINNY_MAX_M; }
 static bool skinny_ok(const GemmArgs& g) {
     static const bool off = dev_knob("CLIPMI_GEMM_SKINNY", 1) == 0;
-    return !off && g.M >= 1 && g.M <= SKINNY_MAX_M && g.N % 16 == 0 && g.K % 32 == 0 && g.K >= 32;
+    if (skinny_wide(g) && (g.N % 32 != 0 || g.K % 256 != 0)) return false;
+    return !off && g.M >= 1 && g.M <= skinny_limit(g) && g.N % 16 == 0 && g.K % 32 == 0 && g.K >= 32;
 }
 
 template <int EPI>
@@ -127,14 +130,34 @@
     return 0;
 }
 
-bool gemm_resid_writes_leaves(int M, int N, int K) {
-    GemmArgs g{};
-    g.M = M; g.N = N; g.K = K;
+bool gemm_resid_writes_leaves(int M, int N, int K, int skinny_rows) {
+    GemmArgs g{};
+    g.M = M; g.N = N; g.K = K; g.skinny_rows = skinny_rows;
     return skinny_ok(g) && N % 256 == 0 && N <= 1024;
+}
+
+template <int EPI>
+static int launch_skinny_wide_t(const GemmArgs& g, hipStream_t st) {
+    constexpr int RT = 2, CT = 2;
+    const int ngroups = g.N / (16 * CT), mtiles = (g.M + 16 * RT - 1) / (16 * RT);
+    const int waves = ngroups * mtiles <= 4 * NUM_CU ? 1 : 4;
+    const dim3 grid((ngroups + waves - 1) / waves, mtiles);
+    hipLaunchKernelGGL((gemm_skinny_wide_kernel<EPI, RT, CT, 8>), grid, dim3(waves * 64), 0, st, g);
+    CLIPMI_CHECK_LAUNCH("gemm_skinny_wide_kernel");
+    return 0;
 }
 
 static int launch_skinny(const GemmArgs& g, int epi, hipStream_t st) {
     if (!g.A || !g.W || (!g.out && epi != EPI_BIAS_RESID_LN_F32)) return set_err(CLIPMI_EINVAL, "gemm: NULL pointer");
+    if (skinny_wide(g)) {
+        if (!g.bias) return set_err(CLIPMI_EINVAL, "gemm_skinny_wide: NULL bias");
+        switch (epi) {
+            case EPI_LN_BIAS_BF16: return launch_skinny_wide_t<EPI_LN_BIAS_BF16>(g, st);
+            case EPI_LN_BIAS_QGELU_BF16: return launch_skinny_wide_t<EPI_LN_BIAS_QGELU_BF16>(g, st);
+            case EPI_BIAS_RESID_LN_F32: return launch_skinny_wide_t<EPI_BIAS_RESID_LN_F32>(g, st);
+        }
+        return set_err(CLIPMI_EINVAL, "gemm_skinny_wide: epilogue %d", epi);
+    }
     switch (epi) {
         case EPI_BIAS_BF16: return launch_skinny_t<EPI_BIAS_BF16>(g, st);
         case EPI_BIAS_QGELU_BF16: return launch_skinny_t<EPI_BIAS_QGELU_BF16>(g, st);
@@ -213,11 +236,12 @@
         }
     }
     if (g.M < 1 || !g.A || !g.W || (!g.out && epi != EPI_BIAS_RESID_LN_F32)) return set_err(CLIPMI_EINVAL, "gemm: bad arguments");
-    const bool skinny = algo == 0 && skinny_ok(g);
+    const bool skinny = algo == 0 && skinny_ok(g) &&
+                        (!skinny_wide(g) || epi_is_ln(epi) || (epi == EPI_BIAS_RESID_LN_F32 && g.ln_leaf));
     if (skinny && epi != EPI_BIAS_RESID_LN_F32) return launch_skinny(g, epi, st);
     if (epi == EPI_BIAS_RESID_LN_F32 && skinny && g.ln_leaf) return launch_skinny(g, epi, st);
     if (g.ln_leaf_in && !(skinny && epi_is_ln(epi)))
-        return set_err(CLIPMI_EINVAL, "gemm: ln_leaf_in is read by the skinny LN-folded consumers only (M <= %d)", SKINNY_MAX_M);
+        return set_err(CLIPMI_EINVAL, "gemm: ln_leaf_in is read by the skinny LN-folded consumers only (M <= %d)", skinny_limit(g));
     if (epi == EPI_BIAS_RESID_LN_F32 && !use256p) {
         GemmArgs t = g;
         t.out = g.tmp_f32;
diff --git a/cli-p_amd/csrc/gemm.hpp b/cli-p_amd/csrc/gemm.hpp
--- a/cli-p_amd/csrc/gemm.hpp
+++ b/cli-p_amd/csrc/gemm.hpp
@@ -213,8 +213,10 @@
     unsigned lda_bytes;
     float* ln_leaf;
     const float* ln_leaf_in;
+    int skinny_rows;
 };
 constexpr int SKINNY_MAX_M = 128;
+constexpr int TAIL_SKINNY_MAX_M = 1024;
 __host__ __device__ inline size_t gemm_lda(const GemmArgs& g) { return g.lda_bytes ? (size_t)g.lda_bytes / 2 : (size_t)g.K; }
 
 __device__ __forceinline__ void gemm_tile_coords(int bid, int nwg, int mtiles, int ntn, int GM, int GN, int& bm, int& bn) {
@@ -410,7 +412,7 @@
 int launch_gemm(const GemmArgs& g, int epi, hipStream_t st, GemmProbe* probe = nullptr);
 int launch_gemm_algo(const GemmArgs& g, int epi, int algo, hipStream_t st, GemmProbe* probe = nullptr);
 int launch_gemm_fp8(const GemmArgs& g, int epi, hipStream_t st, int mx = 1);
-bool gemm_resid_writes_leaves(int M, int N, int K);
+bool gemm_resid_writes_leaves(int M, int N, int K, int skinny_rows = 0);
 bool gemm_fp8_emits_mx(int M, int N, int K);
 int launch_split_stats(const float* x_or_add, bool add, void* x3, float* part, int M, int W, hipStream_t st);
 
diff --git a/cli-p_amd/csrc/gemm_skinny.hpp b/cli-p_amd/csrc/gemm_skinny.hpp
--- a/cli-p_amd/csrc/gemm_skinny.hpp
+++ b/cli-p_amd/csrc/gemm_skinny.hpp
@@ -126,4 +126,139 @@
     if (valid) *reinterpret_cast<f32x4*>(static_cast<float*>(g.out) + orow * g.N + n) = v;
 }
 
+template <int EPI, int RT, int CT, int DEPTH>
+__global__ void __launch_bounds__(256) gemm_skinny_wide_kernel(GemmArgs g) {
+    static_assert(epi_is_ln(EPI) || EPI == EPI_BIAS_RESID_LN_F32, "the tail's epilogues");
+    const int lane = threadIdx.x & 63;
+    const int wave = __builtin_amdgcn_readfirstlane(threadIdx.x >> 6);
+    const int fr = lane & 15, fg = lane >> 4;
+    const int ngroups = g.N / (16 * CT);
+    const int grp = blockIdx.x * (blockDim.x >> 6) + wave;
+    if (grp >= ngroups) return;
+    const int n0 = grp * (16 * CT), m0 = blockIdx.y * (16 * RT);
+    const int K = g.K;
+    const int nk = K >> 5;
+    const bf16x8* wp[CT];
+    const bf16x8* ap[RT];
+    size_t orow[RT];
+    bool valid[RT];
+#pragma unroll
+    for (int ct = 0; ct < CT; ++ct) wp[ct] = reinterpret_cast<const bf16x8*>(g.W + (size_t)(n0 + 16 * ct + fr) * K + 8 * fg);
+#pragma unroll
+    for (int rt = 0; rt < RT; ++rt) {
+        int am = m0 + 16 * rt + fr;
+        valid[rt] = am < g.M;
+        am = valid[rt] ? am : g.M - 1;
+        orow[rt] = (size_t)am;
+        ap[rt] = reinterpret_cast<const bf16x8*>(g.A + (size_t)am * gemm_lda(g) + 8 * fg);
+    }
+    f32x4 bz[CT], cs[CT];
+#pragma unroll
+    for (int ct = 0; ct < CT; ++ct) {
+        const int n = n0 + 16 * ct + 4 * fg;
+        bz[ct] = *reinterpret_cast<const f32x4*>(g.bias + n);
+        cs[ct] = epi_is_ln(EPI) ? *reinterpret_cast<const f32x4*>(g.colsum + n) : f32x4{0.f, 0.f, 0.f, 0.f};
+    }
+
+    f32x4 acc[RT][CT];
+#pragma unroll
+    for (int rt = 0; rt < RT; ++rt)
+#pragma unroll
+        for (int ct = 0; ct < CT; ++ct) acc[rt][ct] = f32x4{0.f, 0.f, 0.f, 0.f};
+    bf16x8 wf[DEPTH][CT], af[DEPTH][RT];
+#pragma unroll
+    for (int d = 0; d < DEPTH; ++d) {
+        const int s = d < nk ? d : nk - 1;
+#pragma unroll
+        for (int ct = 0; ct < CT; ++ct) wf[d][ct] = wp[ct][4 * s];
+#pragma unroll
+        for (int rt = 0; rt < RT; ++rt) af[d][rt] = ap[rt][4 * s];
+    }
+    for (int s0 = 0; s0 < nk; s0 += DEPTH) {
+#pragma unroll
+        for (int d = 0; d < DEPTH; ++d) {
+            if (s0 + d < nk) {
+#pragma unroll
+                for (int rt = 0; rt < RT; ++rt)
+#pragma unroll
+                    for (int ct = 0; ct < CT; ++ct)
+                        acc[rt][ct] = __builtin_amdgcn_mfma_f32_16x16x32_bf16(wf[d][ct], af[d][rt], acc[rt][ct], 0, 0, 0);
+            }
+            int s = s0 + d + DEPTH;
+            s = s < nk ? s : nk - 1;
+#pragma unroll
+            for (int ct = 0; ct < CT; ++ct) wf[d][ct] = wp[ct][4 * s];
+#pragma unroll
+            for (int rt = 0; rt < RT; ++rt) af[d][rt] = ap[rt][4 * s];
+        }
+    }
+
+#pragma unroll
+    for (int rt = 0; rt < RT; ++rt) {
+        if (epi_is_ln(EPI)) {
+            const int nseg = K >> 8;
+            float part[8] = {0.f, 0.f, 0.f, 0.f, 0.f, 0.f, 0.f, 0.f};
+            if (!g.ln_leaf_in) {
+                const float* pp = g.ln_part_in + orow[rt] * 2 * nseg;
+#pragma unroll
+                for (int i = 0; i < 4; ++i)
+                    if (i < nseg) { part[2 * i] = pp[2 * i]; part[2 * i + 1] = pp[2 * i + 1]; }
+            } else {
+                const f32x2* lf = reinterpret_cast<const f32x2*>(g.ln_leaf_in) + orow[rt] * (size_t)(K >> 2) + fg;
+#pragma unroll
+                for (int j = 0; j < 4; ++j) {
+                    if (j < nseg) {
+                        f32x2 v[16];
+#pragma unroll
+                        for (int t = 0; t < 16; ++t) v[t] = lf[64 * j + 4 * t];
+                        float sm[2];
+#pragma unroll
+                        for (int c = 0; c < 2; ++c) {
+                            float a[8], b[4];
+#pragma unroll
+                            for (int t = 0; t < 8; ++t) a[t] = v[t][c] + v[t + 8][c];
+#pragma unroll
+                            for (int t = 0; t < 4; ++t) b[t] = a[t] + a[t + 4];
+                            const float c0 = b[0] + b[2], c1 = b[1] + b[3];
+                            float d = c0 + c1;
+                            d = lane_fold32(d, d);
+                            sm[c] = lane_fold16(d, d);
+                        }
+                        part[2 * j] = sm[0];
+                        part[2 * j + 1] = sm[1];
+                    }
+                }
+            }
+            const f32x2 st = ln_row_stats(part, K >> 8, K);
+#pragma unroll
+            for (int ct = 0; ct < CT; ++ct) {
+                const int n = n0 + 16 * ct + 4 * fg;
+                f32x4 v = ln_apply(acc[rt][ct], st.x, st.y, cs[ct], bz[ct]);
+                if (epi_is_qgelu(EPI)) v = quick_gelu4(v);
+                if (valid[rt])
+                    *reinterpret_cast<uint2*>(static_cast<unsigned short*>(g.out) + orow[rt] * g.N + n) =
+                        make_uint2(pack_bf16x2(v.x, v.y), pack_bf16x2(v.z, v.w));
+            }
+        } else {
+#pragma unroll
+            for (int ct = 0; ct < CT; ++ct) {
+                const int n = n0 + 16 * ct + 4 * fg;
+                const uint2 xh = *reinterpret_cast<const uint2*>(resid_hi(g.x3, orow[rt], g.N) + n);
+                const unsigned xl = *reinterpret_cast<const unsigned*>(resid_lo(g.x3, orow[rt], g.N) + n);
+                const f32x4 v = acc[rt][ct] + bz[ct];
+                const f32x4 o = v + split_join(xh, xl);
+                uint2 nh;
+                unsigned nl;
+                split_make(o, nh, nl);
+                if (valid[rt]) {
+                    *reinterpret_cast<uint2*>(resid_hi(g.x3, orow[rt], g.N) + n) = nh;
+                    *reinterpret_cast<unsigned*>(resid_lo(g.x3, orow[rt], g.N) + n) = nl;
+                    *reinterpret_cast<f32x2*>(g.ln_leaf + (orow[rt] * (size_t)(g.N >> 2) + (size_t)(n >> 2)) * 2) =
+                        f32x2{ln_lane_sum(o), ln_lane_sumsq(o)};
+                }
+            }
+        }
+    }
 }
+
+}
diff --git a/cli-p_amd/csrc/vit_kernels.hip b/cli-p_amd/csrc/vit_kernels.hip
--- a/cli-p_amd/csrc/vit_kernels.hip
+++ b/cli-p_amd/csrc/vit_kernels.hip
@@ -55,15 +55,16 @@
         const long long resident = (long long)NUM_CU * 5;
         if (out8 && out_bs && fused) {
             hipLaunchKernelGGL(attention52x4_kernel<true>, dim3((unsigned)(items < resident ? items : resident)), dim3(256),
-                               64 * 128 + 52 * 128, st, qkv, out, B, L, heads, out8, out_bs);
+                               64 * 128 + 52 * 128, st, qkv, out, B, L, heads, out8, out_bs, (const unsigned short*)nullptr);
             *fused = true;
         } else if (probe_ev) {
             hipExtLaunchKernelGGL(attention52x4_kernel<false>, dim3((unsigned)(items < resident ? items : resident)), dim3(256),
                                   64 * 128 + 52 * 128, st, probe_ev[0], probe_ev[1], 0, qkv, out, B, L, heads, (unsigned char*)nullptr,
-                                  (unsigned char*)nullptr);
+                                  (unsigned char*)nullptr, (const unsigned short*)nullptr);
         } else {
             hipLaunchKernelGGL(attention52x4_kernel<false>, dim3((unsigned)(items < resident ? items : resident)), dim3(256),
-                               64 * 128 + 52 * 128, st, qkv, out, B, L, heads, (unsigned char*)nullptr, (unsigned char*)nullptr);
+                               64 * 128 + 52 * 128, st, qkv, out, B, L, heads, (unsigned char*)nullptr, (unsigned char*)nullptr,
+                               (const unsigned short*)nullptr);
         }
         CLIPMI_CHECK_LAUNCH("attention52x4_kernel");
         return 0;
@@ -85,6 +86,20 @@
     ATT(1) ATT(2) ATT(4) ATT(5)
 #undef ATT
     return set_err(CLIPMI_EUNSUPPORTED, "attention: L=%d", L);
+}
+
+bool attention_cls_ok(int L) { return L >= 49 && L <= 52; }
+
+int launch_attention_cls(const unsigned short* q, const unsigned short* kv, unsigned short* out, int B, int L, int heads,
+                         hipStream_t st) {
+    if (B < 1) return 0;
+    if (!attention_cls_ok(L)) return set_err(CLIPMI_EUNSUPPORTED, "attention_cls: L=%d (49 <= L <= 52)", L);
+    const long long items = (long long)B * heads;
+    const long long resident = (long long)NUM_CU * 5;
+    hipLaunchKernelGGL((attention52x4_kernel<false, true>), dim3((unsigned)(items < resident ? items : resident)), dim3(256),
+                       64 * 128 + 52 * 128, st, kv, out, B, L, heads, (unsigned char*)nullptr, (unsigned char*)nullptr, q);
+    CLIPMI_CHECK_LAUNCH("attention52x4_kernel<cls>");
+    return 0;
 }
 
 int launch_quantize_rows_fp8(const unsigned short* in, unsigned char* out, float* scale, int M, int K, hipStream_t st) {
@@ -143,6 +158,12 @@
                             heads, causal & 1, (causal & 2) ? 0 : ((causal & 4) ? 2 : 1), as_stream(stream));
 }
 
+extern "C" int clipmi_dbg_attention_cls(const void* q_dev, const void* kv_dev, void* out_dev, int B, int L, int heads, void* stream) {
+    if (!q_dev || !kv_dev || !out_dev) return set_err(CLIPMI_EINVAL, "dbg_attention_cls: NULL pointer");
+    return launch_attention_cls(static_cast<const unsigned short*>(q_dev), static_cast<const unsigned short*>(kv_dev),
+                                static_cast<unsigned short*>(out_dev), B, L, heads, as_stream(stream));
+}
+
 extern "C" int clipmi_dbg_quantize_rows_fp8(const void* in_bf16_dev, void* out_fp8_dev, float* scale_dev, int M, int K,
                                             void* stream) {
     return launch_quantize_rows_fp8(static_cast<const unsigned short*>(in_bf16_dev), static_cast<unsigned char*>(out_fp8_dev),
diff --git a/cli-p_amd/csrc/vit_kernels.hpp b/cli-p_amd/csrc/vit_kernels.hpp
--- a/cli-p_amd/csrc/vit_kernels.hpp
+++ b/cli-p_amd/csrc/vit_kernels.hpp
@@ -115,11 +115,18 @@
 }
 
 static __global__ void __launch_bounds__(256) gather_rows_kernel(const uint4* __restrict__ src, uint4* __restrict__ dst, int B,
-                                                                 int row_step, int row16) {
-    const long long i = (long long)blockIdx.x * 256 + threadIdx.x;
-    if (i >= (long long)B * row16) return;
-    const int b = (int)(i / row16), c = (int)(i - (long long)b * row16);
-    dst[(size_t)b * row16 + c] = src[(size_t)b * row_step * row16 + c];
+                                                                 int row_step, int row16, const uint2* __restrict__ ssrc,
+                                                                 uint2* __restrict__ sdst, int srow8) {
+    long long i = (long long)blockIdx.x * 256 + threadIdx.x;
+    if (i < (long long)B * row16) {
+        const int b = (int)(i / row16), c = (int)(i - (long long)b * row16);
+        dst[(size_t)b * row16 + c] = src[(size_t)b * row_step * row16 + c];
+        return;
+    }
+    i -= (long long)B * row16;
+    if (i >= (long long)B * srow8) return;
+    const int b = (int)(i / srow8), c = (int)(i - (long long)b * srow8);
+    sdst[(size_t)b * srow8 + c] = ssrc[(size_t)b * row_step * srow8 + c];
 }
 
 static __global__ void __launch_bounds__(256) text_embed_kernel(float* x, const int* ids, const float* tok, const float* pos,
@@ -686,40 +693,45 @@
     }
 }
 
-template <bool OUT8>
+template <bool OUT8, bool CLS = false>
 static __global__ void __launch_bounds__(256, 5) attention52x4_kernel(const unsigned short* __restrict__ qkv,
                                                                       unsigned short* __restrict__ out, int B, int L,
-                                                                      int heads, unsigned char* __restrict__ out8, unsigned char* __restrict__ out_bs) {
+                                                                      int heads, unsigned char* __restrict__ out8, unsigned char* __restrict__ out_bs,
+                                                                      const unsigned short* __restrict__ qc) {
     extern __shared__ __attribute__((aligned(16))) char smem[];
     constexpr int NT = 4, ROWS = 52;
     const int lane = threadIdx.x & 63;
     const int wave = __builtin_amdgcn_readfirstlane(threadIdx.x >> 6);
     const int fr = lane & 15, fg = lane >> 4;
     const int W = heads * 64;
-    const size_t rs = (size_t)3 * W;
+    const size_t rs = (size_t)(CLS ? 2 : 3) * W;
+    const int koff = CLS ? 0 : W, voff = koff + W;
+    const bool computes = !CLS || wave == 0;
     char* kt_ = smem;
     char* vt = smem + 64 * 128;
     const int srow = lane >> 3, sch = lane & 7;
     const int items = B * heads;
 
-    bf16x8 q0n, q1n;
+    bf16x8 q0n = {}, q1n = {};
     uint4 kdn0, kdn1, vdn0, vdn1;
 #define ATT52_FETCH(IT)                                                                                  \
     do {                                                                                                 \
         const int b_ = (IT) / heads, h_ = (IT) - b_ * heads;                                             \
-        const unsigned short* base_ = qkv + (size_t)b_ * L * 3 * W + h_ * 64;                            \
+        const unsigned short* base_ = qkv + (size_t)b_ * L * rs + h_ * 64;                               \
         int qrow_ = wave * 16 + fr;                                                                      \
         qrow_ = qrow_ < L ? qrow_ : L - 1;                                                               \
-        const unsigned short* qp_ = base_ + (size_t)qrow_ * rs + fg * 8;                                 \
-        q0n = *reinterpret_cast<const bf16x8*>(qp_);                                                     \
-        q1n = *reinterpret_cast<const bf16x8*>(qp_ + 32);                                                \
+        const unsigned short* qp_ = CLS ? qc + (size_t)b_ * W + h_ * 64 + fg * 8 : base_ + (size_t)qrow_ * rs + fg * 8; \
+        if (computes) {                                                                                  \
+            q0n = *reinterpret_cast<const bf16x8*>(qp_);                                                 \
+            q1n = *reinterpret_cast<const bf16x8*>(qp_ + 32);                                            \
+        }                                                                                                \
         int r0_ = (wave * 2) * 8 + srow, r1_ = (wave * 2 + 1) * 8 + srow;    \
         r0_ = r0_ < L ? r0_ : L - 1;                                         \
         r1_ = r1_ < L ? r1_ : L - 1;                                                                     \
-        kdn0 = *reinterpret_cast<const uint4*>(base_ + (size_t)r0_ * rs + W + sch * 8);                  \
-        vdn0 = *reinterpret_cast<const uint4*>(base_ + (size_t)r0_ * rs + 2 * W + sch * 8);              \
-        kdn1 = *reinterpret_cast<const uint4*>(base_ + (size_t)r1_ * rs + W + sch * 8);                  \
-        vdn1 = *reinterpret_cast<const uint4*>(base_ + (size_t)r1_ * rs + 2 * W + sch * 8);              \
+        kdn0 = *reinterpret_cast<const uint4*>(base_ + (size_t)r0_ * rs + koff + sch * 8);               \
+        vdn0 = *reinterpret_cast<const uint4*>(base_ + (size_t)r0_ * rs + voff + sch * 8);               \
+        kdn1 = *reinterpret_cast<const uint4*>(base_ + (size_t)r1_ * rs + koff + sch * 8);               \
+        vdn1 = *reinterpret_cast<const uint4*>(base_ + (size_t)r1_ * rs + voff + sch * 8);               \
     } while (0)
     int item = blockIdx.x;
     if (item >= items) return;
@@ -739,6 +751,7 @@
         if (has_next) ATT52_FETCH(nxt);
         __syncthreads();
 
+    if (computes) {
     bf16x8 kf[NT][2];
 #pragma unroll
     for (int t = 0; t < NT; ++t) {
@@ -845,8 +858,8 @@
                 if (fg == 0) out_bs[row_ * (W >> 5) + h * 2 + j] = (unsigned char)sb_;
             }
         }
-    } else if (qi < L) {
-        unsigned short* dst = out + ((size_t)b * L + qi) * W + h * 64 + 4 * (fg & ~1);
+    } else if (CLS ? fr == 0 : qi < L) {
+        unsigned short* dst = out + (CLS ? (size_t)b : (size_t)b * L + qi) * W + h * 64 + 4 * (fg & ~1);
 #pragma unroll
         for (int j = 0; j < 2; ++j) {
             const int dt = 2 * j + (odd ? 1 : 0);
@@ -854,6 +867,7 @@
                                 : make_uint4(mine[j].x, mine[j].y, theirs[j].x, theirs[j].y);
             *reinterpret_cast<uint4*>(dst + dt * 16) = v;
         }
+    }
     }
         if (!has_next) break;
         item = nxt;
@@ -1037,6 +1051,9 @@
 int launch_attention(const unsigned short* qkv, unsigned short* out, int B, int L, int heads, int causal, int tr,
                      hipStream_t st, unsigned char* out8 = nullptr, unsigned char* out_bs = nullptr, bool* fused = nullptr,
                      hipEvent_t* probe_ev = nullptr);
+bool attention_cls_ok(int L);
+int launch_attention_cls(const unsigned short* q, const unsigned short* kv, unsigned short* out, int B, int L, int heads,
+                         hipStream_t st);
 int launch_patchify(const PatchArgs& a, hipStream_t st);
 int launch_quantize_rows_fp8(const unsigned short* in, unsigned char* out, float* scale, int M, int K, hipStream_t st);
 int launch_quantize_rows_fp8mx(const unsigned short* in, unsigned char* out, unsigned char* bscale, int M, int K, hipStream_t st);
diff --git a/include/clipmi.h b/include/clipmi.h
--- a/include/clipmi.h
+++ b/include/clipmi.h
@@ -182,6 +182,8 @@
                          void* out_dev, int M, int W, int out_bf16, void* stream);
 int clipmi_dbg_attention(const void* qkv_dev, void* out_dev, int B, int L, int heads,
                          int causal, void* stream);
+int clipmi_dbg_attention_cls(const void* q_dev, const void* kv_dev, void* out_dev, int B, int L, int heads,
+                             void* stream);
 
 int clipmi_dbg_topk_scan_ms(const void* db_dev, int64_t N, int E, const float* q_dev, int Q, int K,
                             float* out_score_dev, int64_t* out_id_dev, void* ws_dev, size_t ws_bytes,
```

Result: no change. 108,700, median of 6 (+0.5%).
